# anilshanbhag/gpu-sort

Measured on AMD Instinct MI355X. Metric: Gkeys/s sorting 2^30 uint32 keys; achieved HBM GB/s vs roofline, higher is better.
Workload: dtype u32; 1 GPU; lsb_radix_sort_2^30_u32_uniform_keys_only; keys_per_gpu=1073741824, algorithm=lsb, distribution=uniform, parallelism=single

## Files before the change

### gpu-sort_amd/_lib.py

```python
import ctypes as C
import os

import torch

_HERE = os.path.dirname(os.path.abspath(__file__))
LIB_PATH = os.environ.get("GS_LIB_PATH", os.path.join(_HERE, "lib", "libgpusort.so"))
CSRC_DIR = os.path.join(_HERE, "csrc")
INCLUDE_DIR = os.path.join(os.path.dirname(_HERE), "include")

GS_KEY_U32, GS_KEY_I32, GS_KEY_F32, GS_KEY_U64, GS_KEY_I64, GS_KEY_F64 = 0, 1, 2, 3, 4, 5
GS_KEY_U8, GS_KEY_I8, GS_KEY_U16, GS_KEY_I16 = 6, 7, 8, 9
GS_KEY_F16, GS_KEY_BF16, GS_KEY_F8 = 10, 11, 12
GS_GEN_UNIFORM, GS_GEN_ZIPF, GS_GEN_ENTROPY_AND, GS_GEN_ENUMERATED = 0, 1, 2, 3

u64, i32, vp, sz = C.c_uint64, C.c_int, C.c_void_p, C.c_size_t
pp = C.POINTER(C.c_void_p)

SIGNATURES = {
    "gs_version": (i32, []),
    "gs_error_string": (C.c_char_p, [i32]),
    "gs_lsb_temp_bytes": (sz, [u64, i32]),
    "gs_lsb_sort_u32": (i32, [vp, sz, pp, pp, C.POINTER(i32), u64, i32, i32, i32, i32, vp]),
    "gs_lsb_copy_temp_bytes": (sz, [u64, i32]),
    "gs_lsb_sort_copy_u32": (i32, [vp, sz, vp, vp, vp, vp, u64, i32, i32, i32, i32, vp]),
    "gs_lsb_wide_temp_bytes": (sz, [u64, i32, i32]),
    "gs_lsb_sort_wide": (i32, [vp, sz, pp, pp, C.POINTER(i32), u64, i32, i32, i32, i32, i32, i32, vp]),
    "gs_lsb_any_temp_bytes": (sz, [u64, i32, i32]),
    "gs_lsb_sort_any": (i32, [vp, sz, vp, vp, vp, vp, u64, i32, i32, i32, i32, i32, vp]),
    "gs_lsb_narrow_temp_bytes": (sz, [u64, i32, i32]),
    "gs_lsb_sort_narrow": (i32, [vp, sz, vp, vp, vp, vp, u64, i32, i32, i32, i32, i32, vp]),
    "gs_lsb_narrow_tile": (C.c_uint32, [i32, i32]),
    "gs_lsb_geometry": (None, [u64, i32, C.POINTER(C.c_uint32), C.POINTER(C.c_uint32), C.POINTER(C.c_uint32)]),
    "gs_lsb_workspace_layout": (i32, [vp, u64, pp, pp, pp]),
    "gs_lsb_pipe_status": (i32, [vp, u64, C.POINTER(C.c_uint32), vp]),
    "gs_lsb_plan_status": (i32, [vp, u64, C.POINTER(C.c_uint32), vp]),
    "gs_lsb_plan_cursor_status": (i32, [vp, u64, C.POINTER(C.c_uint32), vp]),
    "gs_lsb_plan_peek_status": (i32, [C.POINTER(C.c_uint32)]),
    "gs_lsb_plan_look_only": (i32, [vp, vp, vp, u64, i32, i32, vp]),
    "gs_lsb_plan_layout": (i32, [u64, C.POINTER(C.c_uint64)]),
    "gs_lsb_upsweep_u32": (i32, [vp, sz, vp, u64, i32, i32, i32, i32, vp]),
    "gs_lsb_scan_spine": (i32, [vp, sz, u64, vp]),
    "gs_lsb_downsweep_u32": (i32, [vp, sz, vp, vp, vp, vp, u64, i32, i32, i32, i32, i32, vp]),
    "gs_msb_temp_bytes": (sz, [u64, i32]),
    "gs_msb_sort_u32": (i32, [vp, sz, vp, vp, u64, vp, vp, pp, pp, i32, vp, i32]),
    "gs_msb_wide_temp_bytes": (sz, [u64, i32, i32]),
    "gs_msb_sort_wide": (i32, [vp, sz, vp, vp, u64, vp, vp, i32, i32, pp, pp, i32, vp, i32]),
    "gs_msb_large_temp_bytes": (sz, [u64, i32]),
    "gs_msb_sort_large_u32": (i32, [vp, sz, vp, vp, u64, vp, vp, i32, vp, i32]),
    "gs_msb_large_wide_temp_bytes": (sz, [u64, i32, i32]),
    "gs_msb_sort_large_wide": (i32, [vp, sz, vp, vp, u64, vp, vp, i32, i32, i32, vp, i32]),
    "gs_lsb_large_temp_bytes": (sz, [u64, i32, i32]),
    "gs_lsb_sort_large": (i32, [vp, sz, pp, pp, C.POINTER(i32), u64, i32, i32, i32, i32, i32, i32, vp]),
    "gs_lsb_narrow_large_temp_bytes": (sz, [u64, i32, i32]),
    "gs_lsb_sort_narrow_large": (i32, [vp, sz, vp, vp, vp, vp, u64, i32, i32, i32, i32, i32, vp]),
    "gs_topk_temp_bytes": (sz, [u64, u64, i32]),
    "gs_topk_u32": (i32, [vp, sz, vp, vp, vp, vp, u64, u64, i32, i32, vp]),
    "gs_topk_status": (i32, [vp, u64, u64, i32, C.POINTER(C.c_uint32), vp]),
    "gs_topk_u16_temp_bytes": (sz, [u64, u64, i32]),
    "gs_topk_u16": (i32, [vp, sz, vp, vp, vp, vp, u64, u64, i32, i32, vp]),
    "gs_topk_u16_status": (i32, [vp, u64, u64, i32, C.POINTER(C.c_uint32), vp]),
    "gs_topk_u64_temp_bytes": (sz, [u64, u64, i32]),
    "gs_topk_u64": (i32, [vp, sz, vp, vp, vp, vp, u64, u64, i32, i32, vp]),
    "gs_topk_u64_status": (i32, [vp, u64, u64, i32, C.POINTER(C.c_uint32), vp]),
    "gs_topk_rows_temp_bytes": (sz, [u64, u64, u64, i32]),
    "gs_topk_rows_u32": (i32, [vp, sz, vp, vp, vp, vp, u64, u64, u64, u64, i32, i32, vp]),
    "gs_topk_rows_max_k": (C.c_uint32, []),
    "gs_topk_rows_plan": (i32, [u64, u64, u64, i32, C.POINTER(C.c_uint32)]),
    "gs_topk_rows_u16_temp_bytes": (sz, [u64, u64, u64, i32]),
    "gs_topk_rows_u16": (i32, [vp, sz, vp, vp, vp, vp, u64, u64, u64, u64, i32, i32, vp]),
    "gs_topk_rows_u64_temp_bytes": (sz, [u64, u64, u64, i32]),
    "gs_topk_rows_u64": (i32, [vp, sz, vp, vp, vp, vp, u64, u64, u64, u64, i32, i32, vp]),
    "gs_topk_segmented_temp_bytes": (sz, [u64, C.c_uint32, u64, i32]),
    "gs_topk_segmented_u32": (i32, [vp, sz, vp, vp, vp, vp, vp, u64, C.c_uint32, vp, vp, u64, i32, i32, vp]),
    "gs_topk_segmented_u16_temp_bytes": (sz, [u64, C.c_uint32, u64, i32]),
    "gs_topk_segmented_u16": (i32, [vp, sz, vp, vp, vp, vp, vp, u64, C.c_uint32, vp, vp, u64, i32, i32, vp]),
    "gs_topk_segmented_u64_temp_bytes": (sz, [u64, C.c_uint32, u64, i32]),
    "gs_topk_segmented_u64": (i32, [vp, sz, vp, vp, vp, vp, vp, u64, C.c_uint32, vp, vp, u64, i32, i32, vp]),
    "gs_topk_segmented_plan": (i32, [u64, C.c_uint32, u64, i32, C.POINTER(C.c_uint32)]),
    "gs_topk_segmented_status": (i32, [vp, u64, C.c_uint32, u64, i32, C.POINTER(C.c_uint32), vp]),
    "gs_msb_census": (i32, [vp, u64, i32, vp, vp]),
    "gs_msb_wide_census": (i32, [vp, u64, i32, i32, vp, vp]),
    "gs_msb_capacities": (None, [u64, i32, C.POINTER(C.c_uint32), C.POINTER(C.c_uint32), C.POINTER(C.c_uint32)]),
    "gs_msb_classify_upto": (i32, [vp, sz, vp, vp, u64, i32, i32, vp]),
    "gs_msb_read_lists": (i32, [vp, u64, i32, i32, vp, C.c_uint32, C.POINTER(C.c_uint32), C.POINTER(C.POINTER(C.c_uint32)), C.c_uint32,
                                C.POINTER(C.c_uint32), vp]),
    "gs_segmented_temp_bytes": (sz, [u64, i32, C.c_uint32]),
    "gs_segmented_sort_u32": (i32, [vp, sz, pp, pp, C.POINTER(i32), u64, C.c_uint32, vp, vp, i32, i32, i32, i32, vp]),
    "gs_segmented_wide_temp_bytes": (sz, [u64, i32, i32, C.c_uint32]),
    "gs_segmented_sort_wide": (i32, [vp, sz, pp, pp, C.POINTER(i32), u64, C.c_uint32, vp, vp, i32, i32, i32, i32, i32, i32, vp]),
    "gs_segmented_narrow_temp_bytes": (sz, [u64, i32, i32, C.c_uint32]),
    "gs_segmented_sort_narrow": (i32, [vp, sz, pp, pp, C.POINTER(i32), u64, C.c_uint32, vp, vp, i32, i32, i32, i32, i32, vp]),
    "gs_segmented_narrow_cap": (C.c_uint32, [i32, i32]),
    "gs_msb_first_pass_u32": (i32, [vp, sz, vp, vp, vp, vp, u64, i32, vp, vp]),
    "gs_msb_finish_temp_bytes": (sz, [u64, i32, i32]),
    "gs_msb_finish_u32": (i32, [vp, sz, vp, vp, vp, vp, u64, vp, i32, i32, vp, i32]),
    "gs_shard_histogram_u32": (i32, [vp, u64, i32, vp, i32, vp]),
    "gs_shard_partition_u32": (i32, [vp, sz, vp, vp, vp, vp, u64, i32, vp, i32, vp, vp, i32, vp]),
    "gs_generate_u32": (i32, [vp, u64, i32, u64, u64, i32, vp]),
    "gs_check_sorted_u32": (i32, [vp, u64, i32, vp, vp]),
    "gs_check_pairs_enumerated_u32": (i32, [vp, vp, vp, u64, vp, vp]),
    "gs_check_sorted_u64": (i32, [vp, u64, i32, vp, vp]),
    "gs_check_pairs_enumerated_wide": (i32, [vp, vp, vp, u64, i32, vp, vp]),
    "gs_check_sorted_stable": (i32, [vp, vp, u64, i32, i32, i32, i32, i32, vp, vp]),
    "gs_profile_create": (vp, []),
    "gs_profile_destroy": (None, [vp]),
    "gs_profile_begin": (None, [vp]),
    "gs_profile_end": (None, []),
    "gs_profile_read": (i32, [vp, C.POINTER(C.c_double), C.POINTER(u64)]),
    "gs_kernel_name": (C.c_char_p, [i32]),
}
GS_K_COUNT = 10


class GpuSortError(RuntimeError):
    def __init__(self, code, what):
        self.code = code
        super().__init__(f"{what}: hipError {code} ({error_string(code)})")


def _load():
    if not os.path.exists(LIB_PATH):
        raise ImportError(
            f"{LIB_PATH} is missing: the HIP extension is not built. "
            "Run `python -c 'import __graft_entry__ as g; g.build()'` (or make -C gpu-sort_amd/csrc). "
            "There is no CPU fallback."
        )
    lib = C.CDLL(LIB_PATH)
    for name, (res, args) in SIGNATURES.items():
        fn = getattr(lib, name)
        fn.restype = res
        fn.argtypes = args
    return lib


lib = _load()


def error_string(code):
    s = lib.gs_error_string(int(code))
    return s.decode() if s else "?"


def check(code, what):
    if code != 0:
        raise GpuSortError(code, what)


class KernelProfile:

    def __init__(self):
        self._p = lib.gs_profile_create()

    def __enter__(self):
        lib.gs_profile_begin(self._p)
        return self

    def __exit__(self, *exc):
        lib.gs_profile_end()
        return False

    def read(self):
        ms = (C.c_double * GS_K_COUNT)()
        cnt = (u64 * GS_K_COUNT)()
        check(lib.gs_profile_read(self._p, ms, cnt), "gs_profile_read")
        return {lib.gs_kernel_name(i).decode(): (ms[i], int(cnt[i])) for i in range(GS_K_COUNT) if cnt[i]}

    def close(self):
        if self._p and lib is not None:
            lib.gs_profile_destroy(self._p)
        self._p = None

    def __del__(self):
        try:
            self.close()
        except Exception:
            pass
```

### gpu-sort_amd/csrc/gs_lsb_downsweep.inc

```
#ifndef GS_EXP_SLEEP_MODE
#define GS_EXP_SLEEP_MODE 0
#endif
#ifndef GS_EXP_SLEEP_MIN_TILES
#define GS_EXP_SLEEP_MIN_TILES 49152u
#endif
#ifndef GS_EXP_SLEEP_PAIRS
#define GS_EXP_SLEEP_PAIRS 0
#endif
template <bool HAS_VALUES, bool OFF64 = false>
struct DownsweepSmem {
    uint32_t whist[LSB_WAVES][RADIX];
#ifdef GS_EXP_ALLWAVE_KEYS
    uint16_t wbase[LSB_WAVES][RADIX];
#else
    uint16_t wbase[HAS_VALUES ? LSB_WAVES : 1][RADIX];
#endif
    std::conditional_t<OFF64, uint64_t, uint32_t> gbase[RADIX];
    uint32_t stage[LSB_TILE * (HAS_VALUES ? 2 : 1)];
    uint32_t dead;
};

#ifdef GS_EXP_PHASES
__device__ uint32_t gs_phase_buf[131072 * 16];
#define GS_PHASE(k)                                                                          \
    do {                                                                                     \
        const unsigned long long now_ = __builtin_amdgcn_s_memtime();                        \
        if (tid == 0 && t < 131072u) gs_phase_buf[t * 16 + (k)] = (uint32_t)(now_ - tprev_); \
        tprev_ = now_;                                                                       \
    } while (0)
#define GS_PHASE_WAIT(what) asm volatile("s_waitcnt " what ::: "memory")
#else
#define GS_PHASE(k) do { } while (0)
#define GS_PHASE_WAIT(what) do { } while (0)
#endif

constexpr uint32_t PIPE_SPIN_LIMIT = 1u << 18;

template <bool HAS_VALUES, bool TAIL, int TW, bool BIG, bool PIPE, bool OFF64 = false, bool CURSOR = false>
__device__ __forceinline__ void downsweep_tile(DownsweepSmem<HAS_VALUES, OFF64> &sm, const uint32_t t,
    const uint32_t *__restrict__ keys_in, uint32_t *__restrict__ keys_out, const uint32_t *__restrict__ vals_in,
    uint32_t *__restrict__ vals_out, const uint32_t *__restrict__ spine, const uint16_t *__restrict__ prefix16,
    const uint32_t *__restrict__ totals, const PassParams &p, const uint64_t *__restrict__ sc, uint32_t tag,
    uint32_t *__restrict__ error_word, const uint32_t tid_ = threadIdx.x, const uint64_t *__restrict__ dbase = nullptr,
    uint32_t *__restrict__ cursor = nullptr, uint32_t *__restrict__ irr = nullptr, const uint32_t irr_cap = 0u)
{
    static_assert(!CURSOR || (!HAS_VALUES && !TAIL && !PIPE && !OFF64), "cursor mode: full tiles of keys-only three-launch passes");
#ifdef GS_EXP_ALLWAVE_KEYS
    constexpr bool ALLWAVE = true;
#else
    constexpr bool ALLWAVE = HAS_VALUES;
#endif

    [[maybe_unused]] const int tid = (int)tid_;
    const int lane = (int)(tid_ & 63u), w = (int)(tid_ >> 6);
    const uint32_t full_tiles = p.n / (uint32_t)LSB_TILE;
    auto tw_in = [&](uint32_t k) { return TW == 0 ? k : twiddle_in(k, TW == 2 ? p.f32_in : 0, p.xor_in); };
    auto tw_out = [&](uint32_t k) { return TW == 0 ? k : twiddle_out(k, TW == 2 ? p.f32_out : 0, p.xor_out); };
    uint32_t wbits = p.bits;
    asm volatile("" : "+v"(wbits));
    auto digit = [&](uint32_t k) { return __builtin_amdgcn_ubfe(k, p.shift, wbits); };

    uint32_t *my = sm.whist[w];
    const uint16_t *mybase = sm.wbase[w];
    const uint32_t wbase = (uint32_t)w * (WAVE * LSB_KPT) + lane;
    const uint32_t tail_valid = p.n - full_tiles * (uint32_t)LSB_TILE;
    (void)full_tiles;

#ifdef GS_EXP_PHASES
    unsigned long long tprev_ = __builtin_amdgcn_s_memtime();
    const unsigned long long t0_ = tprev_, r0_ = __builtin_amdgcn_s_memrealtime();
#endif
#ifdef GS_EXP_SLEEP_START
    __builtin_amdgcn_s_sleep(GS_EXP_SLEEP_START);
#endif
    if (!HAS_VALUES) __builtin_amdgcn_s_setprio(3);
    const uint64_t tile_base = (uint64_t)t * LSB_TILE;
    const uint32_t valid = TAIL ? tail_valid : (uint32_t)LSB_TILE;

    uint64_t scg[4] = {0, 0, 0, 0};
    const uint64_t *scrow = nullptr;
    if (PIPE && w == 0) {
        scrow = sc + (size_t)(t / LSB_CHUNK) * RADIX + 4 * lane;
#pragma unroll
        for (int q = 0; q < 4; ++q) scg[q] = ld_agent(scrow + q);
    }

    uint32_t key[LSB_KPT], val[HAS_VALUES ? LSB_KPT : 1], pos[LSB_KPT];
    {
        const uint32_t *kin = keys_in + tile_base;
        if (!TAIL) {
#pragma unroll
            for (int i = 0; i < LSB_KPT; ++i) key[i] = kin[wbase + i * WAVE];
        } else {
            const uint32_t pad = twiddle_out(0xffffffffu, TW == 2 ? p.f32_in : 0, TW ? p.xor_in : 0u);
#pragma unroll
            for (int i = 0; i < LSB_KPT; ++i) {
                const uint32_t idx = wbase + i * WAVE;
                key[i] = pad;
                if (idx < tail_valid) key[i] = kin[idx];
            }
        }
    }
    [[maybe_unused]] uint32_t cur_lo = 0, cur_hi = 0, claim[4] = {0, 0, 0, 0};
    if constexpr (CURSOR) {
        if (w == 0) {
            cur_lo = (tw_in(keys_in[tile_base]) >> (p.shift - (uint32_t)RADIX_BITS)) & (uint32_t)(RADIX - 1);
            cur_hi = (tw_in(keys_in[tile_base + (LSB_TILE - 1)]) >> (p.shift - (uint32_t)RADIX_BITS)) & (uint32_t)(RADIX - 1);
        }
    }
    GS_PHASE(0);
#ifndef GS_EXP_RANK_PRIO
#define GS_EXP_RANK_PRIO 0
#endif
    if (!HAS_VALUES) __builtin_amdgcn_s_setprio(GS_EXP_RANK_PRIO);
    if (HAS_VALUES) {
        const uint32_t *vin = vals_in + tile_base;
#pragma unroll
        for (int i = 0; i < LSB_KPT; ++i) {
            const uint32_t idx = wbase + i * WAVE;
            val[i] = 0;
            if (!TAIL || idx < valid) val[i] = vin[idx];
        }
    }
    uint32_t dstart[4] = {0, 0, 0, 0};
    if constexpr (OFF64) {
        if (TAIL && w == 0) {
            const uint4 tot = reinterpret_cast<const uint4 *>(totals)[lane];
            dstart[0] = tot.x; dstart[1] = tot.y; dstart[2] = tot.z; dstart[3] = tot.w;
        }
    } else if (!CURSOR && w == 0) {
        const uint4 tot = reinterpret_cast<const uint4 *>(totals)[lane];
        const uint32_t lane_sum = tot.x + tot.y + tot.z + tot.w;
        const uint32_t ex = wave_inclusive_scan(lane_sum) - lane_sum;
        dstart[0] = ex + (TAIL ? tot.x : 0u);
        dstart[1] = dstart[0] + (TAIL ? tot.y : tot.x);
        dstart[2] = dstart[1] + (TAIL ? tot.z : tot.y);
        dstart[3] = dstart[2] + (TAIL ? tot.w : tot.z);
    }

    uint32_t tbase[4] = {0, 0, 0, 0};
    if (!TAIL && !PIPE && !CURSOR && w == 0) {
        const uint32_t *sp = spine + (uint32_t)(4 * lane) * p.grid + t / LSB_CHUNK;
        const uint2 pf = reinterpret_cast<const uint2 *>(prefix16 + (size_t)t * RADIX)[lane];
        tbase[0] = sp[0] + (pf.x & 0xffffu);
        tbase[1] = sp[p.grid] + (pf.x >> 16);
        tbase[2] = sp[2 * p.grid] + (pf.y & 0xffffu);
        tbase[3] = sp[3 * p.grid] + (pf.y >> 16);
    }

    if (PIPE && !TAIL && w == 0) {
        uint32_t spins = 0;
        bool gave_up = false;
        for (;;) {
            const bool ok = (uint32_t)(scg[0] >> 32) == tag && (uint32_t)(scg[1] >> 32) == tag &&
                            (uint32_t)(scg[2] >> 32) == tag && (uint32_t)(scg[3] >> 32) == tag;
            if (__builtin_amdgcn_ballot_w64(!ok) == 0) break;
            if (++spins > PIPE_SPIN_LIMIT) {
                if (lane == 0) atomicOr(error_word, 1u);
                gave_up = true;
                break;
            }
            __builtin_amdgcn_s_sleep(8);
#pragma unroll
            for (int q = 0; q < 4; ++q) scg[q] = ld_agent(scrow + q);
        }
        if (lane == 0) sm.dead = gave_up ? 1u : 0u;
        const uint64_t pf = ld_agent(reinterpret_cast<const uint64_t *>(prefix16 + (size_t)t * RADIX) + lane);
        tbase[0] = (uint32_t)scg[0] + (uint32_t)(pf & 0xffffu);
        tbase[1] = (uint32_t)scg[1] + (uint32_t)((pf >> 16) & 0xffffu);
        tbase[2] = (uint32_t)scg[2] + (uint32_t)((pf >> 32) & 0xffffu);
        tbase[3] = (uint32_t)scg[3] + (uint32_t)(pf >> 48);
    }

    auto publish_gbase = [&](const uint32_t (&ex)[4], const uint32_t (&run)[4]) {
        uint32_t g[4];
#pragma unroll
        for (int q = 0; q < 4; ++q) g[q] = dstart[q] + tbase[q] - ex[q];
        if (TAIL) {
#pragma unroll
            for (int q = 0; q < 4; ++q) g[q] -= run[q];
            const uint32_t pads = (uint32_t)LSB_TILE - valid, dmax = p.mask;
            if (lane == (int)(dmax >> 2)) {
#pragma unroll
                for (int q = 0; q < 4; ++q)
                    if ((dmax & 3u) == (uint32_t)q) g[q] += pads;
            }
        }
        if constexpr (OFF64) {
#pragma unroll
            for (int q = 0; q < 4; ++q) sm.gbase[4 * lane + q] = dbase[4 * lane + q] + (uint64_t)(int64_t)(int32_t)g[q];
        } else {
            if (!BIG) {
#pragma unroll
                for (int q = 0; q < 4; ++q) g[q] <<= 2;
            }
            reinterpret_cast<uint4 *>(sm.gbase)[lane] = make_uint4(g[0], g[1], g[2], g[3]);
        }
    };

#pragma unroll
    for (int i = lane; i < RADIX; i += WAVE) my[i] = 0;
    GS_PHASE_WAIT("vmcnt(0)");
    GS_PHASE(1);
#pragma unroll
    for (int i = 0; i < LSB_KPT; ++i) key[i] = tw_in(key[i]);
    {
        uint32_t d_prev = 0, plo = 0, phi = 0;
#pragma unroll
        for (int i = 0; i <= LSB_KPT; ++i) {
            uint32_t d_cur = 0, clo = 0, chi = 0;
            if (i < LSB_KPT) {
                d_cur = digit(key[i]);
                match_digit(d_cur, clo, chi);
            }
            if (i > 0) {
                const uint32_t lower = count_lower(plo, phi);
                pos[i - 1] = my[d_prev] + lower;
                if (lower == 0)
                    __hip_atomic_fetch_add(&my[d_prev], (uint32_t)(__popc(plo) + __popc(phi)), __ATOMIC_RELAXED,
                                           __HIP_MEMORY_SCOPE_WAVEFRONT);
            }
            d_prev = d_cur; plo = clo; phi = chi;
        }
    }
#pragma unroll
    for (int i = 0; i < LSB_KPT; ++i) {
        asm volatile("" : "+v"(pos[i]), "+v"(key[i]));
    }
    if constexpr (CURSOR) {
        if (w == 0 && lane == 0) {
            const bool straddles = cur_lo != cur_hi;
            sm.dead = straddles ? 1u : 0u;
            if (straddles) {
                const uint32_t at = atomicAdd(&irr[0], 1u);
                if (at < irr_cap) irr[1u + at] = t;
            }
        }
    }
    GS_PHASE_WAIT("lgkmcnt(0)");
    GS_PHASE(2);
    __syncthreads();
    GS_PHASE(3);
    if (PIPE && !TAIL && sm.dead) return;
    if (CURSOR && sm.dead) return;

    if constexpr (ALLWAVE) {
        uint32_t run[4] = {0, 0, 0, 0}, below[4] = {0, 0, 0, 0};
#pragma unroll
        for (int j = 0; j < LSB_WAVES; ++j) {
            const uint4 x = reinterpret_cast<const uint4 *>(sm.whist[j])[lane];
            run[0] += x.x; run[1] += x.y; run[2] += x.z; run[3] += x.w;
            if (j < w) { below[0] += x.x; below[1] += x.y; below[2] += x.z; below[3] += x.w; }
        }
        const uint32_t lane_sum = run[0] + run[1] + run[2] + run[3];
        uint32_t ex[4];
        ex[0] = wave_inclusive_scan(lane_sum) - lane_sum;
        ex[1] = ex[0] + run[0];
        ex[2] = ex[1] + run[1];
        ex[3] = ex[2] + run[2];
        reinterpret_cast<uint2 *>(sm.wbase[w])[lane] =
            make_uint2((ex[0] + below[0]) | ((ex[1] + below[1]) << 16), (ex[2] + below[2]) | ((ex[3] + below[3]) << 16));
        if (w == 0) publish_gbase(ex, run);
    } else {
        if (w == 0) {
            uint32_t run[4] = {0, 0, 0, 0};
#pragma unroll
            for (int j = 0; j < LSB_WAVES; ++j) {
                const uint4 x = reinterpret_cast<const uint4 *>(sm.whist[j])[lane];
                run[0] += x.x; run[1] += x.y; run[2] += x.z; run[3] += x.w;
            }
            const uint32_t lane_sum = run[0] + run[1] + run[2] + run[3];
            uint32_t ex[4];
            ex[0] = wave_inclusive_scan(lane_sum) - lane_sum;
            ex[1] = ex[0] + run[0];
            ex[2] = ex[1] + run[1];
            ex[3] = ex[2] + run[2];
            if constexpr (CURSOR) {
                reinterpret_cast<uint4 *>(sm.gbase)[lane] = make_uint4(ex[0], ex[1], ex[2], ex[3]);
                uint32_t *row = cursor + (size_t)__builtin_amdgcn_readfirstlane(cur_lo) * RADIX;
#pragma unroll
                for (int q = 0; q < 4; ++q) {
                    const int d = q * WAVE + lane;
                    const uint32_t e0 = sm.gbase[d], e1 = sm.gbase[d == RADIX - 1 ? d : d + 1];
                    const uint32_t cnt = (d == RADIX - 1 ? (uint32_t)LSB_TILE : e1) - e0;
                    claim[q] = __hip_atomic_fetch_add(row + d, cnt, __ATOMIC_RELAXED, __HIP_MEMORY_SCOPE_AGENT);
                }
            } else {
                publish_gbase(ex, run);
            }
            asm volatile("" ::: "memory");
            uint4 e4 = make_uint4(ex[0] << 2, ex[1] << 2, ex[2] << 2, ex[3] << 2);
#pragma unroll
            for (int j = 0; j < LSB_WAVES; ++j) {
                const uint4 x = reinterpret_cast<const uint4 *>(sm.whist[j])[lane];
                reinterpret_cast<uint4 *>(sm.whist[j])[lane] = e4;
                e4.x += x.x << 2; e4.y += x.y << 2; e4.z += x.z << 2; e4.w += x.w << 2;
            }
        }
        __syncthreads();
    }
    GS_PHASE(4);

    {
        uint32_t wb[LSB_KPT];
#pragma unroll
        for (int i = 0; i < LSB_KPT; ++i) {
            const uint32_t d = digit(key[i]);
            wb[i] = ALLWAVE ? (uint32_t)mybase[d] : my[d];
        }
#pragma unroll
        for (int i = 0; i < LSB_KPT; ++i) {
            if (HAS_VALUES) {
                reinterpret_cast<uint2 *>(sm.stage)[pos[i] + wb[i]] = make_uint2(key[i], val[i]);
            } else if (ALLWAVE) {
                sm.stage[pos[i] + wb[i]] = key[i];
            } else {
                const uint32_t at = (pos[i] << 2) + wb[i];
                *reinterpret_cast<uint32_t *>(reinterpret_cast<char *>(sm.stage) + at) = key[i];
            }
        }
    }
    if constexpr (CURSOR) {
        if (w == 0) {
#pragma unroll
            for (int q = 0; q < 4; ++q) {
                const int d = q * WAVE + lane;
                const uint32_t g = claim[q] - sm.gbase[d];
                sm.gbase[d] = BIG ? g : g << 2;
            }
        }
    }
    GS_PHASE_WAIT("lgkmcnt(0)");
    GS_PHASE(5);
    __syncthreads();
    GS_PHASE(6);
#ifndef GS_EXP_SLEEP
#define GS_EXP_SLEEP 32
#define GS_EXP_SLEEP_MODE_DEFAULT 0
#else
#define GS_EXP_SLEEP_MODE_DEFAULT GS_EXP_SLEEP_MODE
#endif
    if ((!HAS_VALUES || GS_EXP_SLEEP_PAIRS) && full_tiles >= GS_EXP_SLEEP_MIN_TILES) {
        [[maybe_unused]] const int ws = __builtin_amdgcn_readfirstlane(w);
#if GS_EXP_SLEEP_MODE_DEFAULT == 3
        if (ws & 1) __builtin_amdgcn_s_sleep(GS_EXP_SLEEP); else __builtin_amdgcn_s_sleep(GS_EXP_SLEEP_B);
#elif GS_EXP_SLEEP_MODE_DEFAULT == 4
        if (ws >= 4) __builtin_amdgcn_s_sleep(GS_EXP_SLEEP);
#elif GS_EXP_SLEEP_MODE_DEFAULT == 1
        if (ws & 1) __builtin_amdgcn_s_sleep(GS_EXP_SLEEP);
#elif GS_EXP_SLEEP_MODE_DEFAULT == 0
        __builtin_amdgcn_s_sleep(GS_EXP_SLEEP);
#endif
    }
#ifndef GS_EXP_STORE_PRIO
#define GS_EXP_STORE_PRIO 3
#endif
    if (!HAS_VALUES) __builtin_amdgcn_s_setprio(GS_EXP_STORE_PRIO);
#pragma unroll
    for (int i = 0; i < LSB_KPT; ++i) {
        const uint32_t slot = (uint32_t)w * (WAVE * LSB_KPT) + i * WAVE + lane;
        uint32_t k, v = 0;
        if (HAS_VALUES) {
            const uint2 kv = reinterpret_cast<const uint2 *>(sm.stage)[slot];
            k = kv.x; v = kv.y;
        } else {
            k = sm.stage[slot];
        }
        const auto g = sm.gbase[digit(k)];
        if (!TAIL || slot < valid) {
            if constexpr (OFF64) {
                const uint64_t dst = g + slot;
                keys_out[dst] = tw_out(k);
                if (HAS_VALUES) vals_out[dst] = v;
            } else if (BIG) {
                const uint32_t dst = g + slot;
                keys_out[dst] = tw_out(k);
                if (HAS_VALUES) vals_out[dst] = v;
            } else {
                const uint32_t off = g + slot * 4u;
                *reinterpret_cast<uint32_t *>(reinterpret_cast<char *>(keys_out) + off) = tw_out(k);
                if (HAS_VALUES) *reinterpret_cast<uint32_t *>(reinterpret_cast<char *>(vals_out) + off) = v;
            }
        }
    }
    GS_PHASE(7);
#ifdef GS_EXP_DRAIN
    asm volatile("s_waitcnt vmcnt(0)" ::: "memory");
#endif
    GS_PHASE_WAIT("vmcnt(0)");
    GS_PHASE(8);
#ifdef GS_EXP_PHASES
    if (tid == 0 && t < 131072u) {
        gs_phase_buf[t * 16 + 9] = (uint32_t)(__builtin_amdgcn_s_memtime() - t0_);
        gs_phase_buf[t * 16 + 10] = (uint32_t)(__builtin_amdgcn_s_memrealtime() - r0_);
        gs_phase_buf[t * 16 + 11] = (uint32_t)r0_;
        gs_phase_buf[t * 16 + 12] = blockIdx.x;
        gs_phase_buf[t * 16 + 13] = __builtin_amdgcn_s_getreg((31 << 11) | 4);
        gs_phase_buf[t * 16 + 14] = __builtin_amdgcn_s_getreg((31 << 11) | 20);
    }
#endif
}
```

### gpu-sort_amd/csrc/gs_lsb_plan.hip

```cpp
#include "gs_device.hpp"
#include "gs_lsb.hpp"
#include "gs_msb_tasks.hpp"
#ifndef GS_PLAN_N_MIN
#define GS_PLAN_N_MIN (1ull << 28)
#endif
#include <cstddef>
#include <cstdlib>
#include <cstring>
#include <type_traits>

namespace gs {

#include "gs_lsb_upsweep.inc"

#include "gs_lsb_downsweep.inc"

constexpr uint32_t PLAN_GROUPS = 65536;
constexpr uint32_t PLAN_WORDS = PLAN_GROUPS / 2;
constexpr uint32_t PLAN_PLANNED = 1u, PLAN_CLASSIC = 2u;
constexpr uint32_t PLAN_SKIP = 0xffffffffu;
constexpr int PLAN_LOOK_THREADS = 1024, PLAN_LOOK_WAVES = PLAN_LOOK_THREADS / WAVE, PLAN_LOOK_BATCH = 32;
constexpr uint32_t PLAN_LOOK_HALVES = PLAN_LOOK_WAVES / LSB_CHUNK;
static_assert(PLAN_LOOK_WAVES % LSB_CHUNK == 0, "a look workgroup takes whole chunks");
constexpr uint32_t PLAN_LOOK_MAX_GRID = MI355X_CUS;
constexpr uint32_t PLAN_BLOCKS = 128, PLAN_BLOCK_WORDS = PLAN_WORDS / PLAN_BLOCKS, PLAN_BLOCK_GROUPS = PLAN_GROUPS / PLAN_BLOCKS;
constexpr int PLAN_SORT_BITS = 16;
constexpr int PLAN_SKEW_LANES = 8;
constexpr uint32_t PLAN_IRR_CAP = RADIX - 1;
constexpr size_t PLAN_CURSOR_BYTES = (size_t)PLAN_GROUPS * sizeof(uint32_t);

struct PlanBlock {
    uint32_t route, max_group, nonempty, tasks[MSB_NCLASS], total;
    uint32_t shift[4];
    uint32_t ups_skip[4];
    MsbLevel level[2];
    union {
        uint32_t wg_bad[PLAN_LOOK_MAX_GRID];
        uint32_t irr[1 + PLAN_IRR_CAP];
    };
    uint32_t blk_total[PLAN_BLOCKS], blk_max[PLAN_BLOCKS], blk_nonempty[PLAN_BLOCKS];
    uint32_t blk_class[PLAN_BLOCKS][MSB_NCLASS];
    uint32_t blk_class_base[PLAN_BLOCKS][MSB_NCLASS];
    uint32_t offsets[PLAN_GROUPS + 1];
    uint32_t cursor_mode;
};
static_assert(1 + PLAN_IRR_CAP <= PLAN_LOOK_MAX_GRID, "the list of straddling tiles fits the look's flags");
static_assert(sizeof(MsbLevel) == 64 && offsetof(PlanBlock, level) == 64, "plan block layout");

__device__ __forceinline__ int plan_class_of(uint32_t size)
{
    return size <= msb_class_cap(0) ? 0 : size <= msb_class_cap(1) ? 1 : size <= msb_class_cap(2) ? 2 : 3;
}

__device__ __forceinline__ void look_add(uint32_t *tab, uint32_t *my, uint32_t g)
{
    const unsigned long long act = __builtin_amdgcn_ballot_w64(true);
    const uint32_t g0 = __builtin_amdgcn_readfirstlane(g);
    if (__builtin_amdgcn_ballot_w64(g == g0) == act) {
        if (count_lower_mask(act) == 0) {
            atomicAdd(&tab[g0 >> 1], (uint32_t)__popcll(act) << ((g0 & 1u) * 16u));
            atomicAdd(&my[g0 & 0xffu], (uint32_t)__popcll(act));
        }
    } else {
        atomicAdd(&tab[g >> 1], 1u << ((g & 1u) * 16u));
        atomicAdd(&my[g & 0xffu], 1u);
    }
}

__device__ __forceinline__ void look_add_skew(uint32_t *tab, uint32_t *my, uint32_t g, int lane)
{
    unsigned long long rest = ~0ull;
#pragma unroll
    for (int r = 0; r < 2; ++r) {
        if (rest == 0ull) break;
        const int lead = __builtin_amdgcn_readfirstlane(__builtin_ctzll(rest));
        const uint32_t g0 = (uint32_t)__builtin_amdgcn_readlane((int)g, lead);
        const unsigned long long m = __builtin_amdgcn_ballot_w64(g == g0) & rest;
        if (lane == lead) {
            atomicAdd(&tab[g0 >> 1], (uint32_t)__popcll(m) << ((g0 & 1u) * 16u));
            atomicAdd(&my[g0 & 0xffu], (uint32_t)__popcll(m));
        }
        rest &= ~m;
    }
    if ((rest >> lane) & 1ull) {
        atomicAdd(&tab[g >> 1], 1u << ((g & 1u) * 16u));
        atomicAdd(&my[g & 0xffu], 1u);
    }
}

__device__ __forceinline__ uint32_t look_slot_of_block(uint32_t b, uint32_t grid)
{
    if (grid % MI355X_XCDS) return b;
    return (b % MI355X_XCDS) * (grid / MI355X_XCDS) + b / MI355X_XCDS;
}

struct LookSmem {
    uint32_t tab[PLAN_WORDS];
    uint32_t hist[PLAN_LOOK_WAVES][RADIX + 1];
    uint32_t red[2];
};
static_assert(sizeof(LookSmem) <= 160 * 1024, "the look's LDS");

__global__ __launch_bounds__(PLAN_LOOK_THREADS) void lsb_plan_look_kernel(const uint32_t *__restrict__ keys, uint32_t *__restrict__ partial,
                                                                          PlanBlock *__restrict__ plan, uint32_t *__restrict__ spine,
                                                                          uint16_t *__restrict__ prefix16, uint32_t n, uint32_t chunks,
                                                                          int f32_in, uint32_t xor_in)
{
    __shared__ LookSmem sm;
    uint32_t *tab = sm.tab;
    const int tid = threadIdx.x, w = wave_id(), lane = lane_id();
    for (uint32_t i = tid; i < PLAN_WORDS; i += PLAN_LOOK_THREADS) tab[i] = 0;
    for (uint32_t i = tid; i < sizeof(sm.hist) / sizeof(uint32_t); i += PLAN_LOOK_THREADS) (&sm.hist[0][0])[i] = 0;
    if (tid < 2) sm.red[tid] = 0;
    __syncthreads();
    uint32_t *my = sm.hist[w];
    const uint32_t num_tiles = n / (uint32_t)LSB_TILE + (n % (uint32_t)LSB_TILE ? 1u : 0u);
    const uint32_t units = (chunks + PLAN_LOOK_HALVES - 1u) / PLAN_LOOK_HALVES;
    auto group_of = [&](uint32_t raw) { return twiddle_in(raw, f32_in, xor_in) >> 16; };
    uint32_t counted = 0;
    constexpr int GB = PLAN_LOOK_BATCH;
#pragma unroll 1
    for (uint32_t unit = look_slot_of_block(blockIdx.x, gridDim.x); unit < units; unit += gridDim.x) {
        const uint32_t tile = unit * (uint32_t)PLAN_LOOK_WAVES + (uint32_t)w;
        if (tile < num_tiles) {
        const uint32_t lo = tile * (uint32_t)LSB_TILE;
        const uint32_t len = (n - lo < (uint32_t)LSB_TILE) ? n - lo : (uint32_t)LSB_TILE;
        const uint32_t *src = keys + lo;
        counted += len;
        if (len == (uint32_t)LSB_TILE) {
#pragma unroll 1
            for (uint32_t j = 0; j < (uint32_t)LSB_TILE; j += GB * WAVE) {
                const uint32_t *at = src + j + lane;
                uint32_t v[GB];
#pragma unroll
                for (int u = 0; u < GB; ++u) v[u] = __builtin_nontemporal_load(at + u * WAVE);
                const uint32_t ga = group_of(v[0]), gb = group_of(v[GB / 2]);
                const unsigned long long ma = __builtin_amdgcn_ballot_w64(ga == __builtin_amdgcn_readfirstlane(ga)),
                                         mb = __builtin_amdgcn_ballot_w64(gb == __builtin_amdgcn_readfirstlane(gb));
                if (ma == ~0ull || mb == ~0ull) {
#pragma unroll
                    for (int u = 0; u < GB; ++u) look_add(tab, my, group_of(v[u]));
                } else if (__popcll(ma) >= PLAN_SKEW_LANES || __popcll(mb) >= PLAN_SKEW_LANES) {
#pragma unroll
                    for (int u = 0; u < GB; ++u) look_add_skew(tab, my, group_of(v[u]), lane);
                } else {
#pragma unroll
                    for (int u = 0; u < GB; ++u) {
                        const uint32_t g = group_of(v[u]);
                        atomicAdd(&tab[g >> 1], 1u << ((g & 1u) * 16u));
                        atomicAdd(&my[g & 0xffu], 1u);
                    }
                }
            }
        } else {
            const uint32_t last = len - 1u;
#pragma unroll 1
            for (uint32_t j = 0; j < len; j += GB * WAVE) {
                uint32_t v[GB];
#pragma unroll
                for (int u = 0; u < GB; ++u) {
                    const uint32_t idx = j + u * WAVE + lane;
                    v[u] = src[idx < last ? idx : last];
                }
#pragma unroll
                for (int u = 0; u < GB; ++u)
                    if (j + u * WAVE + lane < len) look_add(tab, my, group_of(v[u]));
            }
        }
        }
        __syncthreads();
        if (tid < (int)PLAN_LOOK_HALVES * RADIX) {
            const uint32_t half = (uint32_t)tid / RADIX, d = (uint32_t)tid % RADIX, chunk = unit * PLAN_LOOK_HALVES + half;
            uint32_t run = 0;
#pragma unroll
            for (int j = 0; j < LSB_CHUNK; ++j) {
                const uint32_t t = chunk * LSB_CHUNK + (uint32_t)j;
                if (t < num_tiles) prefix16[(size_t)t * RADIX + d] = (uint16_t)run;
                uint32_t *c = &sm.hist[half * LSB_CHUNK + j][d];
                run += *c;
                *c = 0;
            }
            if (chunk < chunks) spine[d * chunks + chunk] = run;
        }
        __syncthreads();
    }
    uint32_t sum = 0;
    uint32_t *out = partial + (size_t)blockIdx.x * PLAN_WORDS;
    for (uint32_t i = tid; i < PLAN_WORDS; i += PLAN_LOOK_THREADS) {
        const uint32_t c = tab[i];
        sum += (c & 0xffffu) + (c >> 16);
        out[i] = c;
    }
    sum = wave_reduce_sum(sum);
    if (lane == 0) { atomicAdd(&sm.red[0], sum); atomicAdd(&sm.red[1], counted); }
    __syncthreads();
    if (tid == 0) plan->wg_bad[blockIdx.x] = sm.red[0] != sm.red[1] ? 1u : 0u;
}

__global__ __launch_bounds__(RADIX) void lsb_plan_reduce_kernel(const uint32_t *__restrict__ partial, PlanBlock *__restrict__ plan, uint32_t parts)
{
    __shared__ uint32_t scratch[8];
    __shared__ uint32_t red[2 + MSB_NCLASS];
    const uint32_t tid = threadIdx.x, wi = blockIdx.x * PLAN_BLOCK_WORDS + tid;
    if (tid < 2 + MSB_NCLASS) red[tid] = 0;
    uint32_t c0 = 0, c1 = 0;
#pragma unroll 8
    for (uint32_t g = 0; g < parts; ++g) {
        const uint32_t v = partial[(size_t)g * PLAN_WORDS + wi];
        c0 += v & 0xffffu;
        c1 += v >> 16;
    }
    uint32_t total = 0;
    const uint32_t ex = block_exclusive_scan_256(c0 + c1, scratch, &total);
    plan->offsets[2 * wi] = ex;
    plan->offsets[2 * wi + 1] = ex + c0;
    atomicMax(&red[0], c0 > c1 ? c0 : c1);
    if (c0) { atomicAdd(&red[1], 1u); atomicAdd(&red[2 + plan_class_of(c0)], 1u); }
    if (c1) { atomicAdd(&red[1], 1u); atomicAdd(&red[2 + plan_class_of(c1)], 1u); }
    __syncthreads();
    if (tid == 0) {
        plan->blk_total[blockIdx.x] = total;
        plan->blk_max[blockIdx.x] = red[0];
        plan->blk_nonempty[blockIdx.x] = red[1];
    }
    if (tid < MSB_NCLASS) plan->blk_class[blockIdx.x][tid] = red[2 + tid];
}

__global__ __launch_bounds__(RADIX) void lsb_plan_decide_kernel(PlanBlock *__restrict__ plan, uint32_t n, uint32_t parts, uint32_t cursor_on)
{
    __shared__ uint32_t s_base, s_total, s_max, s_nz, s_cls[MSB_NCLASS], s_clsbase[MSB_NCLASS];
    const uint32_t tid = threadIdx.x, b = blockIdx.x;
    if (tid == 0) {
        uint32_t base = 0, total = 0, mx = 0, nz = 0;
        for (uint32_t i = 0; i < PLAN_BLOCKS; ++i) {
            if (i == b) base = total;
            total += plan->blk_total[i];
            const uint32_t m = plan->blk_max[i];
            mx = m > mx ? m : mx;
            nz += plan->blk_nonempty[i];
        }
        s_base = base; s_total = total; s_max = mx; s_nz = nz;
    } else if (tid <= MSB_NCLASS) {
        const uint32_t c = tid - 1u;
        uint32_t base = 0, total = 0;
        for (uint32_t i = 0; i < PLAN_BLOCKS; ++i) {
            if (i == b) base = total;
            total += plan->blk_class[i][c];
        }
        s_cls[c] = total; s_clsbase[c] = base;
    }
    const int any_bad = __syncthreads_or(tid < parts ? (int)plan->wg_bad[tid] : 0);
    const uint32_t g = b * PLAN_BLOCK_GROUPS + 2u * tid;
    plan->offsets[g] += s_base;
    plan->offsets[g + 1] += s_base;
    if (tid < MSB_NCLASS) plan->blk_class_base[b][tid] = s_clsbase[tid];
    if (b == 0 && tid == 0) {
        const bool planned = !any_bad && s_total == n && s_max <= msb_class_cap(MSB_NCLASS - 1);
        plan->route = planned ? PLAN_PLANNED : PLAN_CLASSIC;
        plan->max_group = s_max;
        plan->nonempty = s_nz;
        plan->total = s_total;
        MsbLevel l0{}, l1{};
        for (int c = 0; c < MSB_NCLASS; ++c) {
            plan->tasks[c] = planned ? s_cls[c] : 0u;
            l0.task_count[c] = planned ? s_cls[c] : 0u;
        }
        l0.keys = n;
        l1.packed = planned ? (1ull << 32) : 0ull;
        plan->level[0] = l0;
        plan->level[1] = l1;
        for (int q = 0; q < 4; ++q) {
            plan->shift[q] = planned ? (q < 2 ? 16u + 8u * (uint32_t)q : PLAN_SKIP) : 8u * (uint32_t)q;
            plan->ups_skip[q] = planned && q != 1 ? 1u : 0u;
        }
        plan->offsets[PLAN_GROUPS] = n;
        plan->cursor_mode = planned && cursor_on ? 1u : 0u;
    }
}

constexpr int PLAN_PEEK_WORDS = 9;
static_assert(offsetof(PlanBlock, total) == (PLAN_PEEK_WORDS - 2) * sizeof(uint32_t), "the head is eight words");
__global__ void lsb_plan_peek_kernel(const PlanBlock *__restrict__ plan, uint32_t *mailbox)
{
    const uint32_t *head = &plan->route;
    for (int i = 0; i < PLAN_PEEK_WORDS - 1; ++i) mailbox[i] = head[i];
    mailbox[PLAN_PEEK_WORDS - 1] = plan->cursor_mode;
    __threadfence_system();
}

struct PlanLists { MsbTask *tasks[MSB_NCLASS]; uint32_t cap[MSB_NCLASS]; };
__global__ __launch_bounds__(PLAN_BLOCK_GROUPS) void lsb_plan_tasks_kernel(const PlanBlock *__restrict__ plan, PlanLists lists)
{
    __shared__ uint32_t wcnt[PLAN_BLOCK_GROUPS / WAVE][MSB_NCLASS];
    if (plan->route != PLAN_PLANNED) return;
    const uint32_t tid = threadIdx.x, g = blockIdx.x * PLAN_BLOCK_GROUPS + tid;
    const int w = wave_id(), lane = lane_id();
    const uint32_t off = plan->offsets[g], size = plan->offsets[g + 1] - off;
    const int cls = size ? plan_class_of(size) : -1;
    uint32_t lower = 0;
#pragma unroll
    for (int c = 0; c < MSB_NCLASS; ++c) {
        const unsigned long long m = __builtin_amdgcn_ballot_w64(cls == c);
        if (cls == c) lower = count_lower_mask(m);
        if (lane == 0) wcnt[w][c] = (uint32_t)__popcll(m);
    }
    __syncthreads();
    if (cls >= 0) {
        uint32_t idx = plan->blk_class_base[blockIdx.x][cls] + lower;
        for (int j = 0; j < w; ++j) idx += wcnt[j][cls];
        if (idx < lists.cap[cls]) lists.tasks[cls][idx] = MsbTask{off, size, (uint32_t)PLAN_SORT_BITS, 0u};
    }
}

template <bool PLAIN>
__global__ __launch_bounds__(LSB_THREADS, GS_EXP_UPS_WPE) void lsb_plan_upsweep_kernel(const uint32_t *__restrict__ keys,
                                                                       uint32_t *__restrict__ spine, uint16_t *__restrict__ prefix16,
                                                                       const uint32_t *__restrict__ slot_shift,
                                                                       const uint32_t *__restrict__ slot_ups_skip, PassParams p)
{
    __shared__ UpsweepSmem<false, false> sm;
    const uint32_t sh = *slot_shift;
    if (sh == PLAN_SKIP || *slot_ups_skip) return;
    p.shift = sh;
    upsweep_chunk<false, false, PLAIN>(sm, keys, chunk_of_block(blockIdx.x, p.grid), spine, prefix16, nullptr, nullptr, p, PipeParams{});
}

template <bool TAIL, int TW, bool BIG>
__global__ __launch_bounds__(LSB_THREADS, 6) void lsb_plan_downsweep_kernel(const uint32_t *__restrict__ keys_in, uint32_t *__restrict__ keys_out,
                                                                            const uint32_t *__restrict__ totals, const uint32_t *__restrict__ spine,
                                                                            const uint16_t *__restrict__ prefix16,
                                                                            const uint32_t *__restrict__ slot_shift, PassParams p)
{
    __shared__ __attribute__((aligned(16))) DownsweepSmem<false> sm;
    const uint32_t sh = *slot_shift;
    if (sh == PLAN_SKIP) return;
    p.shift = sh;
    const uint32_t full_tiles = p.n / (uint32_t)LSB_TILE;
    if (!TAIL && blockIdx.x >= full_tiles) return;
    const uint32_t t = TAIL ? full_tiles : tile_of_item_wide(blockIdx.x, full_tiles);
    downsweep_tile<false, TAIL, TW, BIG, false>(sm, t, keys_in, keys_out, nullptr, nullptr, spine, prefix16, totals, p, nullptr, 0u, nullptr);
}

template <bool PLAIN>
__global__ __launch_bounds__(LSB_THREADS, GS_EXP_UPS_WPE) void lsb_plan_upsweep2_kernel(const uint32_t *__restrict__ keys,
                                                                        uint32_t *__restrict__ spine, uint16_t *__restrict__ prefix16,
                                                                        PlanBlock *__restrict__ plan, uint32_t *__restrict__ cursor,
                                                                        PassParams p)
{
    __shared__ UpsweepSmem<false, false> sm;
    if (plan->cursor_mode) {
        if (blockIdx.x == 0 && threadIdx.x == 0) plan->irr[0] = 0;
        for (uint32_t i = blockIdx.x * (uint32_t)LSB_THREADS + threadIdx.x; i < PLAN_GROUPS; i += gridDim.x * (uint32_t)LSB_THREADS)
            cursor[i] = plan->offsets[((i & (uint32_t)(RADIX - 1)) << RADIX_BITS) | (i >> RADIX_BITS)];
        return;
    }
    const uint32_t sh = plan->shift[1];
    if (sh == PLAN_SKIP || plan->ups_skip[1]) return;
    p.shift = sh;
    upsweep_chunk<false, false, PLAIN>(sm, keys, chunk_of_block(blockIdx.x, p.grid), spine, prefix16, nullptr, nullptr, p, PipeParams{});
}

template <bool TAIL, bool BIG>
__global__ __launch_bounds__(LSB_THREADS, 6) void lsb_plan_scatter2_kernel(const uint32_t *__restrict__ keys_in, uint32_t *__restrict__ keys_out,
                                                                           const uint32_t *__restrict__ totals, const uint32_t *__restrict__ spine,
                                                                           const uint16_t *__restrict__ prefix16, PlanBlock *__restrict__ plan,
                                                                           uint32_t *__restrict__ cursor, PassParams p)
{
    __shared__ __attribute__((aligned(16))) DownsweepSmem<false> sm;
    const uint32_t sh = plan->shift[1];
    if (sh == PLAN_SKIP) return;
    p.shift = sh;
    const uint32_t full_tiles = p.n / (uint32_t)LSB_TILE;
    const uint32_t mode = plan->cursor_mode;
    if constexpr (TAIL) {
        if (mode) return;
        downsweep_tile<false, true, 2, true, false>(sm, full_tiles, keys_in, keys_out, nullptr, nullptr, spine, prefix16, totals, p, nullptr, 0u,
                                                    nullptr);
    } else {
        if (blockIdx.x >= full_tiles) return;
        const uint32_t t = tile_of_item_wide(blockIdx.x, full_tiles);
        if (mode)
            downsweep_tile<false, false, 0, BIG, false, false, true>(sm, t, keys_in, keys_out, nullptr, nullptr, spine, prefix16, totals, p,
                                                                     nullptr, 0u, nullptr, threadIdx.x, nullptr, cursor, plan->irr, PLAN_IRR_CAP);
        else
            downsweep_tile<false, false, 0, BIG, false>(sm, t, keys_in, keys_out, nullptr, nullptr, spine, prefix16, totals, p, nullptr, 0u,
                                                        nullptr);
    }
}

__global__ __launch_bounds__(LSB_THREADS) void lsb_plan_irregular_kernel(const uint32_t *__restrict__ keys_in, uint32_t *__restrict__ keys_out,
                                                                         const PlanBlock *__restrict__ plan, uint32_t *__restrict__ cursor,
                                                                         uint32_t n)
{
    if (!plan->cursor_mode) return;
    const uint32_t full_tiles = n / (uint32_t)LSB_TILE;
    uint32_t lo, len;
    if (blockIdx.x == PLAN_IRR_CAP) {
        lo = full_tiles * (uint32_t)LSB_TILE;
        len = n - lo;
    } else {
        const uint32_t listed = plan->irr[0] < PLAN_IRR_CAP ? plan->irr[0] : PLAN_IRR_CAP;
        if (blockIdx.x >= listed) return;
        const uint32_t t = plan->irr[1u + blockIdx.x];
        if (t >= full_tiles) return;
        lo = t * (uint32_t)LSB_TILE;
        len = (uint32_t)LSB_TILE;
    }
    const int lane = lane_id();
    for (uint32_t i = threadIdx.x; i - (uint32_t)lane < len; i += (uint32_t)LSB_THREADS) {
        const bool have = i < len;
        const uint32_t k = have ? keys_in[lo + i] : 0u;
        const uint32_t g = k >> 16, c = ((g & (uint32_t)(RADIX - 1)) << RADIX_BITS) | (g >> RADIX_BITS);
        unsigned long long rest = __builtin_amdgcn_ballot_w64(have);
        uint32_t at = 0;
#pragma unroll
        for (int r = 0; r < 2; ++r) {
            if (rest == 0ull) break;
            const int lead = __builtin_amdgcn_readfirstlane(__builtin_ctzll(rest));
            const uint32_t c0 = (uint32_t)__builtin_amdgcn_readlane((int)c, lead);
            const unsigned long long m = __builtin_amdgcn_ballot_w64(have && c == c0) & rest;
            uint32_t first = 0;
            if (lane == lead) first = __hip_atomic_fetch_add(cursor + c0, (uint32_t)__popcll(m), __ATOMIC_RELAXED, __HIP_MEMORY_SCOPE_AGENT);
            first = (uint32_t)__builtin_amdgcn_readlane((int)first, lead);
            if ((m >> lane) & 1ull) at = first + (uint32_t)__popcll(m & ((1ull << lane) - 1ull));
            rest &= ~m;
        }
        if ((rest >> lane) & 1ull) at = __hip_atomic_fetch_add(cursor + c, 1u, __ATOMIC_RELAXED, __HIP_MEMORY_SCOPE_AGENT);
        if (have && at < n) keys_out[at] = k;
    }
}

static inline size_t align256(size_t x) { return (x + 255) & ~(size_t)255; }

static inline bool plan_enabled()
{
    static const bool v = [] { const char *e = getenv("GS_LSB_KEYS_PLAN"); return !(e && strcmp(e, "classic") == 0); }();
    return v;
}
static inline bool plan_cursor_enabled()
{
    static const bool v = [] { const char *e = getenv("GS_LSB_PLAN_SCATTER2"); return !(e && strcmp(e, "stable") == 0); }();
    return v;
}
constexpr uint64_t PLAN_N_MAX = (uint64_t)PLAN_GROUPS * 16620u;
constexpr uint64_t PLAN_N_FLOOR = 65536;
constexpr uint64_t PLAN_N_MIN = GS_PLAN_N_MIN;
static inline uint64_t plan_min_items()
{
    static const uint64_t v = [] {
        const char *e = getenv("GS_LSB_PLAN_MIN_ITEMS");
        if (!e) return PLAN_N_MIN;
        const uint64_t x = strtoull(e, nullptr, 10);
        return x < PLAN_N_FLOOR ? PLAN_N_FLOOR : x;
    }();
    return v;
}
static inline bool plan_has_block(uint64_t n) { return !lsb_pipe_enabled() && n >= plan_min_items(); }
static inline bool plan_size_ok(uint64_t n) { return plan_has_block(n) && n <= PLAN_N_MAX; }
static inline uint32_t plan_list_cap(uint64_t n, int c)
{
    const uint64_t m = c == 0 ? n : n / ((uint64_t)msb_class_cap(c - 1) + 1u) + 1u;
    return (uint32_t)(m < PLAN_GROUPS ? m : PLAN_GROUPS);
}
static inline size_t plan_lists_bytes(uint64_t n)
{
    size_t b = 0;
    for (int c = 0; c < MSB_NCLASS; ++c) b += (size_t)plan_list_cap(n, c) * sizeof(MsbTask);
    return b;
}
static inline size_t plan_block_offset(uint64_t n)
{
    const size_t a = lsb_temp_bytes(n), b = plan_lists_bytes(n);
    return align256(a > b ? a : b);
}
static inline size_t plan_temp_bytes(uint64_t n) { return plan_block_offset(n) + align256(sizeof(PlanBlock)); }
static inline uint32_t *plan_cursors(char *base, uint64_t n) { return (uint32_t *)(base + plan_block_offset(n) - PLAN_CURSOR_BYTES); }

template <int TW, bool BIG>
static void launch_plan_downsweep(const uint32_t *kin, uint32_t *kout, const LsbWorkspace &ws, const uint32_t *slot_shift,
                                  const PassParams &p, hipStream_t s)
{
    hipLaunchKernelGGL((lsb_plan_downsweep_kernel<false, TW, BIG>), dim3(p.ds_grid), dim3(LSB_THREADS), 0, s, kin, kout, ws.totals,
                       ws.spine, ws.prefix16, slot_shift, p);
}

static int lsb_plan_slot2(const uint32_t *kin, uint32_t *kout, const LsbWorkspace &ws, PlanBlock *plan, uint32_t *cursor,
                          const PassParams &p, hipStream_t s);
static int lsb_plan_slot(const uint32_t *kin, uint32_t *kout, const LsbWorkspace &ws, const uint32_t *slot_shift,
                         const uint32_t *slot_ups_skip, const PassParams &p, bool real, bool ups_real, hipStream_t s)
{
    {
        KernelTimer kt(ups_real ? GS_K_LSB_UPSWEEP : GS_K_OTHER, s);
        if (!p.f32_in && !p.xor_in)
            hipLaunchKernelGGL(lsb_plan_upsweep_kernel<true>, dim3(p.grid), dim3(LSB_THREADS), 0, s, kin, ws.spine, ws.prefix16, slot_shift,
                               slot_ups_skip, p);
        else
            hipLaunchKernelGGL(lsb_plan_upsweep_kernel<false>, dim3(p.grid), dim3(LSB_THREADS), 0, s, kin, ws.spine, ws.prefix16, slot_shift,
                               slot_ups_skip, p);
    }
    {
        if (const int e = lsb_scan_as(ws.spine, ws.totals, p.grid, s, real ? GS_K_LSB_SCAN : GS_K_OTHER)) return e;
    }
    {
        KernelTimer kt(real ? GS_K_LSB_DOWNSWEEP : GS_K_OTHER, s);
        if (p.n >= (uint32_t)LSB_TILE) {
            const int tw = (p.f32_in || p.f32_out) ? 2 : ((p.xor_in | p.xor_out) ? 1 : 0);
            const bool big = p.n > (1u << 30);
#define GS_PDS(TW_, BIG_) launch_plan_downsweep<TW_, BIG_>(kin, kout, ws, slot_shift, p, s)
            if (big) { if (tw == 2) GS_PDS(2, true); else if (tw == 1) GS_PDS(1, true); else GS_PDS(0, true); }
            else { if (tw == 2) GS_PDS(2, false); else if (tw == 1) GS_PDS(1, false); else GS_PDS(0, false); }
#undef GS_PDS
        }
        if (p.n % (uint32_t)LSB_TILE)
            hipLaunchKernelGGL((lsb_plan_downsweep_kernel<true, 2, true>), dim3(1), dim3(LSB_THREADS), 0, s, kin, kout, ws.totals,
                               (const uint32_t *)nullptr, (const uint16_t *)nullptr, slot_shift, p);
    }
    return (int)hipGetLastError();
}

static int lsb_plan_slot2(const uint32_t *kin, uint32_t *kout, const LsbWorkspace &ws, PlanBlock *plan, uint32_t *cursor,
                          const PassParams &p, hipStream_t s)
{
    if (p.f32_in || p.f32_out || p.xor_in || p.xor_out) return hipErrorInvalidValue;
    if ((char *)cursor < (char *)ws.prefix16) return hipErrorInvalidValue;
    {
        KernelTimer kt(GS_K_OTHER, s);
        hipLaunchKernelGGL(lsb_plan_upsweep2_kernel<true>, dim3(p.grid), dim3(LSB_THREADS), 0, s, kin, ws.spine, ws.prefix16, plan, cursor, p);
    }
    if (const int e = lsb_scan_as(ws.spine, ws.totals, p.grid, s, GS_K_LSB_SCAN)) return e;
    {
        KernelTimer kt(GS_K_LSB_DOWNSWEEP, s);
        if (p.n >= (uint32_t)LSB_TILE) {
            if (p.n > (1u << 30))
                hipLaunchKernelGGL((lsb_plan_scatter2_kernel<false, true>), dim3(p.ds_grid), dim3(LSB_THREADS), 0, s, kin, kout, ws.totals,
                                   ws.spine, ws.prefix16, plan, cursor, p);
            else
                hipLaunchKernelGGL((lsb_plan_scatter2_kernel<false, false>), dim3(p.ds_grid), dim3(LSB_THREADS), 0, s, kin, kout, ws.totals,
                                   ws.spine, ws.prefix16, plan, cursor, p);
        }
        if (p.n % (uint32_t)LSB_TILE)
            hipLaunchKernelGGL((lsb_plan_scatter2_kernel<true, true>), dim3(1), dim3(LSB_THREADS), 0, s, kin, kout, ws.totals,
                               (const uint32_t *)nullptr, (const uint16_t *)nullptr, plan, cursor, p);
    }
    {
        KernelTimer kt(GS_K_OTHER, s);
        hipLaunchKernelGGL(lsb_plan_irregular_kernel, dim3(PLAN_IRR_CAP + (p.n % (uint32_t)LSB_TILE ? 1u : 0u)), dim3(LSB_THREADS), 0, s, kin,
                           kout, plan, cursor, p.n);
    }
    return (int)hipGetLastError();
}

static int lsb_plan_look(const uint32_t *keys, uint32_t *alt, const LsbWorkspace &ws, PlanBlock *plan, uint64_t n, const PassParams &tw,
                         hipStream_t s)
{
    const uint32_t parts = (uint32_t)(n / PLAN_WORDS < PLAN_LOOK_MAX_GRID ? n / PLAN_WORDS : PLAN_LOOK_MAX_GRID);
    const uint32_t chunks = lsb_make_params(n, 16, RADIX_BITS).grid;
    KernelTimer kt(GS_K_OTHER, s);
    hipLaunchKernelGGL(lsb_plan_look_kernel, dim3(parts), dim3(PLAN_LOOK_THREADS), 0, s, keys, alt, plan, ws.spine, ws.prefix16, (uint32_t)n,
                       chunks, tw.f32_in, tw.xor_in);
    hipLaunchKernelGGL(lsb_plan_reduce_kernel, dim3(PLAN_BLOCKS), dim3(RADIX), 0, s, alt, plan, parts);
    hipLaunchKernelGGL(lsb_plan_decide_kernel, dim3(PLAN_BLOCKS), dim3(RADIX), 0, s, plan, (uint32_t)n, parts, plan_cursor_enabled() ? 1u : 0u);
    return (int)hipGetLastError();
}

static int lsb_plan_slot2_cursor(const uint32_t *kin, uint32_t *kout, const LsbWorkspace &ws, PlanBlock *plan, uint32_t *cursor,
                                 const PassParams &p, hipStream_t s)
{
    if (p.f32_in || p.f32_out || p.xor_in || p.xor_out) return hipErrorInvalidValue;
    if ((char *)cursor < (char *)ws.prefix16) return hipErrorInvalidValue;
    {
        KernelTimer kt(GS_K_OTHER, s);
        hipLaunchKernelGGL(lsb_plan_upsweep2_kernel<true>, dim3(p.grid), dim3(LSB_THREADS), 0, s, kin, ws.spine, ws.prefix16, plan, cursor, p);
    }
    if (p.n >= (uint32_t)LSB_TILE) {
        KernelTimer kt(GS_K_LSB_DOWNSWEEP, s);
        if (p.n > (1u << 30))
            hipLaunchKernelGGL((lsb_plan_scatter2_kernel<false, true>), dim3(p.ds_grid), dim3(LSB_THREADS), 0, s, kin, kout, ws.totals,
                               ws.spine, ws.prefix16, plan, cursor, p);
        else
            hipLaunchKernelGGL((lsb_plan_scatter2_kernel<false, false>), dim3(p.ds_grid), dim3(LSB_THREADS), 0, s, kin, kout, ws.totals,
                               ws.spine, ws.prefix16, plan, cursor, p);
    }
    {
        KernelTimer kt(GS_K_OTHER, s);
        hipLaunchKernelGGL(lsb_plan_irregular_kernel, dim3(PLAN_IRR_CAP + (p.n % (uint32_t)LSB_TILE ? 1u : 0u)), dim3(LSB_THREADS), 0, s, kin,
                           kout, plan, cursor, p.n);
    }
    return (int)hipGetLastError();
}

struct PlanPeek {
    uint32_t *host = nullptr, *dev = nullptr;
    hipEvent_t ev = nullptr;
    int device = -1;
    bool armed = false;
};
static bool plan_peek_enabled()
{
    static const bool on = [] { const char *e = getenv("GS_LSB_PLAN_PEEK"); return !(e && e[0] == '0'); }();
    return on;
}
constexpr int PLAN_PEEK_DEVICES = 16;
struct PlanPeekTable {
    PlanPeek slot[PLAN_PEEK_DEVICES];
    ~PlanPeekTable()
    {
        for (PlanPeek &pk : slot) {
            if (pk.ev) (void)hipEventDestroy(pk.ev);
            if (pk.host) (void)hipHostFree(pk.host);
        }
    }
};
static PlanPeek *plan_peek_get(hipStream_t s)
{
    if (!plan_peek_enabled()) return nullptr;
    hipStreamCaptureStatus cs = hipStreamCaptureStatusNone;
    if (hipStreamIsCapturing(s, &cs) != hipSuccess || cs != hipStreamCaptureStatusNone) { (void)hipGetLastError(); return nullptr; }
    thread_local PlanPeekTable table;
    int dev = -1;
    if (hipGetDevice(&dev) != hipSuccess || dev < 0 || dev >= PLAN_PEEK_DEVICES) { (void)hipGetLastError(); return nullptr; }
    PlanPeek &pk = table.slot[dev];
    if (pk.device != dev) {
        void *h = nullptr, *d = nullptr;
        if (hipHostMalloc(&h, 64, hipHostMallocMapped | hipHostMallocPortable) != hipSuccess ||
            hipHostGetDevicePointer(&d, h, 0) != hipSuccess ||
            hipEventCreateWithFlags(&pk.ev, hipEventDisableTiming) != hipSuccess) {
            (void)hipGetLastError();
            if (h) (void)hipHostFree(h);
            pk.ev = nullptr;
            return nullptr;
        }
        pk.host = (uint32_t *)h; pk.dev = (uint32_t *)d; pk.device = dev;
    }
    if (pk.armed) { (void)hipEventSynchronize(pk.ev); (void)hipGetLastError(); }
    pk.armed = false;
    return &pk;
}
static void plan_peek_arm(PlanPeek *pk, const PlanBlock *plan, hipStream_t s)
{
    if (!pk) return;
    for (int i = 0; i < PLAN_PEEK_WORDS; ++i) ((volatile uint32_t *)pk->host)[i] = 0;
    KernelTimer kt(GS_K_OTHER, s);
    hipLaunchKernelGGL(lsb_plan_peek_kernel, dim3(1), dim3(1), 0, s, plan, pk->dev);
    pk->armed = hipGetLastError() == hipSuccess && hipEventRecord(pk->ev, s) == hipSuccess;
    if (!pk->armed) (void)hipGetLastError();
}
struct PlanSeen { bool ok = false; uint32_t route = 0, tasks[MSB_NCLASS] = {0, 0, 0, 0}, cursor_mode = 0; };
static PlanSeen plan_peek_wait(PlanPeek *pk, uint64_t n)
{
    PlanSeen seen;
    if (!pk || !pk->armed) return seen;
    pk->armed = false;
    if (hipEventSynchronize(pk->ev) != hipSuccess) { (void)hipGetLastError(); return seen; }
    uint32_t w[PLAN_PEEK_WORDS];
    for (int i = 0; i < PLAN_PEEK_WORDS; ++i) w[i] = ((const volatile uint32_t *)pk->host)[i];
    const uint32_t route = w[0], nonempty = w[2], total = w[7], mode = w[8];
    if (route != PLAN_PLANNED && route != PLAN_CLASSIC) return seen;
    if (route == PLAN_PLANNED ? (uint64_t)total != n : (uint64_t)total > n) return seen;
    if (mode > 1u || (mode && route != PLAN_PLANNED)) return seen;
    uint64_t sum = 0;
    for (int c = 0; c < MSB_NCLASS; ++c) {
        if (w[3 + c] > plan_list_cap(n, c)) return seen;
        sum += w[3 + c];
    }
    if (route == PLAN_PLANNED ? sum != nonempty : sum != 0) return seen;
    seen.ok = true;
    seen.route = route;
    seen.cursor_mode = mode;
    for (int c = 0; c < MSB_NCLASS; ++c) seen.tasks[c] = w[3 + c];
    return seen;
}
static thread_local uint32_t plan_peek_last[4] = {0, 0, 0, 0};

int lsb_plan_sort(char *base, uint32_t *d_keys[2], int *selector, uint64_t n, int descending, int key_type, hipStream_t s)
{
    const LsbWorkspace ws = lsb_carve(base, n);
    char *lists_end = base + plan_block_offset(n);
    PlanBlock *plan = (PlanBlock *)lists_end;
    PlanLists lists;
    for (int c = MSB_NCLASS - 1; c >= 0; --c) {
        lists.cap[c] = plan_list_cap(n, c);
        lists_end -= (size_t)lists.cap[c] * sizeof(MsbTask);
        lists.tasks[c] = (MsbTask *)lists_end;
    }
    int sel = *selector, e;
    PassParams tw{};
    lsb_twiddle_masks(key_type, descending, true, true, tw);
    if ((e = lsb_plan_look(d_keys[sel], d_keys[sel ^ 1], ws, plan, n, tw, s))) return e;
    PlanPeek *peek = plan_peek_get(s);
    plan_peek_arm(peek, plan, s);
    PlanSeen seen;
    plan_peek_last[0] = plan_peek_last[1] = 0; plan_peek_last[2] = 4; plan_peek_last[3] = (1u << MSB_NCLASS) - 1u;
    for (int slot = 0; slot < 4; ++slot) {
        PassParams p = lsb_make_params(n, 0, RADIX_BITS);
        lsb_twiddle_masks(key_type, descending, slot == 0, slot == 3, p);
        const uint32_t *kin = d_keys[sel];
        uint32_t *kout = d_keys[sel ^ 1];
        e = hipSuccess;
        if (seen.ok && seen.route == PLAN_CLASSIC)
            e = lsb_plan_slot(kin, kout, ws, &plan->shift[slot], &plan->ups_skip[slot], p, true, true, s);
        else if (seen.ok && slot >= 2)
            ;
        else if (seen.ok && slot == 1 && seen.cursor_mode)
            e = lsb_plan_slot2_cursor(kin, kout, ws, plan, plan_cursors(base, n), p, s);
        else if (slot == 1 && plan_cursor_enabled())
            e = lsb_plan_slot2(kin, kout, ws, plan, plan_cursors(base, n), p, s);
        else
            e = lsb_plan_slot(kin, kout, ws, &plan->shift[slot], &plan->ups_skip[slot], p, slot < 2, slot == 1, s);
        if (e) return e;
        sel ^= 1;
        if (slot == 0) {
            seen = plan_peek_wait(peek, n);
            if (seen.ok) {
                plan_peek_last[0] = 1; plan_peek_last[1] = seen.route; plan_peek_last[2] = seen.route == PLAN_PLANNED ? 2 : 4;
                plan_peek_last[3] = 0;
                for (int c = 0; c < MSB_NCLASS; ++c) plan_peek_last[3] |= seen.tasks[c] ? 1u << c : 0u;
            }
        }
    }
    if (seen.ok && seen.route == PLAN_CLASSIC) {
        *selector = sel;
        return hipSuccess;
    }
    {
        KernelTimer kt(GS_K_OTHER, s);
        hipLaunchKernelGGL(lsb_plan_tasks_kernel, dim3(PLAN_BLOCKS), dim3(PLAN_BLOCK_GROUPS), 0, s, plan, lists);
    }
    if ((e = (int)hipGetLastError())) return e;
    if ((e = msb_local_sorts_in_place(plan->level, lists.tasks, PLAN_GROUPS, PLAN_GROUPS, d_keys[sel], PLAN_SORT_BITS, n, tw.f32_out,
                                      tw.xor_out, s, seen.ok ? seen.tasks : nullptr)))
        return e;
    *selector = sel;
    return hipSuccess;
}


bool lsb_plan_has_block(uint64_t n) { return plan_has_block(n); }
size_t lsb_plan_temp_bytes(uint64_t n) { return plan_temp_bytes(n); }
bool lsb_plan_applies(uint64_t n) { return plan_enabled() && plan_size_ok(n); }

}

using namespace gs;

extern "C" {

int gs_lsb_plan_status(void *d_temp, uint64_t num_items, uint32_t out[8], void *stream)
{
    GS_CLEAR_STALE_ERROR();
    if (!d_temp || !out || num_items >= (1ull << 32)) return hipErrorInvalidValue;
    memset(out, 0, 8 * sizeof(uint32_t));
    if (!plan_enabled() || !plan_size_ok(num_items)) return hipSuccess;
    const PlanBlock *plan = (const PlanBlock *)(gs_ws_base(d_temp) + plan_block_offset(num_items));
    hipError_t e = hipMemcpyAsync(out, plan, 8 * sizeof(uint32_t), hipMemcpyDeviceToHost, (hipStream_t)stream);
    if (e == hipSuccess) e = hipStreamSynchronize((hipStream_t)stream);
    return (int)e;
}

int gs_lsb_plan_cursor_status(void *d_temp, uint64_t num_items, uint32_t out[4], void *stream)
{
    GS_CLEAR_STALE_ERROR();
    if (!d_temp || !out || num_items >= (1ull << 32)) return hipErrorInvalidValue;
    memset(out, 0, 4 * sizeof(uint32_t));
    if (!plan_enabled() || !plan_size_ok(num_items)) return hipSuccess;
    const PlanBlock *plan = (const PlanBlock *)(gs_ws_base(d_temp) + plan_block_offset(num_items));
    uint32_t w[2] = {0, 0};
    hipError_t e = hipMemcpyAsync(&w[0], &plan->cursor_mode, sizeof(uint32_t), hipMemcpyDeviceToHost, (hipStream_t)stream);
    if (e == hipSuccess) e = hipMemcpyAsync(&w[1], &plan->irr[0], sizeof(uint32_t), hipMemcpyDeviceToHost, (hipStream_t)stream);
    if (e == hipSuccess) e = hipStreamSynchronize((hipStream_t)stream);
    if (e != hipSuccess) return (int)e;
    if (w[0] == 1u) {
        out[0] = 1;
        out[2] = w[1];
        out[1] = w[1] + (num_items % (uint64_t)LSB_TILE ? 1u : 0u);
    }
    return hipSuccess;
}

int gs_lsb_plan_peek_status(uint32_t out[4])
{
    if (!out) return hipErrorInvalidValue;
    memcpy(out, plan_peek_last, sizeof(plan_peek_last));
    return hipSuccess;
}

int gs_lsb_plan_look_only(void *d_temp, const void *d_keys, void *d_alt, uint64_t num_items, int key_type, int descending, void *stream)
{
    GS_CLEAR_STALE_ERROR();
    if (!d_temp || !d_keys || !d_alt || num_items >= (1ull << 32)) return hipErrorInvalidValue;
    if (!plan_enabled() || !plan_size_ok(num_items)) return hipErrorInvalidValue;
    char *base = gs_ws_base(d_temp);
    PassParams tw{};
    lsb_twiddle_masks(key_type, descending, true, true, tw);
    return lsb_plan_look((const uint32_t *)d_keys, (uint32_t *)d_alt, lsb_carve(base, num_items), (PlanBlock *)(base + plan_block_offset(num_items)),
                         num_items, tw, (hipStream_t)stream);
}

int gs_lsb_plan_layout(uint64_t num_items, uint64_t out[4])
{
    if (!out || num_items >= (1ull << 32) || !plan_enabled() || !plan_size_ok(num_items)) return hipErrorInvalidValue;
    char *base = (char *)(uintptr_t)GS_WS_ALIGN;
    const LsbWorkspace ws = lsb_carve(base, num_items);
    out[0] = (uint64_t)((char *)ws.spine - base);
    out[1] = (uint64_t)((char *)ws.prefix16 - base);
    out[2] = plan_block_offset(num_items);
    out[3] = lsb_make_params(num_items, 16, RADIX_BITS).grid;
    return hipSuccess;
}

}
```

### gpu-sort_amd/csrc/gs_msb.hip

```cpp
#include "gs_device.hpp"
#include <new>
#include "gs_lsb.hpp"
#include "gs_msb_tasks.hpp"
#include <type_traits>
#include <vector>
#include <cstdlib>

namespace gs {

constexpr int MSB_THREADS = 512;
constexpr int MSB_WAVES = MSB_THREADS / WAVE;
constexpr int MSB_KPT = 16;
constexpr int MSB_TILE = MSB_THREADS * MSB_KPT;
constexpr uint32_t MSB_MERGE = 3000;
constexpr uint32_t MSB_MAX_GRID = 16384;
__host__ __device__ constexpr uint32_t msb_tiles_of(uint32_t x) { return x / (uint32_t)MSB_TILE + (x % (uint32_t)MSB_TILE ? 1u : 0u); }
#ifndef GS_PAIR_CLASSES
#define GS_PAIR_CLASSES 4
#endif
__host__ __device__ constexpr int msb_num_classes(bool has_values) { return has_values ? GS_PAIR_CLASSES : 4; }

struct MsbBucket { uint32_t offset, size, tile_start, tiles; };
struct MsbPiece { uint32_t lo, size, tile_start, bucket; };
struct MsbTile { uint32_t lo, valid, bucket, pad; };
// ... 685 lines not shown
    const uint32_t cand = P->cand, mid_lo = B.offset + P->less, mid_hi = mid_lo + P->eq;
    const uint32_t cand_out = twiddle_out(cand, f32_out, xor_out);
    uint32_t wl = 0, wg = 0;
#pragma unroll
    for (int i = 0; i < MSB_KPT; ++i) {
        const bool in = FULL || wbase + i * WAVE < valid;
        wl += (uint32_t)__popcll(__builtin_amdgcn_ballot_w64(in && key[i] < cand));
        wg += (uint32_t)__popcll(__builtin_amdgcn_ballot_w64(in && key[i] > cand));
    }
    if (lane == 0) { scratch[w] = wl; scratch[MSB_WAVES + w] = wg; }
    __syncthreads();
    if (threadIdx.x == 0) {
        uint32_t tl = 0, tg = 0;
#pragma unroll
        for (int j = 0; j < MSB_WAVES; ++j) { const uint32_t a = scratch[j], b2 = scratch[MSB_WAVES + j]; scratch[j] = tl; scratch[MSB_WAVES + j] = tg; tl += a; tg += b2; }
        scratch[2 * MSB_WAVES] = tl ? atomicAdd(&P->cur_less, tl) : 0u;
        scratch[2 * MSB_WAVES + 1] = tg ? atomicAdd(&P->cur_greater, tg) : 0u;
    }
    __syncthreads();
    uint32_t nl = B.offset + scratch[2 * MSB_WAVES] + scratch[w];
    uint32_t ng = B.offset + B.size - 1u - scratch[2 * MSB_WAVES + 1] - scratch[MSB_WAVES + w];
#pragma unroll
    for (int i = 0; i < MSB_KPT; ++i) {
        const uint32_t idx = wbase + i * WAVE;
        const bool in = FULL || idx < valid;
        const uint32_t k = key[i], at = lo + idx;
        const unsigned long long ml = __builtin_amdgcn_ballot_w64(in && k < cand), mg = __builtin_amdgcn_ballot_w64(in && k > cand);
        if (in) {
            if (k < cand) other[nl + count_lower_mask(ml)] = k;
            else if (k > cand) other[ng - count_lower_mask(mg)] = k;
            if (at >= mid_lo && at < mid_hi && (write_all || k != cand)) result[at] = cand_out;
        }
        nl += (uint32_t)__popcll(ml);
        ng -= (uint32_t)__popcll(mg);
    }
}

template <bool FULL>
__device__ __forceinline__ void msb_pivot_tile_pairs(uint32_t *__restrict__ scratch ,
                                                     MsbPivot *__restrict__ P, const MsbBucket &B, const uint32_t *__restrict__ src_k,
                                                     const uint32_t *__restrict__ src_v, uint32_t *__restrict__ other_k,
                                                     uint32_t *__restrict__ other_v, uint32_t *__restrict__ mid_k,
                                                     uint32_t *__restrict__ mid_v, uint32_t lo, uint32_t valid, int f32_out, uint32_t xor_out)
{
    const int lane = lane_id(), w = wave_id();
    const uint32_t wbase = (uint32_t)w * (WAVE * MSB_KPT) + lane;
    uint32_t key[MSB_KPT], val[MSB_KPT];
    const uint32_t *pk = src_k + lo, *pv = src_v + lo;
#pragma unroll
    for (int i = 0; i < MSB_KPT; ++i) {
        const uint32_t idx = wbase + i * WAVE, at = FULL ? idx : (idx < valid ? idx : valid - 1u);
        key[i] = pk[at]; val[i] = pv[at];
    }
    const uint32_t cand = P->cand, mid_lo = B.offset + P->less;
    const uint32_t cand_out = twiddle_out(cand, f32_out, xor_out);
    uint32_t wl = 0, wg = 0, we = 0;
#pragma unroll
    for (int i = 0; i < MSB_KPT; ++i) {
        const bool in = FULL || wbase + i * WAVE < valid;
        wl += (uint32_t)__popcll(__builtin_amdgcn_ballot_w64(in && key[i] < cand));
        wg += (uint32_t)__popcll(__builtin_amdgcn_ballot_w64(in && key[i] > cand));
        we += (uint32_t)__popcll(__builtin_amdgcn_ballot_w64(in && key[i] == cand));
    }
    if (lane == 0) { scratch[w] = wl; scratch[MSB_WAVES + w] = wg; scratch[2 * MSB_WAVES + w] = we; }
    __syncthreads();
    if (threadIdx.x == 0) {
        uint32_t tl = 0, tg = 0, te = 0;
#pragma unroll
        for (int j = 0; j < MSB_WAVES; ++j) {
            const uint32_t a = scratch[j], b2 = scratch[MSB_WAVES + j], c = scratch[2 * MSB_WAVES + j];
            scratch[j] = tl; scratch[MSB_WAVES + j] = tg; scratch[2 * MSB_WAVES + j] = te;
            tl += a; tg += b2; te += c;
        }
        scratch[3 * MSB_WAVES] = tl ? atomicAdd(&P->cur_less, tl) : 0u;
        scratch[3 * MSB_WAVES + 1] = tg ? atomicAdd(&P->cur_greater, tg) : 0u;
        scratch[3 * MSB_WAVES + 2] = te ? atomicAdd(&P->pad1, te) : 0u;
    }
    __syncthreads();
    uint32_t nl = B.offset + scratch[3 * MSB_WAVES] + scratch[w];
    uint32_t ng = B.offset + B.size - 1u - scratch[3 * MSB_WAVES + 1] - scratch[MSB_WAVES + w];
    uint32_t ne = mid_lo + scratch[3 * MSB_WAVES + 2] + scratch[2 * MSB_WAVES + w];
#pragma unroll
    for (int i = 0; i < MSB_KPT; ++i) {
        const bool in = FULL || wbase + i * WAVE < valid;
        const uint32_t k = key[i];
        const unsigned long long ml = __builtin_amdgcn_ballot_w64(in && k < cand), mg = __builtin_amdgcn_ballot_w64(in && k > cand),
                                 me = __builtin_amdgcn_ballot_w64(in && k == cand);
        if (in) {
            if (k < cand) { const uint32_t at = nl + count_lower_mask(ml); other_k[at] = k; other_v[at] = val[i]; }
            else if (k > cand) { const uint32_t at = ng - count_lower_mask(mg); other_k[at] = k; other_v[at] = val[i]; }
            else { const uint32_t at = ne + count_lower_mask(me); if (mid_k) mid_k[at] = cand_out; mid_v[at] = val[i]; }
        }
        nl += (uint32_t)__popcll(ml);
        ng -= (uint32_t)__popcll(mg);
        ne += (uint32_t)__popcll(me);
    }
}

__global__ __launch_bounds__(MSB_THREADS) void msb_pivot_copyback_kernel(MsbWs ws, int L, const uint32_t *__restrict__ from_v,
                                                                         uint32_t *__restrict__ result_k, uint32_t *__restrict__ result_v,
                                                                         int f32_out, uint32_t xor_out)
{
    const unsigned long long packed = ws.level[L].packed;
    if (blockIdx.x >= (uint32_t)packed) return;
    const MsbTile T = ws.tiles[blockIdx.x];
    const MsbPivot P = ws.pivots[T.bucket];
    if (!P.flag) return;
    const MsbBucket B = ws.buckets[L & 1][T.bucket];
    const uint32_t mid_lo = B.offset + P.less, mid_hi = mid_lo + P.eq, cand_out = twiddle_out(P.cand, f32_out, xor_out);
    for (uint32_t i = threadIdx.x; i < T.valid; i += MSB_THREADS) {
        const uint32_t at = T.lo + i;
        if (at >= mid_lo && at < mid_hi) { result_k[at] = cand_out; result_v[at] = from_v[at]; }
    }
}

template <bool HAS_VALUES, bool REMAP, bool TWOUT, bool FULL, bool BIG, bool PIVOT = false>
__global__ __launch_bounds__(MSB_THREADS, HAS_VALUES ? 4 : 6) void msb_scatter_kernel(
    MsbWs ws, int L, const uint32_t *__restrict__ src_k, uint32_t *__restrict__ dst_k, const uint32_t *__restrict__ src_v,
    uint32_t *__restrict__ dst_v, DigitSel ds, int f32_out, uint32_t xor_out, int ragged_anywhere,
    uint32_t *__restrict__ result_k = nullptr, int pivot_f32_out = 0, uint32_t pivot_xor_out = 0u, uint32_t *__restrict__ result_v = nullptr)
{
    __shared__ __attribute__((aligned(16))) ScatterSmem<HAS_VALUES, REMAP> sm;
    const unsigned long long packed = ws.level[L].packed;
    auto one_tile = [&](uint32_t g) {
        const MsbTile T = ws.tiles[g];
        if (FULL ? T.valid != (uint32_t)MSB_TILE : T.valid == (uint32_t)MSB_TILE) return;
        if (PIVOT && ws.pivots[T.bucket].flag) {
            const MsbBucket B = ws.buckets[L & 1][T.bucket];
            const bool in_place = result_k == src_k;
            if constexpr (HAS_VALUES) {
                msb_pivot_tile_pairs<FULL>(sm.gbase, ws.pivots + T.bucket, B, src_k, src_v, dst_k, dst_v, in_place ? (uint32_t *)nullptr : result_k,
                                           in_place ? dst_v : result_v, T.lo, T.valid, pivot_f32_out, pivot_xor_out);
            } else {
                msb_pivot_tile<FULL>(sm.gbase, ws.pivots + T.bucket, B, src_k, dst_k, result_k, T.lo, T.valid, pivot_f32_out, pivot_xor_out,
                                     !in_place || pivot_f32_out != 0 || pivot_xor_out != 0u);
            }
            return;
        }
        if (REMAP) load_remap(ds, sm.tab);
        msb_scatter_tile<HAS_VALUES, REMAP, TWOUT, FULL, BIG>(sm, ds, ws.cursors + (size_t)T.bucket * RADIX, ws.spine + g / MSB_WAVES,
                                                              ws.stride, ws.prefix16 + (size_t)g * RADIX, src_k, dst_k, src_v, dst_v,
                                                              T.lo, T.valid, f32_out, xor_out);
    };
    if (FULL) {
        if (blockIdx.x >= (uint32_t)packed) return;
#ifdef GS_MSB_WIDE_GROUP
        one_tile(tile_of_item_wide(blockIdx.x, (uint32_t)packed));
#else
        one_tile(tile_of_item(blockIdx.x, (uint32_t)packed));
#endif
    } else if (ragged_anywhere == 1) {
        if (blockIdx.x >= (uint32_t)packed) return;
        one_tile(blockIdx.x);
    } else {
        const bool two = ragged_anywhere == 2;
        const uint32_t b = two ? blockIdx.x >> 1 : blockIdx.x;
        if (b >= (uint32_t)(packed >> 32)) return;
        const MsbBucket B = ws.buckets[L & 1][b];
        const bool short_first = B.tiles >= 2u && ws_first_tile(ws, B.offset, B.size) != (1u << ws.tile_shift);
        if (two) {
            if (blockIdx.x & 1u) { if (short_first) one_tile(B.tile_start); }
            else one_tile(B.tile_start + B.tiles - 1u);
        } else {
            one_tile(B.tile_start + B.tiles - 1u);
            if (short_first) {
                __syncthreads();
                one_tile(B.tile_start);
            }
        }
    }
}

template <bool HAS_VALUES, bool REMAP, bool TWOUT>
static void launch_scatter(const MsbWs &ws, int L, uint32_t tiles_ub, uint32_t buckets_ub, bool big, const uint32_t *sk, uint32_t *dk,
                           const uint32_t *sv, uint32_t *dv, const DigitSel &ds, int f32_out, uint32_t xor_out, hipStream_t s,
                           bool ragged_anywhere = false, uint32_t *pivot_result = nullptr, int pivot_f32_out = 0,
                           uint32_t pivot_xor_out = 0u, uint32_t *pivot_result_v = nullptr)
{
    const dim3 blk(MSB_THREADS);
    const bool two_per_bucket = !ragged_anywhere && buckets_ub <= 1024u;
    const dim3 rg(ragged_anywhere ? tiles_ub : two_per_bucket ? 2u * buckets_ub : buckets_ub);
    const int ra = ragged_anywhere ? 1 : two_per_bucket ? 2 : 0;
    if constexpr (!REMAP) {
        if (pivot_result) {
            if (big) {
                hipLaunchKernelGGL((msb_scatter_kernel<HAS_VALUES, false, TWOUT, true, true, true>), dim3(tiles_ub), blk, 0, s, ws, L, sk, dk, sv,
                                   dv, ds, f32_out, xor_out, 0, pivot_result, pivot_f32_out, pivot_xor_out, pivot_result_v);
                hipLaunchKernelGGL((msb_scatter_kernel<HAS_VALUES, false, TWOUT, false, true, true>), rg, blk, 0, s, ws, L, sk, dk, sv, dv, ds,
                                   f32_out, xor_out, ra, pivot_result, pivot_f32_out, pivot_xor_out, pivot_result_v);
            } else {
                hipLaunchKernelGGL((msb_scatter_kernel<HAS_VALUES, false, TWOUT, true, false, true>), dim3(tiles_ub), blk, 0, s, ws, L, sk, dk, sv,
                                   dv, ds, f32_out, xor_out, 0, pivot_result, pivot_f32_out, pivot_xor_out, pivot_result_v);
                hipLaunchKernelGGL((msb_scatter_kernel<HAS_VALUES, false, TWOUT, false, false, true>), rg, blk, 0, s, ws, L, sk, dk, sv, dv, ds,
                                   f32_out, xor_out, ra, pivot_result, pivot_f32_out, pivot_xor_out, pivot_result_v);
            }
            if constexpr (HAS_VALUES) {
                if (pivot_result == sk)
                    hipLaunchKernelGGL(msb_pivot_copyback_kernel, dim3(tiles_ub), blk, 0, s, ws, L, (const uint32_t *)dv, pivot_result,
                                       pivot_result_v, pivot_f32_out, pivot_xor_out);
            }
            return;
        }
    }
    if (big) {
        hipLaunchKernelGGL((msb_scatter_kernel<HAS_VALUES, REMAP, TWOUT, true, true>), dim3(tiles_ub), blk, 0, s, ws, L, sk, dk, sv, dv,
                           ds, f32_out, xor_out, 0);
        hipLaunchKernelGGL((msb_scatter_kernel<HAS_VALUES, REMAP, TWOUT, false, true>), rg, blk, 0, s, ws, L, sk, dk, sv, dv, ds,
                           f32_out, xor_out, ra);
    } else {
        hipLaunchKernelGGL((msb_scatter_kernel<HAS_VALUES, REMAP, TWOUT, true, false>), dim3(tiles_ub), blk, 0, s, ws, L, sk, dk, sv, dv,
                           ds, f32_out, xor_out, 0);
        hipLaunchKernelGGL((msb_scatter_kernel<HAS_VALUES, REMAP, TWOUT, false, false>), rg, blk, 0, s, ws, L, sk, dk, sv, dv, ds,
                           f32_out, xor_out, ra);
    }
}

__host__ __device__ constexpr int local_b1(int cap) { return cap >= 16384 ? 14 : cap >= 8192 ? 13 : cap >= 4096 ? 12 : 11; }
template <int THREADS, int KPT, bool HAS_VALUES>
struct LocalSmem {
    static constexpr int WAVES = THREADS / WAVE;
    union {
        uint32_t stage[KPT * THREADS * (HAS_VALUES ? 2 : 1)];
        uint32_t hist[1 << (local_b1(KPT * THREADS * (HAS_VALUES ? 2 : 1)) > local_b1(KPT * THREADS) ? local_b1(KPT * THREADS * (HAS_VALUES ? 2 : 1)) : local_b1(KPT * THREADS))];
        uint32_t whist[WAVES][RADIX];
    };
    uint32_t wtot[16];
};

enum { LS_ALL = 0, LS_ONEPASS = 1, LS_FLAGGED = 2, LS_DEDUPE = 3, LS_DEDUPE_ALL = 4 };
constexpr uint32_t LS_FLAG = 0x80000000u;
constexpr uint32_t LS_DONE = 0x40000000u;
constexpr uint32_t DD_BITW = 4096;
constexpr uint32_t DD_MAX = 2048;
constexpr uint32_t DD_CNT = 4096;
__host__ __device__ constexpr bool ls_is_dedupe(int mode) { return mode == LS_DEDUPE || mode == LS_DEDUPE_ALL; }
constexpr uint32_t LS_DD = 0x20000000u;

__global__ __launch_bounds__(256) void msb_task_sample_kernel(MsbWs ws, int L, const uint32_t *__restrict__ src_k, int has_values)
{
    if (!(L < 3 && (ws.level[L + 1].packed >> 32) != 0ull)) return;
    const uint32_t lane = lane_id(), wv = (blockIdx.x * blockDim.x + threadIdx.x) >> 6, nwv = (gridDim.x * blockDim.x) >> 6;
    bool flagged = false;
    for (int cls = 0; cls < MSB_NCLASS; ++cls) {
        uint32_t ntasks = ws.level[L].task_count[cls];
        if (ntasks > ws.max_tasks) ntasks = ws.max_tasks;
        const int b1 = local_b1((int)ws.caps[cls]), onepass_bits = local_b1((int)ws.caps[cls] * (has_values ? 2 : 1)) + 2;
        for (uint32_t t = wv; t < ntasks; t += nwv) {
            const MsbTask c = ws.tasks[cls][t];
            if (c.sort_bits <= (uint32_t)b1 || c.sort_bits > 16u || c.size < 64u) continue;
            const uint32_t smp = src_k[c.offset + (uint32_t)(((unsigned long long)(c.size - 8u) * (2u * (lane >> 3) + 1u)) >> 4) + (lane & 7u)];
            unsigned long long same = ~0ull;
            for (uint32_t b = 0; b < c.sort_bits; ++b) {
                const bool bit = (smp >> b) & 1u;
                const unsigned long long m = __builtin_amdgcn_ballot_w64(bit);
                same &= bit ? m : ~m;
            }
            const int mult = __popcll(same);
            uint32_t add = 0;
            if (c.sort_bits <= (uint32_t)onepass_bits && __builtin_amdgcn_ballot_w64(mult >= 3) != 0ull) { add |= LS_FLAG; flagged = true; }
            if (__popcll(__builtin_amdgcn_ballot_w64(mult >= 2)) >= 4) add |= LS_DD;
            if (add && lane == 0) ws.tasks[cls][t].pad = c.pad | add;
        }
    }
    if (flagged && lane == 0) ws.level[L].flagged = 1u;
}
#ifdef GS_EXP_LS_PHASES
constexpr uint32_t LSP_TASKS = 65536;
__device__ uint32_t gs_ls_phase_buf[3 * MSB_NCLASS * LSP_TASKS * 16];
#define LSP_PLAN (MODE == LS_ONEPASS ? 0 : ls_is_dedupe(MODE) ? 2 : 1)
#define LSP(k)                                                                                                         \
    do {                                                                                                               \
        const unsigned long long now_ = __builtin_amdgcn_s_memtime();                                                  \
        if (tid == 0 && ti < LSP_TASKS) gs_ls_phase_buf[((LSP_PLAN * MSB_NCLASS + cls) * LSP_TASKS + ti) * 16 + (k)] += (uint32_t)(now_ - tprev_); \
        tprev_ = now_;                                                                                                 \
    } while (0)
#define LSP_WAIT(what) asm volatile("s_waitcnt " what ::: "memory")
#else
#define LSP(k) do { } while (0)
#define LSP_WAIT(what) do { } while (0)
#endif
template <int THREADS, int KPT, bool HAS_VALUES, bool STABLE = false, int MODE = LS_ALL, bool PLAIN = false>
#ifndef GS_LS_WPE_512x18
#define GS_LS_WPE_512x18 4
#endif
__global__ __launch_bounds__(THREADS, (THREADS == 1024 && !(HAS_VALUES && KPT > 9)) ? 8 : (THREADS == 512 && KPT == 18 && !HAS_VALUES) ? GS_LS_WPE_512x18 : 4) void msb_local_sort_kernel(
    MsbWs ws, int L, int cls, const uint32_t *__restrict__ src_k, uint32_t *__restrict__ dst_k, const uint32_t *__restrict__ src_v,
    uint32_t *__restrict__ dst_v, int f32_in, uint32_t xor_in, int f32_out, uint32_t xor_out)
{
    constexpr int WAVES = THREADS / WAVE;
    constexpr int LOCAL_B1 = local_b1(KPT * THREADS);
    constexpr int ONEPASS_BITS = local_b1(KPT * THREADS * (HAS_VALUES ? 2 : 1)) + 2;
    static_assert(KPT * THREADS >= (1 << LOCAL_B1) && KPT * THREADS >= WAVES * RADIX, "counters must fit the staging buffer");
    __shared__ __attribute__((aligned(16))) LocalSmem<THREADS, KPT, HAS_VALUES> sm;
    uint32_t ntasks = ws.level[L].task_count[cls];
    if (ntasks > ws.max_tasks) ntasks = ws.max_tasks;
    if ((MODE == LS_FLAGGED || MODE == LS_DEDUPE) && ws.level[L].flagged == 0u) return;
    const int tid = threadIdx.x, lane = lane_id(), w = wave_id();
    uint32_t *my = sm.whist[w];
    const uint32_t wbase0 = (uint32_t)w * (WAVE * KPT) + lane;
    auto fresh = [](uint32_t x) { asm volatile("" : "+v"(x)); return x; };
    static_assert(!(STABLE && MODE != LS_ALL), "the stable sort has one plan");
    auto advance = [&](uint32_t from, MsbTask &out) {
        uint32_t t = from;
        for (; t < ntasks; t += gridDim.x) {
            const MsbTask c = ws.tasks[cls][t];
            const bool mine = MODE == LS_ALL ? (STABLE || (c.pad & LS_DONE) == 0u)
                        : MODE == LS_ONEPASS ? (c.sort_bits > (uint32_t)LOCAL_B1 && c.sort_bits <= (uint32_t)ONEPASS_BITS && (c.pad & LS_FLAG) == 0u)
                        : MODE == LS_FLAGGED ? (c.pad & (LS_FLAG | LS_DONE)) == LS_FLAG
                        : ((c.pad & LS_DD) != 0u && (MODE == LS_DEDUPE_ALL || (c.pad & LS_FLAG) != 0u) && c.sort_bits > (uint32_t)LOCAL_B1 && c.sort_bits <= 16u);
            if (mine) {
                out.offset = __builtin_amdgcn_readfirstlane(c.offset);
                out.size = __builtin_amdgcn_readfirstlane(c.size);
                out.sort_bits = __builtin_amdgcn_readfirstlane(c.sort_bits);
                out.pad = __builtin_amdgcn_readfirstlane(c.pad);
                break;
            }
            if (MODE == LS_ONEPASS && tid == 0 && (c.pad & LS_FLAG) == 0u) { ws.tasks[cls][t].pad = c.pad | LS_FLAG; ws.level[L].flagged = 1u; }
        }
        return t;
    };
    MsbTask T{};
    uint32_t ti = advance(blockIdx.x, T);
    if (ti >= ntasks) return;
    uint32_t key[KPT], val[HAS_VALUES ? KPT : 1], pos[KPT];
    auto request = [&](const MsbTask &t) {
        const uint32_t *pk = src_k + t.offset, *pv = HAS_VALUES ? src_v + t.offset : nullptr;
        const uint32_t last = t.size - 1u;
        const uint32_t wbase = fresh(wbase0);
#pragma unroll
        for (int i = 0; i < KPT; ++i) {
            const uint32_t idx = wbase + i * WAVE;
            const uint32_t off = (idx < last ? idx : last) * 4u;
            key[i] = *reinterpret_cast<const uint32_t *>(reinterpret_cast<const char *>(pk) + off);
            if (HAS_VALUES) val[i] = *reinterpret_cast<const uint32_t *>(reinterpret_cast<const char *>(pv) + off);
        }
    };
    request(T);
    [[maybe_unused]] bool zeroed = false;
    for (;;) {
#ifdef GS_EXP_LS_PHASES
        unsigned long long tprev_ = __builtin_amdgcn_s_memtime();
        const unsigned long long t0_ = tprev_, r0_ = __builtin_amdgcn_s_memrealtime();
#endif
        MsbTask Tn = T;
        const uint32_t tn = advance(ti + gridDim.x, Tn);
        const bool has_next = tn < ntasks;
        LSP(0);
        LSP_WAIT("vmcnt(0)");
        LSP(1);
        {
            const uint32_t wbase = fresh(wbase0);
#pragma unroll
            for (int i = 0; i < KPT; ++i) {
                const uint32_t idx = wbase + i * WAVE;
                const uint32_t k = PLAIN ? key[i] : twiddle_in(key[i], f32_in, xor_in);
                key[i] = (idx < T.size) ? k : 0xffffffffu;
            }
        }
        const uint32_t B = T.sort_bits;
        bool done = false;
        if constexpr (MODE == LS_ONEPASS) {
            const uint32_t nwords = (1u << B) >> 2, maskB = (1u << B) - 1u, wmask = maskB & ~3u;
            if (!zeroed) {
                for (uint32_t j = tid; j < nwords; j += THREADS) sm.hist[j] = 0;
                __syncthreads();
            }
            zeroed = false;
            LSP(2);
            uint32_t overflow = 0;
            {
                const uint32_t wbase = fresh(wbase0);
                const uint32_t ba = key[0] & maskB, bb = key[KPT / 2] & maskB;
                const bool hot = __builtin_amdgcn_ballot_w64(ba == __builtin_amdgcn_readfirstlane(ba)) == __builtin_amdgcn_ballot_w64(true) ||
                                 __builtin_amdgcn_ballot_w64(bb == __builtin_amdgcn_readfirstlane(bb)) == __builtin_amdgcn_ballot_w64(true);
                if (hot) {
#pragma unroll
                for (int i = 0; i < KPT; ++i) {
                    pos[i] = 0;
                    if (wbase + i * WAVE < T.size) {
                        const uint32_t bin = key[i] & maskB, sh = (bin & 3u) * 8u;
                        const unsigned long long act = __builtin_amdgcn_ballot_w64(true);
                        const uint32_t b0 = __builtin_amdgcn_readfirstlane(bin);
                        uint32_t r;
                        if (__builtin_amdgcn_ballot_w64(bin == b0) == act) {
                            const uint32_t lower = count_lower_mask(act), cnt = (uint32_t)__popcll(act);
                            uint32_t old = 0;
                            if (lower == 0) old = atomicAdd(&sm.hist[b0 >> 2], cnt << sh);
                            old = (__builtin_amdgcn_readfirstlane(old) >> sh) & 255u;
                            r = old + lower;
                            overflow |= (old + cnt > 255u) ? 1u : 0u;
                        } else {
                            r = (atomicAdd(&sm.hist[bin >> 2], 1u << sh) >> sh) & 255u;
                            overflow |= (r >= 255u) ? 1u : 0u;
                        }
                        pos[i] = r;
                    }
                }
                } else {
                    uint32_t rmax = 0;
#pragma unroll
                    for (int i = 0; i < KPT; ++i) {
                        const uint32_t sh = (key[i] & 3u) << 3;
                        const uint32_t inc = (wbase + i * WAVE < T.size) ? (1u << sh) : 0u;
                        const uint32_t old = atomicAdd(reinterpret_cast<uint32_t *>(reinterpret_cast<char *>(sm.hist) + (key[i] & wmask)), inc);
                        pos[i] = __builtin_amdgcn_ubfe(old, sh, 8u);
                        rmax = pos[i] > rmax ? pos[i] : rmax;
                    }
                    overflow = (rmax >= 255u) ? 1u : 0u;
                }
            }
            LSP_WAIT("lgkmcnt(0)");
            LSP(3);
            const int ovf_ = __syncthreads_or((int)overflow);
            LSP(4);
            if (!ovf_) {
                constexpr uint32_t WPT = ((1u << ONEPASS_BITS) >> 2) / THREADS;
                static_assert(WPT >= 4 && WPT % 4 == 0, "words per thread");
                static_assert(KPT * THREADS <= 65536, "a word's base must fit 16 bits");
                uint32_t rk[(KPT + 3) / 4];
#pragma unroll
                for (int j = 0; j < (KPT + 3) / 4; ++j) {
                    rk[j] = pos[4 * j];
                    if (4 * j + 1 < KPT) rk[j] |= pos[4 * j + 1] << 8;
                    if (4 * j + 2 < KPT) rk[j] |= pos[4 * j + 2] << 16;
                    if (4 * j + 3 < KPT) rk[j] |= pos[4 * j + 3] << 24;
                }
#pragma unroll
                for (int j = 0; j < (KPT + 3) / 4; ++j) asm volatile("" : "+v"(rk[j]));
#pragma unroll
                for (int i = 0; i < KPT; ++i) asm volatile("" : "+v"(key[i]));
                const bool act = (uint32_t)tid * WPT < nwords;
                uint32_t ssum = 0;
                if (act) {
#pragma unroll
                    for (uint32_t q = 0; q < WPT; q += 4) {
                        const uint4 c4 = reinterpret_cast<const uint4 *>(sm.hist)[((uint32_t)tid * WPT + q) >> 2];
                        ssum = __builtin_amdgcn_sad_u8(c4.x, 0u, ssum); ssum = __builtin_amdgcn_sad_u8(c4.y, 0u, ssum);
                        ssum = __builtin_amdgcn_sad_u8(c4.z, 0u, ssum); ssum = __builtin_amdgcn_sad_u8(c4.w, 0u, ssum);
                    }
                }
                const uint32_t inc = wave_inclusive_scan(ssum);
                if (lane == 63) sm.wtot[w] = inc;
                LSP(5);
                __syncthreads();
                LSP(6);
                const uint32_t wsv = (lane < WAVES) ? sm.wtot[lane] : 0u;
                const uint32_t wincl = wave_inclusive_scan(wsv);
                uint32_t run = (uint32_t)__shfl((int)(wincl - wsv), w, WAVE) + inc - ssum;
                uint32_t wide = 0;
                auto pack = [&](uint32_t c) {
                    wide |= c & 0xf0f0f0f0u;
                    const uint32_t nib = (c & 0xfu) | ((c >> 4) & 0xf0u) | ((c >> 8) & 0xf00u) | ((c >> 12) & 0xf000u);
                    const uint32_t e = run | (nib << 16);
                    run = __builtin_amdgcn_sad_u8(c, 0u, run);
                    return e;
                };
                if (act) {
#pragma unroll
                    for (uint32_t q = 0; q < WPT; q += 4) {
                        uint4 *p4 = reinterpret_cast<uint4 *>(sm.hist) + (((uint32_t)tid * WPT + q) >> 2);
                        const uint4 c4 = *p4;
                        uint4 e4;
                        e4.x = pack(c4.x); e4.y = pack(c4.y); e4.z = pack(c4.z); e4.w = pack(c4.w);
                        *p4 = e4;
                    }
                }
                LSP_WAIT("lgkmcnt(0)");
                LSP(7);
                const int wide_ = __syncthreads_or((int)(wide != 0u));
                LSP(8);
                if (!wide_) {
#pragma unroll
                for (int i = 0; i < KPT; ++i) {
                    const uint32_t wd = *reinterpret_cast<const uint32_t *>(reinterpret_cast<const char *>(sm.hist) + (key[i] & wmask));
                    const uint32_t low = __builtin_amdgcn_ubfe(wd >> 16, 0u, (key[i] & 3u) << 2);
                    pos[i] = ((rk[i >> 2] >> (8 * (i & 3))) & 255u) + (wd & 0xffffu) + (low & 0xfu) + ((low >> 4) & 0xfu) + (low >> 8);
                }
#pragma unroll
                for (int i = 0; i < KPT; ++i) asm volatile("" : "+v"(pos[i]));
                LSP(9);
                __syncthreads();
                LSP(10);
                {
                    const uint32_t wbase = fresh(wbase0);
#pragma unroll
                    for (int i = 0; i < KPT; ++i) {
                        const uint32_t idx = wbase + i * WAVE;
                        const uint32_t at = idx < T.size ? pos[i] : idx;
                        if (HAS_VALUES) reinterpret_cast<uint2 *>(sm.stage)[at] = make_uint2(key[i], val[i]);
                        else sm.stage[at] = key[i];
                    }
                }
                LSP_WAIT("lgkmcnt(0)");
                LSP(11);
                __syncthreads();
                LSP(12);
                done = true;
                }
            }
        }
        if constexpr (ls_is_dedupe(MODE)) {
            static_assert((uint32_t)(KPT * THREADS * (HAS_VALUES ? 2 : 1)) >= DD_BITW + DD_CNT, "the map and the counters are overlaid on the staging buffer");
            static_assert(DD_BITW % THREADS == 0 && DD_CNT % (4 * THREADS) == 0 && KPT * THREADS <= 65536 && DD_MAX * 2 <= DD_CNT, "dedupe geometry");
            const uint32_t maskB = (1u << B) - 1u;
            uint32_t *const bitw = sm.stage, *const cnt = sm.stage + DD_BITW;
            if (!zeroed) {
                for (uint32_t j = tid; j < DD_BITW + DD_CNT; j += THREADS) sm.stage[j] = 0;
                __syncthreads();
            }
            zeroed = false;
            LSP(2);
            {
                const uint32_t wbase = fresh(wbase0);
#pragma unroll
                for (int i = 0; i < KPT; ++i) {
                    if (wbase + i * WAVE < T.size) {
                        const uint32_t v = key[i] & maskB, bit = 1u << (v & 15u);
                        if (!(bitw[v >> 4] & bit)) atomicOr(&bitw[v >> 4], bit);
                    }
                }
            }
            LSP_WAIT("lgkmcnt(0)");
            LSP(3);
            __syncthreads();
            LSP(4);
            constexpr uint32_t WPT = DD_BITW / THREADS;
            static_assert(WPT % 4 == 0, "map words per thread");
            uint32_t ssum = 0;
#pragma unroll
            for (uint32_t q = 0; q < WPT; q += 4) {
                const uint4 c4 = reinterpret_cast<const uint4 *>(bitw)[((uint32_t)tid * WPT + q) >> 2];
                ssum += (uint32_t)(__popc(c4.x) + __popc(c4.y) + __popc(c4.z) + __popc(c4.w));
            }
            uint32_t inc = wave_inclusive_scan(ssum);
            if (lane == 63) sm.wtot[w] = inc;
            __syncthreads();
            uint32_t wsv = (lane < WAVES) ? sm.wtot[lane] : 0u;
            uint32_t wincl = wave_inclusive_scan(wsv);
            uint32_t run = (uint32_t)__shfl((int)(wincl - wsv), w, WAVE) + inc - ssum;
            const uint32_t distinct = (uint32_t)__shfl((int)wincl, WAVES - 1, WAVE);
            LSP(5);
            if (distinct <= DD_MAX) {
#pragma unroll
                for (uint32_t q = 0; q < WPT; q += 4) {
                    uint4 *p4 = reinterpret_cast<uint4 *>(bitw) + (((uint32_t)tid * WPT + q) >> 2);
                    uint4 c4 = *p4;
                    const uint32_t px = run, py = px + (uint32_t)__popc(c4.x), pz = py + (uint32_t)__popc(c4.y), pw = pz + (uint32_t)__popc(c4.z);
                    run = pw + (uint32_t)__popc(c4.w);
                    c4.x |= px << 16; c4.y |= py << 16; c4.z |= pz << 16; c4.w |= pw << 16;
                    *p4 = c4;
                }
                __syncthreads();
                LSP(6);
                const uint32_t rs = distinct <= 256u ? 4u : distinct <= 512u ? 3u : distinct <= 1024u ? 2u : 1u;
                const uint32_t rep = (uint32_t)lane & ((1u << rs) - 1u);
                {
                    const uint32_t wbase = fresh(wbase0);
#pragma unroll
                    for (int i = 0; i < KPT; ++i) {
                        pos[i] = 0;
                        if (wbase + i * WAVE < T.size) {
                            const uint32_t v = key[i] & maskB, wd = bitw[v >> 4];
                            const uint32_t id = (((wd >> 16) + (uint32_t)__popc(wd & ((1u << (v & 15u)) - 1u))) << rs) | rep;
#ifdef GS_EXP_DD_NOCONTEND
                            pos[i] = atomicAdd(&cnt[(id + (uint32_t)lane * 31u) & (DD_CNT - 1u)], 1u) | (id << 16);
#else
                            pos[i] = atomicAdd(&cnt[id], 1u) | (id << 16);
#endif
                        }
                    }
                }
#pragma unroll
                for (int i = 0; i < KPT; ++i) asm volatile("" : "+v"(pos[i]), "+v"(key[i]));
                LSP_WAIT("lgkmcnt(0)");
                LSP(7);
                __syncthreads();
                LSP(8);
                constexpr uint32_t CPT = DD_CNT / THREADS;
                uint32_t csum = 0;
#pragma unroll
                for (uint32_t q = 0; q < CPT; q += 4) {
                    const uint4 c4 = reinterpret_cast<const uint4 *>(cnt)[((uint32_t)tid * CPT + q) >> 2];
                    csum += c4.x + c4.y + c4.z + c4.w;
                }
                inc = wave_inclusive_scan(csum);
                if (lane == 63) sm.wtot[w] = inc;
                __syncthreads();
                wsv = (lane < WAVES) ? sm.wtot[lane] : 0u;
                wincl = wave_inclusive_scan(wsv);
                run = (uint32_t)__shfl((int)(wincl - wsv), w, WAVE) + inc - csum;
#pragma unroll
                for (uint32_t q = 0; q < CPT; q += 4) {
                    uint4 *p4 = reinterpret_cast<uint4 *>(cnt) + (((uint32_t)tid * CPT + q) >> 2);
                    const uint4 c4 = *p4;
                    uint4 e4;
                    e4.x = run; e4.y = e4.x + c4.x; e4.z = e4.y + c4.y; e4.w = e4.z + c4.z;
                    run = e4.w + c4.w;
                    *p4 = e4;
                }
                __syncthreads();
                LSP(9);
#pragma unroll
                for (int i = 0; i < KPT; ++i) pos[i] = cnt[pos[i] >> 16] + (pos[i] & 0xffffu);
#pragma unroll
                for (int i = 0; i < KPT; ++i) asm volatile("" : "+v"(pos[i]));
                LSP(10);
                __syncthreads();
                {
                    const uint32_t wbase = fresh(wbase0);
#pragma unroll
                    for (int i = 0; i < KPT; ++i) {
                        const uint32_t idx = wbase + i * WAVE;
                        const uint32_t at = idx < T.size ? pos[i] : idx;
                        if (HAS_VALUES) reinterpret_cast<uint2 *>(sm.stage)[at] = make_uint2(key[i], val[i]);
                        else sm.stage[at] = key[i];
                    }
                }
                LSP_WAIT("lgkmcnt(0)");
                LSP(11);
                __syncthreads();
                LSP(12);
                done = true;
            } else {
                __syncthreads();
            }
        }
        if constexpr (MODE == LS_ONEPASS) {
            if (!done && tid == 0) { ws.tasks[cls][ti].pad = T.pad | LS_FLAG; ws.level[L].flagged = 1u; }
        } else if constexpr (ls_is_dedupe(MODE)) {
            if (done && tid == 0) ws.tasks[cls][ti].pad = T.pad | LS_DONE;
        } else {
        done = true;
        const uint32_t b1 = STABLE ? 0u : (B < (uint32_t)LOCAL_B1 ? B : (uint32_t)LOCAL_B1);
        bool in_regs = STABLE;
        if (!STABLE) {
            const uint32_t nbins = 1u << b1, mask1 = nbins - 1u;
            for (uint32_t j = tid; j < nbins; j += THREADS) sm.hist[j] = 0;
            __syncthreads();
            LSP(2);
            {
                const uint32_t wbase = fresh(wbase0);
#pragma unroll
                for (int i = 0; i < KPT; ++i) {
                    pos[i] = 0;
                    if (wbase + i * WAVE < T.size) {
                        const uint32_t d = key[i] & mask1;
                        const unsigned long long act = __builtin_amdgcn_ballot_w64(true);
                        const uint32_t d0 = __builtin_amdgcn_readfirstlane(d);
                        if (__builtin_amdgcn_ballot_w64(d == d0) == act) {
                            const uint32_t lower = count_lower_mask(act);
                            uint32_t base = 0;
                            if (lower == 0) base = atomicAdd(&sm.hist[d0], (uint32_t)__popcll(act));
                            pos[i] = __builtin_amdgcn_readfirstlane(base) + lower;
                        } else {
                            pos[i] = atomicAdd(&sm.hist[d], 1u);
                        }
                    }
                }
            }
#pragma unroll
            for (int i = 0; i < KPT; ++i) asm volatile("" : "+v"(pos[i]), "+v"(key[i]));
            LSP_WAIT("lgkmcnt(0)");
            LSP(3);
            __syncthreads();
            LSP(4);
            constexpr uint32_t IPT = (1u << LOCAL_B1) / THREADS;
            const bool act = (uint32_t)tid * IPT < nbins;
            uint32_t ssum = 0;
            if (act) {
#pragma unroll
                for (uint32_t q = 0; q < IPT; q += 4) {
                    const uint4 c4 = reinterpret_cast<const uint4 *>(sm.hist)[((uint32_t)tid * IPT + q) >> 2];
                    ssum += c4.x + c4.y + c4.z + c4.w;
                }
            }
            const uint32_t inc = wave_inclusive_scan(ssum);
            if (lane == 63) sm.wtot[w] = inc;
            __syncthreads();
            const uint32_t wsv = (lane < WAVES) ? sm.wtot[lane] : 0u;
            const uint32_t wincl = wave_inclusive_scan(wsv);
            uint32_t run = (uint32_t)__shfl((int)(wincl - wsv), w, WAVE) + inc - ssum;
            if (act) {
#pragma unroll
                for (uint32_t q = 0; q < IPT; q += 4) {
                    uint4 *p4 = reinterpret_cast<uint4 *>(sm.hist) + (((uint32_t)tid * IPT + q) >> 2);
                    const uint4 c4 = *p4;
                    uint4 e4;
                    e4.x = run; e4.y = e4.x + c4.x; e4.z = e4.y + c4.y; e4.w = e4.z + c4.z;
                    run = e4.w + c4.w;
                    *p4 = e4;
                }
            }
            LSP_WAIT("lgkmcnt(0)");
            LSP(5);
            __syncthreads();
            LSP(6);
#pragma unroll
            for (int i = 0; i < KPT; ++i) pos[i] += sm.hist[key[i] & mask1];
#pragma unroll
            for (int i = 0; i < KPT; ++i) asm volatile("" : "+v"(pos[i]));
            LSP(7);
            __syncthreads();
            LSP(8);
            {
                const uint32_t wbase = fresh(wbase0);
#pragma unroll
                for (int i = 0; i < KPT; ++i) {
                    if (wbase + i * WAVE < T.size) {
                        if (HAS_VALUES) reinterpret_cast<uint2 *>(sm.stage)[pos[i]] = make_uint2(key[i], val[i]);
                        else sm.stage[pos[i]] = key[i];
                    }
                }
            }
            LSP_WAIT("lgkmcnt(0)");
            LSP(9);
            __syncthreads();
            LSP(10);
        }
        uint32_t rem = B - b1, np = (rem + 7u) / 8u, shift = b1 + (STABLE ? T.pad : 0u);
        while (rem) {
            const uint32_t b = (rem + np - 1u) / np, nd = 1u << b;
            const uint32_t wbase = fresh(wbase0);
            if (!in_regs) {
#pragma unroll
            for (int i = 0; i < KPT; ++i) {
                const uint32_t idx = wbase + i * WAVE;
                if (HAS_VALUES) {
                    const uint2 kv = reinterpret_cast<const uint2 *>(sm.stage)[idx];
                    key[i] = kv.x; val[i] = kv.y;
                } else {
                    key[i] = sm.stage[idx];
                }
                if (idx >= T.size) key[i] = 0xffffffffu;
            }
            __syncthreads();
            }
            in_regs = false;
#pragma unroll
            for (int i = lane; i < RADIX; i += WAVE) my[i] = 0;
            auto rank_pass = [&](auto width) {
                uint32_t d_prev = 0, plo = 0, phi = 0;
#pragma unroll
                for (int i = 0; i <= KPT; ++i) {
                    uint32_t d_cur = 0, clo = 0, chi = 0;
                    if (i < KPT) {
                        d_cur = __builtin_amdgcn_ubfe(key[i], shift, b);
                        constexpr int MB = decltype(width)::value;
                        if (MB == 2) match_digit2(d_cur, clo, chi);
                        else if (MB == 4) match_digit4(d_cur, clo, chi);
                        else if (MB == 5) match_digit5(d_cur, clo, chi);
                        else match_digit(d_cur, clo, chi);
                    }
                    if (i > 0) {
                        const uint32_t lower = count_lower(plo, phi);
                        pos[i - 1] = my[d_prev] + lower;
                        if (lower == 0)
                            __hip_atomic_fetch_add(&my[d_prev], (uint32_t)(__popc(plo) + __popc(phi)), __ATOMIC_RELAXED,
                                                   __HIP_MEMORY_SCOPE_WAVEFRONT);
                    }
                    d_prev = d_cur; plo = clo; phi = chi;
                }
            };
            if (b <= 2u) rank_pass(std::integral_constant<int, 2>{});
            else if (b <= 4u) rank_pass(std::integral_constant<int, 4>{});
            else if (b <= 5u) rank_pass(std::integral_constant<int, 5>{});
            else rank_pass(std::integral_constant<int, 8>{});
#pragma unroll
            for (int i = 0; i < KPT; ++i) asm volatile("" : "+v"(pos[i]), "+v"(key[i]));
            __syncthreads();
            uint32_t tot = 0, inc = 0;
            if ((uint32_t)tid < nd) {
#pragma unroll
                for (int j = 0; j < WAVES; ++j) {
                    const uint32_t c = sm.whist[j][tid];
                    sm.whist[j][tid] = tot;
                    tot += c;
                }
            }
            if (tid < RADIX) {
                inc = wave_inclusive_scan(tot);
                if (lane == 63) sm.wtot[w] = inc;
            }
            __syncthreads();
            if ((uint32_t)tid < nd) {
                uint32_t ex = inc - tot;
                if (w > 0) ex += sm.wtot[0];
                if (w > 1) ex += sm.wtot[1];
                if (w > 2) ex += sm.wtot[2];
#pragma unroll
                for (int j = 0; j < WAVES; ++j) sm.whist[j][tid] += ex;
            }
            __syncthreads();
#pragma unroll
            for (int i = 0; i < KPT; ++i) pos[i] += my[__builtin_amdgcn_ubfe(key[i], shift, b)];
#pragma unroll
            for (int i = 0; i < KPT; ++i) asm volatile("" : "+v"(pos[i]));
            __syncthreads();
#pragma unroll
            for (int i = 0; i < KPT; ++i) {
                if (HAS_VALUES) reinterpret_cast<uint2 *>(sm.stage)[pos[i]] = make_uint2(key[i], val[i]);
                else sm.stage[pos[i]] = key[i];
            }
            __syncthreads();
            shift += b; rem -= b; --np;
        }
        LSP(11);
        }
        if (has_next) request(Tn);
        LSP(13);
        constexpr uint32_t CAP = (uint32_t)(KPT * THREADS);
        const uint32_t ssh = (T.size + (T.offset & 63u) <= CAP) ? (T.offset & 63u) : 0u;
        if (done) {
        uint32_t *qk = dst_k + T.offset, *qv = HAS_VALUES ? dst_v + T.offset : nullptr;
        if (HAS_VALUES) {
            for (uint32_t jj = tid; jj < T.size + ssh; jj += THREADS) {
                const uint32_t j = jj - ssh;
                if (j >= T.size) continue;
                const uint2 kv = reinterpret_cast<const uint2 *>(sm.stage)[j];
                __builtin_nontemporal_store(PLAIN ? kv.x : twiddle_out(kv.x, f32_out, xor_out), &qk[j]);
                __builtin_nontemporal_store(kv.y, &qv[j]);
            }
        } else {
            const uint32_t t0 = fresh((uint32_t)tid);
            const uint32_t jb = t0 - ssh, s0 = jb < CAP ? jb : jb + CAP;
            pos[0] = sm.stage[s0];
#pragma unroll
            for (int i = 1; i < KPT; ++i) pos[i] = sm.stage[jb + i * THREADS];
            if constexpr ((MODE == LS_ONEPASS || ls_is_dedupe(MODE)) && !HAS_VALUES) {
#pragma unroll
                for (int i = 1; i < KPT; ++i) sm.stage[jb + i * THREADS] = 0;
                sm.stage[s0] = 0;
                zeroed = true;
            }
#pragma unroll
            for (int i = 0; i < KPT; ++i) {
                const uint32_t j = jb + i * THREADS;
                if (j < T.size) __builtin_nontemporal_store(PLAIN ? pos[i] : twiddle_out(pos[i], f32_out, xor_out), reinterpret_cast<uint32_t *>(reinterpret_cast<char *>(qk) + j * 4u));
            }
        }
        }
        LSP(14);
        __syncthreads();
#ifdef GS_EXP_LS_PHASES
        if (tid == 0 && ti < LSP_TASKS) {
            gs_ls_phase_buf[((LSP_PLAN * MSB_NCLASS + cls) * LSP_TASKS + ti) * 16 + 15] += (uint32_t)(__builtin_amdgcn_s_memtime() - t0_);
            (void)r0_;
        }
#endif
        if (!has_next) break;
        T = Tn; ti = tn;
    }
}


template <bool VEC>
__global__ __launch_bounds__(MSB_THREADS) void shard_hist_kernel(const uint32_t *__restrict__ keys, uint64_t n, int bits,
                                                                 unsigned long long *__restrict__ hist, int f32_in,
                                                                 uint32_t xor_in)
{
    __shared__ uint32_t lh[1 << SHARD_MAX_BITS];
    const uint32_t nb = 1u << bits;
    for (uint32_t i = threadIdx.x; i < nb; i += MSB_THREADS) lh[i] = 0;
    __syncthreads();
    const int rshift = 32 - bits;
    auto count = [&](uint32_t k) { atomicAdd(&lh[twiddle_in(k, f32_in, xor_in) >> rshift], 1u); };
    const uint64_t stride = (uint64_t)gridDim.x * MSB_THREADS;
    uint64_t done = 0;
    if (VEC) {
        const uint4 *k4 = reinterpret_cast<const uint4 *>(keys);
        const uint64_t nvec = n >> 2;
        uint64_t v = (uint64_t)blockIdx.x * MSB_THREADS + threadIdx.x;
        for (; v + 3 * stride < nvec; v += 4 * stride) {
            const uint4 a = k4[v], b = k4[v + stride], c = k4[v + 2 * stride], d = k4[v + 3 * stride];
            count(a.x); count(a.y); count(a.z); count(a.w);
            count(b.x); count(b.y); count(b.z); count(b.w);
            count(c.x); count(c.y); count(c.z); count(c.w);
            count(d.x); count(d.y); count(d.z); count(d.w);
        }
        for (; v < nvec; v += stride) { const uint4 a = k4[v]; count(a.x); count(a.y); count(a.z); count(a.w); }
        done = nvec << 2;
    }
    for (uint64_t i = done + (uint64_t)blockIdx.x * MSB_THREADS + threadIdx.x; i < n; i += stride) count(keys[i]);
    __syncthreads();
    for (uint32_t i = threadIdx.x; i < nb; i += MSB_THREADS)
        if (lh[i]) atomicAdd(&hist[i], (unsigned long long)lh[i]);
}

__global__ void shard_counts_kernel(const uint32_t *__restrict__ row, uint32_t n, int num_ranks, unsigned long long *__restrict__ counts)
{
    const int r = threadIdx.x;
    if (r < num_ranks) counts[r] = (unsigned long long)((r + 1 < RADIX ? row[r + 1] : n) - row[r]);
}


static inline bool onepass_possible(int min_bits, int b1, int onepass_bits)
{
    return (min_bits > b1 && min_bits <= onepass_bits) || (min_bits + 8 > b1 && min_bits + 8 <= onepass_bits);
}
template <bool HAS_VALUES, bool STABLE = false>
static void launch_local_sorts(const MsbWs &ws, int L, uint32_t bound, const uint32_t *sk, uint32_t *dk, const uint32_t *sv,
                               uint32_t *dv, int f32_in, uint32_t xor_in, int f32_out, uint32_t xor_out, hipStream_t s,
                               int min_bits = 0, uint64_t num_items = 0, const uint32_t *known_tasks = nullptr, bool maybe_skew = true)
{
    KernelTimer kt(GS_K_MSB_LOCAL_SORT, s);
    auto grid_of = [&](int c) {
        uint64_t b = bound;
        if (known_tasks && known_tasks[c] < b) b = known_tasks[c];
        if (num_items && c > 0) {
            const uint64_t lim = num_items / msb_class_cap(c - 1) + RADIX;
            if (lim < b) b = lim;
        }
#ifndef MSB_LS_MAX_GRID
#define MSB_LS_MAX_GRID MSB_MAX_GRID
#endif
        return (uint32_t)(b < MSB_LS_MAX_GRID ? (b ? b : 1) : MSB_LS_MAX_GRID);
    };
#define GS_LS1P(C, HV, M, P) hipLaunchKernelGGL((msb_local_sort_kernel<msb_class_threads(C), msb_class_kpt(C), HV, STABLE, M, P>), dim3(grid_of(C)), \
                                               dim3(msb_class_threads(C)), 0, s, ws, L, C, sk, dk, sv, dv, f32_in, xor_in, f32_out, xor_out)
#define GS_LS1(C, HV, M) GS_LS1P(C, HV, M, false)
#define GS_LSDD(C, HV, M) hipLaunchKernelGGL((msb_local_sort_kernel<msb_class_threads(C), msb_class_kpt(C), HV, STABLE, M, false>),                \
                                             dim3(grid_of(C)), dim3(msb_class_threads(C)), 0, s, ws, L, C, sk, dk, sv, dv,                             \
                                             f32_in, xor_in, f32_out, xor_out)
    const bool plain = !f32_in && !xor_in && !f32_out && !xor_out;
    static const bool dedupe_on = [] { const char *e = getenv("GS_MSB_DEDUPE"); return !(e && e[0] == '0'); }();
#define GS_LS(C, HV)                                                                                                  \
    do {                                                                                                              \
        constexpr bool DD = !STABLE && msb_class_cap(C) * (HV ? 2u : 1u) >= DD_BITW + DD_CNT;                           \
        const bool dd = DD && dedupe_on && maybe_skew && L < 3 && onepass_possible(min_bits, local_b1((int)msb_class_cap(C)), 16);          \
        if constexpr (STABLE) { GS_LS1(C, HV, LS_ALL); }                                                              \
        else if (!onepass_possible(min_bits, local_b1((int)msb_class_cap(C)), local_b1((int)msb_class_cap(C) * (HV ? 2 : 1)) + 2)) \
            { if constexpr (DD) { if (dd) GS_LSDD(C, HV, LS_DEDUPE_ALL); } GS_LS1(C, HV, LS_ALL); }                    \
        else { if (plain) GS_LS1P(C, HV, LS_ONEPASS, true); else GS_LS1(C, HV, LS_ONEPASS);                           \
               if constexpr (DD) { if (dd) GS_LSDD(C, HV, LS_DEDUPE); } GS_LS1(C, HV, LS_FLAGGED); }                   \
    } while (0)
    auto wanted = [&](int c) { return !known_tasks || known_tasks[c] != 0u; };
    if constexpr (!STABLE) {
        uint64_t waves = bound;
        if (known_tasks) waves = (uint64_t)known_tasks[0] + known_tasks[1] + known_tasks[2] + known_tasks[3];
        if (L < 3 && waves && maybe_skew) {
            const uint32_t blocks = (uint32_t)(waves / 4 + 1 < 2048 ? waves / 4 + 1 : 2048);
            hipLaunchKernelGGL(msb_task_sample_kernel, dim3(blocks), dim3(256), 0, s, ws, L, sk, HAS_VALUES ? 1 : 0);
        }
    }
    if (wanted(0)) GS_LS(0, HAS_VALUES);
    if (wanted(1)) GS_LS(1, HAS_VALUES);
    if (wanted(2)) GS_LS(2, HAS_VALUES);
    if ((!HAS_VALUES || GS_PAIR_CLASSES > 3) && wanted(3)) GS_LS(3, HAS_VALUES);
#undef GS_LS
#undef GS_LS1
#undef GS_LS1P
#undef GS_LSDD
}

int msb_local_sorts_in_place(MsbLevel *level, MsbTask *const tasks[MSB_NCLASS], uint32_t max_tasks, uint32_t bound, uint32_t *keys,
                             int sort_bits, uint64_t num_items, int f32_out, uint32_t xor_out, hipStream_t s, const uint32_t *known_tasks)
{
    MsbWs ws{};
    ws.level = level;
    for (int c = 0; c < MSB_NCLASS; ++c) { ws.tasks[c] = tasks[c]; ws.caps[c] = msb_class_cap(c); }
    ws.max_tasks = max_tasks;
    ws.tile_shift = 13u;
    ws.key_bits = 32u;
    launch_local_sorts<false>(ws, 0, bound, keys, keys, nullptr, nullptr, 0, 0u, f32_out, xor_out, s, sort_bits, num_items, known_tasks);
    return (int)hipGetLastError();
}

static inline bool msb_pivot_enabled()
{
    static const bool on = [] { const char *e = getenv("GS_MSB_PIVOT"); return !(e && e[0] == '0'); }();
    return on;
}

__global__ void msb_peek_kernel(MsbWs ws, int L, unsigned long long *mailbox)
{
    mailbox[0] = ws.level[L].packed;
    mailbox[1] = ((unsigned long long)ws.level[L - 1].task_count[1] << 32) | ws.level[L - 1].task_count[0];
    mailbox[2] = ((unsigned long long)ws.level[L - 1].task_count[3] << 32) | ws.level[L - 1].task_count[2];
    __threadfence_system();
}
struct MsbPeek {
    unsigned long long *host = nullptr, *dev = nullptr;
    hipEvent_t ev = nullptr;
    int device = -1;
    bool armed = false;
};
static bool msb_peek_enabled()
{
    static const bool on = [] { const char *e = getenv("GS_MSB_PEEK"); return !(e && e[0] == '0'); }();
    return on;
}
constexpr int MSB_PEEK_DEVICES = 16;
struct MsbPeekTable {
    MsbPeek slot[MSB_PEEK_DEVICES];
    ~MsbPeekTable()
    {
        for (MsbPeek &pk : slot) {
            if (pk.ev) (void)hipEventDestroy(pk.ev);
            if (pk.host) (void)hipHostFree(pk.host);
        }
    }
};
static MsbPeek *msb_peek_get(hipStream_t s)
{
    if (!msb_peek_enabled()) return nullptr;
    hipStreamCaptureStatus cs = hipStreamCaptureStatusNone;
    if (hipStreamIsCapturing(s, &cs) != hipSuccess || cs != hipStreamCaptureStatusNone) { (void)hipGetLastError(); return nullptr; }
    thread_local MsbPeekTable table;
    int dev = -1;
    if (hipGetDevice(&dev) != hipSuccess || dev < 0 || dev >= MSB_PEEK_DEVICES) { (void)hipGetLastError(); return nullptr; }
    MsbPeek &pk = table.slot[dev];
    if (pk.device != dev) {
        void *h = nullptr, *d = nullptr;
        if (hipHostMalloc(&h, 64, hipHostMallocMapped | hipHostMallocPortable) != hipSuccess ||
            hipHostGetDevicePointer(&d, h, 0) != hipSuccess ||
            hipEventCreateWithFlags(&pk.ev, hipEventDisableTiming) != hipSuccess) {
            (void)hipGetLastError();
            if (h) (void)hipHostFree(h);
            pk.ev = nullptr;
            return nullptr;
        }
        pk.host = (unsigned long long *)h; pk.dev = (unsigned long long *)d; pk.device = dev;
    }
    if (pk.armed) { (void)hipEventSynchronize(pk.ev); (void)hipGetLastError(); }
    pk.armed = false;
    return &pk;
}

static void msb_peek_arm(MsbPeek *pk, const MsbWs &ws, int L, hipStream_t s)
{
    if (!pk) return;
    hipLaunchKernelGGL(msb_peek_kernel, dim3(1), dim3(1), 0, s, ws, L, pk->dev);
    pk->armed = hipEventRecord(pk->ev, s) == hipSuccess;
    if (!pk->armed) (void)hipGetLastError();
}
struct MsbLook { bool ok = false; uint32_t buckets = 0, tiles = 0, tasks[MSB_NCLASS] = {0, 0, 0, 0}; };
static MsbLook msb_peek_wait(MsbPeek *pk)
{
    MsbLook lk;
    if (!pk || !pk->armed) return lk;
    pk->armed = false;
    if (hipEventSynchronize(pk->ev) != hipSuccess) { (void)hipGetLastError(); return lk; }
    const volatile unsigned long long *m = pk->host;
    const unsigned long long a = m[0], b = m[1], c = m[2];
    lk.ok = true;
    lk.buckets = (uint32_t)(a >> 32); lk.tiles = (uint32_t)a;
    lk.tasks[0] = (uint32_t)b; lk.tasks[1] = (uint32_t)(b >> 32); lk.tasks[2] = (uint32_t)c; lk.tasks[3] = (uint32_t)(c >> 32);
    return lk;
}

static void msb_run_levels(const MsbWs &ws, uint64_t num_items, bool pairs, uint32_t npieces, uint32_t *const buf_k[2],
                           uint32_t *const buf_v[2], const PassParams &tw, hipStream_t s, int stop_level = 99,
                           bool allow_pivot = true)
{
    const int nclass = msb_num_classes(pairs);
    const uint32_t tiles_all = (uint32_t)((num_items + MSB_TILE - 1) / MSB_TILE);
    const uint32_t max_tasks_lvl = ws.max_tasks;
    uint32_t *d_keys = buf_k[0], *d_vals = buf_v[0];
    MsbPeek *peek = (stop_level == 99 && (npieces == 0 || getenv("GS_MSB_PEEK_FINISH"))) ? msb_peek_get(s) : nullptr;
    uint32_t known_b = 0, known_tiles = 0;
    bool known = false;
    for (int L = 1; L <= 3; ++L) {
        const int shift = 24 - 8 * L;
        const DigitSel dsel{shift, nullptr, 0, 0, 0u, 8, 0};
        uint32_t *sk = buf_k[L & 1], *dk = buf_k[(L + 1) & 1];
        uint32_t *sv = buf_v[L & 1], *dv = buf_v[(L + 1) & 1];
        const bool in_pieces = npieces != 0 && L == 1;
        const bool pivot = allow_pivot && msb_pivot_enabled() && !in_pieces && L <= 2;
        uint32_t max_b = (L == 1) ? (uint32_t)RADIX : ws.max_buckets;
        uint32_t max_tiles = tiles_all + (in_pieces ? 2u * npieces : max_b + tiles_all / MSB_ALIGN_MIN_TILES + 1u);
        if (known && L >= 2) {
            if (known_b < max_b) max_b = known_b;
            if (known_tiles < max_tiles) max_tiles = known_tiles;
            known = false;
        }
        const bool last = (L == 3);
        { KernelTimer kt(GS_K_MSB_HISTOGRAM, s);
          if (in_pieces) {
              hipLaunchKernelGGL(msb_expand_pieces_kernel, dim3(npieces < 4096u ? npieces : 4096u), dim3(256), 0, s, ws, npieces);
          } else {
              const uint32_t eg = max_b < 4096u ? max_b : 4096u;
              hipLaunchKernelGGL(msb_expand_kernel, dim3(eg), dim3(256), 0, s, ws, L, pivot ? (const uint32_t *)sk : (const uint32_t *)nullptr);
          }
          const uint32_t hg_ub = max_tiles / MSB_WAVES + 1;
          const uint32_t hg = hg_ub < MSB_MAX_GRID ? hg_ub : MSB_MAX_GRID;
          if (pivot) hipLaunchKernelGGL((msb_upsweep_kernel<false, true>), dim3(hg), dim3(MSB_THREADS), 0, s, ws, L, (const uint32_t *)sk, dsel);
          else hipLaunchKernelGGL((msb_upsweep_kernel<false, false>), dim3(hg), dim3(MSB_THREADS), 0, s, ws, L, (const uint32_t *)sk, dsel);
          hipLaunchKernelGGL(msb_scan_kernel, dim3(RADIX), dim3(1024), 0, s, ws, L); }
        { KernelTimer kt(GS_K_MSB_CLASSIFY, s);
          const uint32_t cg = max_b < 4096u ? max_b : 4096u;
          if (last) hipLaunchKernelGGL((msb_classify_kernel<true, false>), dim3(cg), dim3(256), 0, s, ws, L, (const uint32_t *)nullptr, nclass);
          else if (pivot) hipLaunchKernelGGL((msb_classify_kernel<false, true>), dim3(cg), dim3(256), 0, s, ws, L, (const uint32_t *)nullptr, nclass);
          else hipLaunchKernelGGL((msb_classify_kernel<false, false>), dim3(cg), dim3(256), 0, s, ws, L, (const uint32_t *)nullptr, nclass); }
        if (L == stop_level) return;
        if (!last) msb_peek_arm(peek, ws, L + 1, s);
        { KernelTimer kt(GS_K_MSB_PARTITION, s);
          const bool big = num_items > (1ull << 30);
          const uint32_t *svc = pairs ? (const uint32_t *)sv : (const uint32_t *)nullptr;
          uint32_t *dvc = pairs ? dv : (uint32_t *)nullptr;
#define GS_SC(HV, TW) launch_scatter<HV, false, TW>(ws, L, max_tiles, max_b, big, (const uint32_t *)sk, dk, svc, dvc, dsel, tw.f32_out, tw.xor_out, s, in_pieces, \
                                                  pivot ? d_keys : (uint32_t *)nullptr, tw.f32_out, tw.xor_out, pivot && pairs ? d_vals : (uint32_t *)nullptr)
          if (pairs) { if (last) GS_SC(true, true); else GS_SC(true, false); }
          else { if (last) GS_SC(false, true); else GS_SC(false, false); }
#undef GS_SC
        }
        if (!last) {
            const MsbLook lk = msb_peek_wait(peek);
            const uint32_t tb = (uint64_t)max_b * RADIX < (uint64_t)max_tasks_lvl ? max_b * (uint32_t)RADIX : max_tasks_lvl;
            const uint32_t *kt_ = lk.ok ? lk.tasks : nullptr;
            const bool skew = !(lk.ok && lk.buckets == 0);
            if (pairs) launch_local_sorts<true>(ws, L, tb, dk, d_keys, dv, d_vals, 0, 0u, tw.f32_out, tw.xor_out, s, 24 - 8 * L, num_items, kt_, skew);
            else launch_local_sorts<false>(ws, L, tb, dk, d_keys, nullptr, nullptr, 0, 0u, tw.f32_out, tw.xor_out, s, 24 - 8 * L, num_items, kt_, skew);
            if (lk.ok) {
                if (lk.buckets == 0) return;
                known = true; known_b = lk.buckets; known_tiles = lk.tiles;
            }
        }
    }
}

__global__ void msb_small_task_kernel(MsbLevel *level, MsbTask *task, uint32_t n, int cls, uint32_t bits, uint32_t shift0)
{
    if (threadIdx.x == 0) {
        MsbLevel z{};
        z.task_count[cls] = 1;
        level[0] = z;
        task[0] = MsbTask{0u, n, bits, shift0};
    }
}

uint32_t small_sort_capacity(bool pairs) { return msb_class_cap(msb_num_classes(pairs) - 1); }

int small_stable_sort(void *scratch, size_t scratch_bytes, const uint32_t *kin, uint32_t *kout, const uint32_t *vin, uint32_t *vout,
                      uint32_t n, int begin_bit, int end_bit, int f32_in, uint32_t xor_in, int f32_out, uint32_t xor_out,
                      hipStream_t s)
{
    const bool pairs = vin != nullptr;
    if (n == 0 || n > small_sort_capacity(pairs) || scratch_bytes < 256 + sizeof(MsbTask)) return hipErrorInvalidValue;
    int cls = 0;
    while (msb_class_cap(cls) < n) ++cls;
    MsbWs ws{};
    ws.level = (MsbLevel *)scratch;
    for (int c = 0; c < MSB_NCLASS; ++c) ws.tasks[c] = (MsbTask *)((char *)scratch + 256);
    ws.max_tasks = 1;
    KernelTimer kt(GS_K_MSB_LOCAL_SORT, s);
    hipLaunchKernelGGL(msb_small_task_kernel, dim3(1), dim3(64), 0, s, ws.level, ws.tasks[cls], n, cls,
                       (uint32_t)(end_bit - begin_bit), (uint32_t)begin_bit);
#define GS_SM(C, HV) hipLaunchKernelGGL((msb_local_sort_kernel<msb_class_threads(C), msb_class_kpt(C), HV, true, LS_ALL>), dim3(1), \
                                        dim3(msb_class_threads(C)), 0, s, ws, 0, C, kin, kout, vin, vout, f32_in, xor_in, f32_out, xor_out)
    if (pairs) { if (cls == 0) GS_SM(0, true); else if (cls == 1) GS_SM(1, true); else if (cls == 2 || GS_PAIR_CLASSES < 4) GS_SM(2, true); else GS_SM(3, true); }
    else { if (cls == 0) GS_SM(0, false); else if (cls == 1) GS_SM(1, false); else if (cls == 2) GS_SM(2, false); else GS_SM(3, false); }
#undef GS_SM
    return (int)hipGetLastError();
}


constexpr uint32_t SEG_TINY = 256;
__global__ __launch_bounds__(256) void seg_classify_kernel(MsbWs ws, const int *__restrict__ seg_begin,
                                                           const int *__restrict__ seg_end, uint32_t nseg, int nclass,
                                                           uint32_t sort_bits, uint32_t shift0, uint32_t num_items,
                                                           uint32_t tiny_cap = 0)
{
    constexpr int NW = 4, SPT = 4, NLIST = NW + MSB_NCLASS;
    __shared__ uint32_t s_cnt[NLIST], s_base[NLIST];
    const uint32_t cap_max = ws.caps[nclass - 1];
    const int tid = threadIdx.x;
    for (uint32_t base = blockIdx.x * (256u * SPT); base < nseg; base += gridDim.x * (256u * SPT)) {
        if (tid < NLIST) s_cnt[tid] = 0;
        __syncthreads();
        uint32_t b[SPT], size[SPT], off[NLIST], cnt[NLIST];
        int list[SPT];
#pragma unroll
        for (int q = 0; q < NLIST; ++q) cnt[q] = 0;
#pragma unroll
        for (int j = 0; j < SPT; ++j) {
            const uint32_t sg = base + (uint32_t)tid * SPT + j;
            b[j] = 0; size[j] = 0; list[j] = -1;
            if (sg < nseg) {
                int lo = seg_begin[sg], hi = seg_end[sg];
                if (lo < 0) lo = 0;
                if (hi > (int)num_items) hi = (int)num_items;
                if (hi > lo) { b[j] = (uint32_t)lo; size[j] = (uint32_t)(hi - lo); }
            }
            const uint32_t sz = size[j];
            if (sz != 0 && tiny_cap != 0 && sz <= 4u * tiny_cap) list[j] = sz <= (uint32_t)WAVE ? 3 : sz <= tiny_cap ? 0 : sz <= 2u * tiny_cap ? 1 : 2;
            else if (sz != 0 && sz <= cap_max) { int c = 0; while (ws.caps[c] < sz) ++c; list[j] = NW + c; }
            else if (sz > cap_max) {
                const uint32_t tiles = ws_tiles_of_at(ws, b[j], sz);
                const unsigned long long old = atomicAdd(&ws.level[1].packed, (1ull << 32) | tiles);
                if ((uint32_t)(old >> 32) < ws.max_buckets) ws.buckets[1][(uint32_t)(old >> 32)] = MsbBucket{b[j], sz, (uint32_t)old, tiles};
                else MSB_OVERFLOW(ws);
            }
#pragma unroll
            for (int q = 0; q < NLIST; ++q) cnt[q] += list[j] == q ? 1u : 0u;
        }
#pragma unroll
        for (int q = 0; q < NLIST; ++q) off[q] = cnt[q] ? atomicAdd(&s_cnt[q], cnt[q]) : 0u;
        __syncthreads();
        if (tid < NLIST && s_cnt[tid] != 0u)
            s_base[tid] = atomicAdd(tid < NW ? &ws.level[2].task_count[tid] : &ws.level[1].task_count[tid - NW], s_cnt[tid]);
        __syncthreads();
#pragma unroll
        for (int j = 0; j < SPT; ++j) {
#pragma unroll
            for (int q = 0; q < NLIST; ++q) {
                if (list[j] != q) continue;
                const uint32_t at = s_base[q] + off[q]++;
                if (at < ws.max_tasks) {
                    if (q < NW) ws.tasks[q][ws.max_tasks - 1u - at] = MsbTask{b[j], size[j], sort_bits, shift0};
                    else ws.tasks[q - NW][at] = MsbTask{b[j], size[j], sort_bits, shift0};
                } else {
                    MSB_OVERFLOW(ws);
                }
            }
        }
        __syncthreads();
    }
}


template <bool HAS_VALUES, int WKPT >
__global__ __launch_bounds__(256) void seg_wave_sort_kernel(MsbWs ws, const uint32_t *__restrict__ src_k, uint32_t *__restrict__ dst_k,
                                                            const uint32_t *__restrict__ src_v, uint32_t *__restrict__ dst_v, int f32_in,
                                                            uint32_t xor_in, int f32_out, uint32_t xor_out)
{
    typedef uint32_t K;
    constexpr int FW = 0;
#include "gs_seg_wave_body.inc"
}

template <bool HAS_VALUES>
__global__ __launch_bounds__(256) void seg_wave4_sort_kernel(MsbWs ws, const uint32_t *__restrict__ src_k, uint32_t *__restrict__ dst_k,
                                                             const uint32_t *__restrict__ src_v, uint32_t *__restrict__ dst_v, int f32_in,
                                                             uint32_t xor_in, int f32_out, uint32_t xor_out)
{
    typedef uint32_t K;
    constexpr int FW = 0;
#include "gs_seg_wave4_body.inc"
}

template <bool HAS_VALUES, int WKPT, typename K, int FW>
__global__ __launch_bounds__(256) void seg_wave_sort_narrow_kernel(MsbWs ws, const K *__restrict__ src_k, K *__restrict__ dst_k,
                                                                   const uint32_t *__restrict__ src_v, uint32_t *__restrict__ dst_v, int f32_in,
                                                                   uint32_t xor_in, int f32_out, uint32_t xor_out)
{
#include "gs_seg_wave_body.inc"
}
template <bool HAS_VALUES, typename K, int FW>
__global__ __launch_bounds__(256) void seg_wave4_sort_narrow_kernel(MsbWs ws, const K *__restrict__ src_k, K *__restrict__ dst_k,
                                                                    const uint32_t *__restrict__ src_v, uint32_t *__restrict__ dst_v, int f32_in,
                                                                    uint32_t xor_in, int f32_out, uint32_t xor_out)
{
#include "gs_seg_wave4_body.inc"
}

constexpr int MW_THREADS = 512, MW_WAVES = MW_THREADS / WAVE, MW_KPT = 8, MW_TILE = MW_THREADS * MW_KPT;
constexpr uint32_t MW_CAP = 8192;
struct MwNoVal {};

template <typename K> __device__ __forceinline__ K mw_tw_in(K k, int f, uint64_t x)
{
    if constexpr (sizeof(K) == 8) { if (f) k ^= (uint64_t)((int64_t)k >> 63) | 0x8000000000000000ull; return k ^ x; }
    else return twiddle_in((uint32_t)k, f, (uint32_t)x);
}
template <typename K> __device__ __forceinline__ K mw_tw_out(K k, int f, uint64_t x)
{
    if constexpr (sizeof(K) == 8) { k ^= x; if (f) k ^= ~(uint64_t)((int64_t)k >> 63) | 0x8000000000000000ull; return k; }
// ... 1205 lines not shown
```

### gpu-sort_amd/csrc/gs_msb_tasks.hpp

```cpp
#pragma once

#include "gs_host.hpp"

namespace gs {

constexpr int MSB_NCLASS = 4;
#ifndef GS_LS3_THREADS
#define GS_LS3_THREADS 1024
#define GS_LS3_KPT 17
#endif
#ifndef GS_LS2_THREADS
#define GS_LS2_THREADS 512
#define GS_LS2_KPT 18
#endif
#ifndef GS_LS1_THREADS
#define GS_LS1_THREADS 512
#define GS_LS1_KPT 9
#endif
#ifndef GS_LS0_THREADS
#define GS_LS0_THREADS 512
#define GS_LS0_KPT 4
#endif
__host__ __device__ constexpr int msb_class_threads(int c) { return c == 0 ? GS_LS0_THREADS : c == 1 ? GS_LS1_THREADS : c == 2 ? GS_LS2_THREADS : GS_LS3_THREADS; }
__host__ __device__ constexpr int msb_class_kpt(int c) { return c == 0 ? GS_LS0_KPT : c == 1 ? GS_LS1_KPT : c == 2 ? GS_LS2_KPT : GS_LS3_KPT; }
__host__ __device__ constexpr uint32_t msb_class_cap(int c) { return (uint32_t)(msb_class_kpt(c) * msb_class_threads(c)); }
struct MsbTask { uint32_t offset, size, sort_bits, pad; };
struct MsbLevel {
    unsigned long long packed;
    uint32_t task_count[MSB_NCLASS];
    uint32_t flagged;
    uint32_t overflow;
    unsigned long long unused1;
    unsigned long long keys;
    unsigned long long unused2;
    uint32_t census_blocks, pad;
};

int msb_local_sorts_in_place(MsbLevel *level, MsbTask *const tasks[MSB_NCLASS], uint32_t max_tasks, uint32_t bound, uint32_t *keys,
                             int sort_bits, uint64_t num_items, int f32_out, uint32_t xor_out, hipStream_t s,
                             const uint32_t *known_tasks = nullptr);

}
```

### include/gpusort.h

```cpp
#ifndef GPUSORT_H_
#define GPUSORT_H_

#include <stddef.h>
#include <stdint.h>

#ifdef __cplusplus
extern "C" {
#endif

#define GS_VERSION 100

enum gs_key_type {
    GS_KEY_U32 = 0,
    GS_KEY_I32 = 1,
    GS_KEY_F32 = 2,
    GS_KEY_U64 = 3,
    GS_KEY_I64 = 4,
    GS_KEY_F64 = 5,
    GS_KEY_U8 = 6,
    GS_KEY_I8 = 7,
    GS_KEY_U16 = 8,
    GS_KEY_I16 = 9,
    GS_KEY_F16 = 10,
    GS_KEY_BF16 = 11,
    GS_KEY_F8 = 12
};

int         gs_version(void);
const char *gs_error_string(int err);


size_t gs_lsb_temp_bytes(uint64_t num_items, int has_values);

int gs_lsb_sort_u32(void *d_temp, size_t temp_bytes,
                    uint32_t *d_keys[2], uint32_t *d_vals[2], int *selector,
                    uint64_t num_items, int begin_bit, int end_bit,
                    int descending, int key_type, void *stream);

size_t gs_lsb_copy_temp_bytes(uint64_t num_items, int has_values);
int gs_lsb_sort_copy_u32(void *d_temp, size_t temp_bytes,
                         const uint32_t *d_keys_in, uint32_t *d_keys_out,
                         const uint32_t *d_vals_in, uint32_t *d_vals_out,
                         uint64_t num_items, int begin_bit, int end_bit,
                         int descending, int key_type, void *stream);

size_t gs_lsb_wide_temp_bytes(uint64_t num_items, int key_bytes, int val_bytes);
int gs_lsb_sort_wide(void *d_temp, size_t temp_bytes, void *d_keys[2], void *d_vals[2],
                     int *selector, uint64_t num_items, int key_bytes, int val_bytes,
                     int begin_bit, int end_bit, int descending, int key_type, void *stream);

void gs_lsb_geometry(uint64_t num_items, int has_values, uint32_t *grid, uint32_t *tile,
                     uint32_t *tiles_per_chunk);
int  gs_lsb_workspace_layout(void *d_temp, uint64_t num_items, uint32_t **d_spine,
                             uint32_t **d_totals, uint16_t **d_prefix16);
int  gs_lsb_pipe_status(void *d_temp, uint64_t num_items, uint32_t *h_status, void *stream);
int  gs_lsb_plan_status(void *d_temp, uint64_t num_items, uint32_t out[8], void *stream);
int  gs_lsb_plan_cursor_status(void *d_temp, uint64_t num_items, uint32_t out[4], void *stream);
int  gs_lsb_plan_peek_status(uint32_t out[4]);
int  gs_lsb_plan_look_only(void *d_temp, const void *d_keys, void *d_alt, uint64_t num_items,
                           int key_type, int descending, void *stream);
int  gs_lsb_plan_layout(uint64_t num_items, uint64_t out[4]);
int  gs_lsb_upsweep_u32(void *d_temp, size_t temp_bytes, const uint32_t *d_keys_in,
                        uint64_t num_items, int shift, int bits, int descending,
                        int key_type_in, void *stream);
int  gs_lsb_scan_spine(void *d_temp, size_t temp_bytes, uint64_t num_items, void *stream);
int  gs_lsb_downsweep_u32(void *d_temp, size_t temp_bytes,
                          const uint32_t *d_keys_in, uint32_t *d_keys_out,
                          const uint32_t *d_vals_in, uint32_t *d_vals_out,
                          uint64_t num_items, int shift, int bits, int descending,
                          int key_type_in, int key_type_out, void *stream);

size_t gs_lsb_any_temp_bytes(uint64_t num_items, int key_type, int val_bytes);
int gs_lsb_sort_any(void *d_temp, size_t temp_bytes, const void *d_keys_in, void *d_keys_out,
                    const void *d_vals_in, void *d_vals_out, uint64_t num_items, int key_type, int val_bytes,
                    int begin_bit, int end_bit, int descending, void *stream);

size_t gs_lsb_narrow_temp_bytes(uint64_t num_items, int key_type, int val_bytes);
int gs_lsb_sort_narrow(void *d_temp, size_t temp_bytes, const void *d_keys_in, void *d_keys_out,
                       const void *d_vals_in, void *d_vals_out, uint64_t num_items, int key_type, int val_bytes,
                       int begin_bit, int end_bit, int descending, void *stream);
uint32_t gs_lsb_narrow_tile(int key_type, int val_bytes);


size_t gs_msb_temp_bytes(uint64_t num_items, int has_values);

int gs_msb_sort_u32(void *d_temp, size_t temp_bytes,
                    uint32_t *d_keys, uint32_t *d_vals, uint64_t num_items,
                    uint32_t *d_keys_alt, uint32_t *d_vals_alt,
                    uint32_t **d_sorted_keys, uint32_t **d_sorted_vals,
                    int key_type, void *stream, int synchronize);

size_t gs_msb_wide_temp_bytes(uint64_t num_items, int key_bytes, int val_bytes);
int gs_msb_sort_wide(void *d_temp, size_t temp_bytes, void *d_keys, void *d_vals, uint64_t num_items,
                     void *d_keys_alt, void *d_vals_alt, int key_bytes, int val_bytes,
                     void **d_sorted_keys, void **d_sorted_vals, int key_type, void *stream, int synchronize);

size_t gs_msb_large_temp_bytes(uint64_t num_items, int has_values);
int    gs_msb_sort_large_u32(void *d_temp, size_t temp_bytes,
                             uint32_t *d_keys, uint32_t *d_vals, uint64_t num_items,
                             uint32_t *d_keys_alt, uint32_t *d_vals_alt,
                             int key_type, void *stream, int synchronize);

size_t gs_msb_large_wide_temp_bytes(uint64_t num_items, int key_bytes, int val_bytes);
int    gs_msb_sort_large_wide(void *d_temp, size_t temp_bytes, void *d_keys, void *d_vals, uint64_t num_items,
                              void *d_keys_alt, void *d_vals_alt, int key_bytes, int val_bytes, int key_type,
                              void *stream, int synchronize);

size_t gs_lsb_large_temp_bytes(uint64_t num_items, int key_bytes, int val_bytes);
int    gs_lsb_sort_large(void *d_temp, size_t temp_bytes, void *d_keys[2], void *d_vals[2], int *selector,
                         uint64_t num_items, int key_bytes, int val_bytes, int begin_bit, int end_bit,
                         int descending, int key_type, void *stream);

size_t gs_lsb_narrow_large_temp_bytes(uint64_t num_items, int key_type, int val_bytes);
int    gs_lsb_sort_narrow_large(void *d_temp, size_t temp_bytes, const void *d_keys_in, void *d_keys_out,
                                const void *d_vals_in, void *d_vals_out, uint64_t num_items, int key_type,
                                int val_bytes, int begin_bit, int end_bit, int descending, void *stream);

size_t gs_topk_temp_bytes(uint64_t num_items, uint64_t k, int has_values);
int    gs_topk_u32(void *d_temp, size_t temp_bytes,
                   const uint32_t *d_keys_in, const uint32_t *d_vals_in,
                   uint32_t *d_keys_out, uint32_t *d_vals_out,
                   uint64_t num_items, uint64_t k, int descending, int key_type, void *stream);
int    gs_topk_status(void *d_temp, uint64_t num_items, uint64_t k, int has_values, uint32_t out[8], void *stream);

size_t gs_topk_u16_temp_bytes(uint64_t num_items, uint64_t k, int has_values);
int    gs_topk_u16(void *d_temp, size_t temp_bytes,
                   const uint16_t *d_keys_in, const uint32_t *d_vals_in,
                   uint16_t *d_keys_out, uint32_t *d_vals_out,
                   uint64_t num_items, uint64_t k, int descending, int key_type, void *stream);
int    gs_topk_u16_status(void *d_temp, uint64_t num_items, uint64_t k, int has_values, uint32_t out[8], void *stream);

size_t gs_topk_u64_temp_bytes(uint64_t num_items, uint64_t k, int has_values);
int    gs_topk_u64(void *d_temp, size_t temp_bytes,
                   const uint64_t *d_keys_in, const uint32_t *d_vals_in,
                   uint64_t *d_keys_out, uint32_t *d_vals_out,
                   uint64_t num_items, uint64_t k, int descending, int key_type, void *stream);
int    gs_topk_u64_status(void *d_temp, uint64_t num_items, uint64_t k, int has_values, uint32_t out[8], void *stream);

size_t   gs_topk_rows_temp_bytes(uint64_t num_rows, uint64_t num_cols, uint64_t k, int has_values);
int      gs_topk_rows_u32(void *d_temp, size_t temp_bytes,
                          const uint32_t *d_keys_in, const uint32_t *d_vals_in,
                          uint32_t *d_keys_out, uint32_t *d_vals_out,
                          uint64_t num_rows, uint64_t num_cols, uint64_t row_stride, uint64_t k,
                          int descending, int key_type, void *stream);
uint32_t gs_topk_rows_max_k(void);
int      gs_topk_rows_plan(uint64_t num_rows, uint64_t num_cols, uint64_t k, int has_values, uint32_t out[8]);

size_t   gs_topk_rows_u16_temp_bytes(uint64_t num_rows, uint64_t num_cols, uint64_t k, int has_values);
int      gs_topk_rows_u16(void *d_temp, size_t temp_bytes,
                          const uint16_t *d_keys_in, const uint32_t *d_vals_in,
                          uint16_t *d_keys_out, uint32_t *d_vals_out,
                          uint64_t num_rows, uint64_t num_cols, uint64_t row_stride, uint64_t k,
                          int descending, int key_type, void *stream);

size_t   gs_topk_rows_u64_temp_bytes(uint64_t num_rows, uint64_t num_cols, uint64_t k, int has_values);
int      gs_topk_rows_u64(void *d_temp, size_t temp_bytes,
                          const uint64_t *d_keys_in, const uint32_t *d_vals_in,
                          uint64_t *d_keys_out, uint32_t *d_vals_out,
                          uint64_t num_rows, uint64_t num_cols, uint64_t row_stride, uint64_t k,
                          int descending, int key_type, void *stream);

size_t gs_topk_segmented_temp_bytes(uint64_t num_items, uint32_t num_segments, uint64_t k, int has_values);
int    gs_topk_segmented_u32(void *d_temp, size_t temp_bytes,
                             const uint32_t *d_keys_in, const uint32_t *d_vals_in,
                             uint32_t *d_keys_out, uint32_t *d_vals_out, uint32_t *d_counts_out,
                             uint64_t num_items, uint32_t num_segments,
                             const int32_t *d_begin_offsets, const int32_t *d_end_offsets,
                             uint64_t k, int descending, int key_type, void *stream);
int    gs_topk_segmented_plan(uint64_t num_items, uint32_t num_segments, uint64_t k, int has_values, uint32_t out[8]);
int    gs_topk_segmented_status(void *d_temp, uint64_t num_items, uint32_t num_segments, uint64_t k, int has_values,
                                uint32_t out[8], void *stream);

size_t gs_topk_segmented_u16_temp_bytes(uint64_t num_items, uint32_t num_segments, uint64_t k, int has_values);
int    gs_topk_segmented_u16(void *d_temp, size_t temp_bytes,
                             const uint16_t *d_keys_in, const uint32_t *d_vals_in,
                             uint16_t *d_keys_out, uint32_t *d_vals_out, uint32_t *d_counts_out,
                             uint64_t num_items, uint32_t num_segments,
                             const int32_t *d_begin_offsets, const int32_t *d_end_offsets,
                             uint64_t k, int descending, int key_type, void *stream);

size_t gs_topk_segmented_u64_temp_bytes(uint64_t num_items, uint32_t num_segments, uint64_t k, int has_values);
int    gs_topk_segmented_u64(void *d_temp, size_t temp_bytes,
                             const uint64_t *d_keys_in, const uint32_t *d_vals_in,
                             uint64_t *d_keys_out, uint32_t *d_vals_out, uint32_t *d_counts_out,
                             uint64_t num_items, uint32_t num_segments,
                             const int32_t *d_begin_offsets, const int32_t *d_end_offsets,
                             uint64_t k, int descending, int key_type, void *stream);

typedef struct gs_msb_level_census {
    uint64_t buckets;
    uint64_t tiles;
    uint64_t keys;
    uint64_t pivot_buckets;
    uint64_t pivot_keys;
    uint64_t task_keys;
    uint32_t tasks[4];
    uint32_t flagged;
    uint32_t overflow;
} gs_msb_level_census;
int gs_msb_census(void *d_temp, uint64_t num_items, int has_values, gs_msb_level_census out[4], void *stream);
int gs_msb_wide_census(void *d_temp, uint64_t num_items, int key_bytes, int val_bytes, gs_msb_level_census out[8], void *stream);
void gs_msb_capacities(uint64_t num_items, int has_values, uint32_t *max_buckets, uint32_t *max_tasks, uint32_t *max_tiles);

int gs_msb_classify_upto(void *d_temp, size_t temp_bytes, uint32_t *d_keys, uint32_t *d_keys_alt, uint64_t num_items,
                         int stop_level, int flags, void *stream);
int gs_msb_read_lists(void *d_temp, uint64_t num_items, int has_values, int level,
                      uint32_t *h_buckets, uint32_t max_buckets, uint32_t *n_buckets,
                      uint32_t *h_tasks[4], uint32_t max_tasks, uint32_t n_tasks[4], void *stream);


size_t gs_segmented_temp_bytes(uint64_t num_items, int has_values, uint32_t num_segments);
int gs_segmented_sort_u32(void *d_temp, size_t temp_bytes, uint32_t *d_keys[2], uint32_t *d_vals[2],
                          int *selector, uint64_t num_items, uint32_t num_segments,
                          const int32_t *d_begin_offsets, const int32_t *d_end_offsets, int begin_bit,
                          int end_bit, int descending, int key_type, void *stream);

size_t gs_segmented_wide_temp_bytes(uint64_t num_items, int key_bytes, int val_bytes, uint32_t num_segments);
int gs_segmented_sort_wide(void *d_temp, size_t temp_bytes, void *d_keys[2], void *d_vals[2], int *selector,
                           uint64_t num_items, uint32_t num_segments, const int32_t *d_begin_offsets,
                           const int32_t *d_end_offsets, int key_bytes, int val_bytes, int begin_bit, int end_bit,
                           int descending, int key_type, void *stream);

size_t gs_segmented_narrow_temp_bytes(uint64_t num_items, int key_type, int val_bytes, uint32_t num_segments);
int gs_segmented_sort_narrow(void *d_temp, size_t temp_bytes, void *d_keys[2], void *d_vals[2], int *selector,
                             uint64_t num_items, uint32_t num_segments, const int32_t *d_begin_offsets,
                             const int32_t *d_end_offsets, int key_type, int val_bytes, int begin_bit, int end_bit,
                             int descending, void *stream);
uint32_t gs_segmented_narrow_cap(int key_type, int val_bytes);

int gs_msb_first_pass_u32(void *d_temp, size_t temp_bytes, const uint32_t *d_keys_in,
                          uint32_t *d_keys_out, const uint32_t *d_vals_in, uint32_t *d_vals_out,
                          uint64_t num_items, int key_type, uint64_t *d_bucket_counts, void *stream);
size_t gs_msb_finish_temp_bytes(uint64_t num_items, int has_values, int num_src);
int gs_msb_finish_u32(void *d_temp, size_t temp_bytes, uint32_t *d_keys, uint32_t *d_vals,
                      uint32_t *d_keys_out, uint32_t *d_vals_out, uint64_t num_items,
                      const uint64_t *h_piece_counts, int num_src, int key_type, void *stream,
                      int synchronize);

int gs_shard_histogram_u32(const uint32_t *d_keys, uint64_t num_items, int bits,
                           uint64_t *d_hist, int key_type, void *stream);
int gs_shard_partition_u32(void *d_temp, size_t temp_bytes,
                           const uint32_t *d_keys_in, uint32_t *d_keys_out,
                           const uint32_t *d_vals_in, uint32_t *d_vals_out,
                           uint64_t num_items, int bits, const uint8_t *d_dest_of_bin,
                           int num_ranks, const uint64_t *d_bin_hist, uint64_t *d_counts,
                           int key_type, void *stream);

enum gs_gen_kind { GS_GEN_UNIFORM = 0, GS_GEN_ZIPF = 1, GS_GEN_ENTROPY_AND = 2, GS_GEN_ENUMERATED = 3 };
int gs_generate_u32(uint32_t *d_out, uint64_t num_items, int kind, uint64_t seed,
                    uint64_t start_index, int level, void *stream);

int gs_check_sorted_u32(const uint32_t *d_keys, uint64_t num_items, int descending,
                        uint64_t *d_result, void *stream);
int gs_check_pairs_enumerated_u32(const uint32_t *d_keys_in, const uint32_t *d_keys_sorted,
                                  const uint32_t *d_vals, uint64_t num_items,
                                  uint64_t *d_result, void *stream);
int gs_check_sorted_u64(const uint64_t *d_keys, uint64_t num_items, int key_type, uint64_t *d_result, void *stream);
int gs_check_pairs_enumerated_wide(const void *d_keys_in, const void *d_keys_sorted, const uint64_t *d_vals,
                                   uint64_t num_items, int key_bytes, uint64_t *d_result, void *stream);
int gs_check_sorted_stable(const void *d_keys_sorted, const uint64_t *d_rowids, uint64_t num_items, int key_bytes,
                           int key_type, int begin_bit, int end_bit, int descending, uint64_t *d_result, void *stream);

enum gs_kernel_id {
    GS_K_LSB_UPSWEEP = 0, GS_K_LSB_SCAN = 1, GS_K_LSB_DOWNSWEEP = 2,
    GS_K_MSB_HISTOGRAM = 3, GS_K_MSB_CLASSIFY = 4, GS_K_MSB_PARTITION = 5, GS_K_MSB_LOCAL_SORT = 6,
    GS_K_SHARD = 7, GS_K_OTHER = 8,
    GS_K_LSB_PASS = 9,
    GS_K_COUNT = 10
};
typedef struct gs_profile gs_profile;
gs_profile *gs_profile_create(void);
void        gs_profile_destroy(gs_profile *p);
void        gs_profile_begin(gs_profile *p);
void        gs_profile_end(void);
int         gs_profile_read(gs_profile *p, double total_ms[GS_K_COUNT], uint64_t launches[GS_K_COUNT]);
const char *gs_kernel_name(int kernel_id);

#ifdef __cplusplus
}
#endif
#endif
```

Before: 161.6 Gkeys/s.

## Rework planned LSB sort: rank-free cursor scatter, fused peek, capped leftover sorts

Several changes to the planned LSB path. The separate upsweep is replaced with a small cursor-init kernel, and the scatter now uses a cursor kernel that can rank keys with wave-scope LDS atomics in any order. The irregular-tile fix-up kernel is rewritten to aggregate atomics through shared-memory edge counters. The plan peek mailbox is written directly by the decide kernel, which removes one launch. The flagged and dedupe local-sort passes scan tasks a wave at a time and launch with a capped grid. Together these aim to cut kernel launches, global atomic traffic and idle workgroups, at the cost of nondeterministic ordering within digits and more complex code.

```diff
diff --git a/gpu-sort_amd/_lib.py b/gpu-sort_amd/_lib.py
--- a/gpu-sort_amd/_lib.py
+++ b/gpu-sort_amd/_lib.py
@@ -36,6 +36,7 @@
     "gs_lsb_plan_status": (i32, [vp, u64, C.POINTER(C.c_uint32), vp]),
     "gs_lsb_plan_cursor_status": (i32, [vp, u64, C.POINTER(C.c_uint32), vp]),
     "gs_lsb_plan_peek_status": (i32, [C.POINTER(C.c_uint32)]),
+    "gs_lsb_plan_finish_cap": (C.c_uint32, []),
     "gs_lsb_plan_look_only": (i32, [vp, vp, vp, u64, i32, i32, vp]),
     "gs_lsb_plan_layout": (i32, [u64, C.POINTER(C.c_uint64)]),
     "gs_lsb_upsweep_u32": (i32, [vp, sz, vp, u64, i32, i32, i32, i32, vp]),
diff --git a/gpu-sort_amd/csrc/gs_lsb_downsweep.inc b/gpu-sort_amd/csrc/gs_lsb_downsweep.inc
--- a/gpu-sort_amd/csrc/gs_lsb_downsweep.inc
+++ b/gpu-sort_amd/csrc/gs_lsb_downsweep.inc
@@ -36,7 +36,7 @@
 
 constexpr uint32_t PIPE_SPIN_LIMIT = 1u << 18;
 
-template <bool HAS_VALUES, bool TAIL, int TW, bool BIG, bool PIPE, bool OFF64 = false, bool CURSOR = false>
+template <bool HAS_VALUES, bool TAIL, int TW, bool BIG, bool PIPE, bool OFF64 = false, bool CURSOR = false, bool RANK_FREE = false>
 __device__ __forceinline__ void downsweep_tile(DownsweepSmem<HAS_VALUES, OFF64> &sm, const uint32_t t,
     const uint32_t *__restrict__ keys_in, uint32_t *__restrict__ keys_out, const uint32_t *__restrict__ vals_in,
     uint32_t *__restrict__ vals_out, const uint32_t *__restrict__ spine, const uint16_t *__restrict__ prefix16,
@@ -204,7 +204,11 @@
     GS_PHASE(1);
 #pragma unroll
     for (int i = 0; i < LSB_KPT; ++i) key[i] = tw_in(key[i]);
-    {
+    if constexpr (RANK_FREE) {
+        static_assert(!RANK_FREE || CURSOR, "only the cursor scatter is free to rank in any order");
+#pragma unroll
+        for (int i = 0; i < LSB_KPT; ++i) pos[i] = __hip_atomic_fetch_add(&my[digit(key[i])], 1u, __ATOMIC_RELAXED, __HIP_MEMORY_SCOPE_WAVEFRONT);
+    } else {
         uint32_t d_prev = 0, plo = 0, phi = 0;
 #pragma unroll
         for (int i = 0; i <= LSB_KPT; ++i) {
diff --git a/gpu-sort_amd/csrc/gs_lsb_plan.hip b/gpu-sort_amd/csrc/gs_lsb_plan.hip
--- a/gpu-sort_amd/csrc/gs_lsb_plan.hip
+++ b/gpu-sort_amd/csrc/gs_lsb_plan.hip
@@ -226,7 +226,9 @@
     if (tid < MSB_NCLASS) plan->blk_class[blockIdx.x][tid] = red[2 + tid];
 }
 
-__global__ __launch_bounds__(RADIX) void lsb_plan_decide_kernel(PlanBlock *__restrict__ plan, uint32_t n, uint32_t parts, uint32_t cursor_on)
+constexpr int PLAN_PEEK_WORDS = 9;
+__global__ __launch_bounds__(RADIX) void lsb_plan_decide_kernel(PlanBlock *__restrict__ plan, uint32_t n, uint32_t parts, uint32_t cursor_on,
+                                                                uint32_t *mailbox)
 {
     __shared__ uint32_t s_base, s_total, s_max, s_nz, s_cls[MSB_NCLASS], s_clsbase[MSB_NCLASS];
     const uint32_t tid = threadIdx.x, b = blockIdx.x;
@@ -274,19 +276,20 @@
             plan->ups_skip[q] = planned && q != 1 ? 1u : 0u;
         }
         plan->offsets[PLAN_GROUPS] = n;
-        plan->cursor_mode = planned && cursor_on ? 1u : 0u;
-    }
-}
-
-constexpr int PLAN_PEEK_WORDS = 9;
-static_assert(offsetof(PlanBlock, total) == (PLAN_PEEK_WORDS - 2) * sizeof(uint32_t), "the head is eight words");
-__global__ void lsb_plan_peek_kernel(const PlanBlock *__restrict__ plan, uint32_t *mailbox)
-{
-    const uint32_t *head = &plan->route;
-    for (int i = 0; i < PLAN_PEEK_WORDS - 1; ++i) mailbox[i] = head[i];
-    mailbox[PLAN_PEEK_WORDS - 1] = plan->cursor_mode;
-    __threadfence_system();
-}
+        const uint32_t mode = planned && cursor_on ? 1u : 0u;
+        plan->cursor_mode = mode;
+        if (mailbox) {
+            mailbox[0] = planned ? PLAN_PLANNED : PLAN_CLASSIC;
+            mailbox[1] = s_max;
+            mailbox[2] = s_nz;
+            for (int c = 0; c < MSB_NCLASS; ++c) mailbox[3 + c] = planned ? s_cls[c] : 0u;
+            mailbox[3 + MSB_NCLASS] = s_total;
+            mailbox[PLAN_PEEK_WORDS - 1] = mode;
+            __threadfence_system();
+        }
+    }
+}
+static_assert(offsetof(PlanBlock, total) == (PLAN_PEEK_WORDS - 2) * sizeof(uint32_t) && PLAN_PEEK_WORDS == 5 + MSB_NCLASS, "the head is eight words");
 
 struct PlanLists { MsbTask *tasks[MSB_NCLASS]; uint32_t cap[MSB_NCLASS]; };
 __global__ __launch_bounds__(PLAN_BLOCK_GROUPS) void lsb_plan_tasks_kernel(const PlanBlock *__restrict__ plan, PlanLists lists)
@@ -388,45 +391,116 @@
     }
 }
 
-__global__ __launch_bounds__(LSB_THREADS) void lsb_plan_irregular_kernel(const uint32_t *__restrict__ keys_in, uint32_t *__restrict__ keys_out,
-                                                                         const PlanBlock *__restrict__ plan, uint32_t *__restrict__ cursor,
-                                                                         uint32_t n)
-{
-    if (!plan->cursor_mode) return;
+__global__ __launch_bounds__(LSB_THREADS) void lsb_plan_cursor_init_kernel(PlanBlock *__restrict__ plan, uint32_t *__restrict__ cursor)
+{
+    const uint32_t i = blockIdx.x * (uint32_t)LSB_THREADS + threadIdx.x;
+    if (i == 0) plan->irr[0] = 0;
+    cursor[i] = plan->offsets[((i & (uint32_t)(RADIX - 1)) << RADIX_BITS) | (i >> RADIX_BITS)];
+}
+static_assert(PLAN_GROUPS % LSB_THREADS == 0, "whole workgroups set the cursors");
+
+#ifndef GS_PLAN_RANK_FREE
+#define GS_PLAN_RANK_FREE 1
+#endif
+template <bool BIG>
+__global__ __launch_bounds__(LSB_THREADS, 6) void lsb_plan_scatter2_cursor_kernel(const uint32_t *__restrict__ keys_in, uint32_t *__restrict__ keys_out,
+                                                                                  uint32_t *__restrict__ irr, uint32_t *__restrict__ cursor,
+                                                                                  PassParams p)
+{
+    __shared__ __attribute__((aligned(16))) DownsweepSmem<false> sm;
+    const uint32_t full_tiles = p.n / (uint32_t)LSB_TILE;
+    if (blockIdx.x >= full_tiles) return;
+    const uint32_t t = tile_of_item_wide(blockIdx.x, full_tiles);
+    constexpr bool RANK_FREE = GS_PLAN_RANK_FREE != 0;
+    downsweep_tile<false, false, 0, BIG, false, false, true, RANK_FREE>(sm, t, keys_in, keys_out, nullptr, nullptr, nullptr, nullptr, nullptr, p, nullptr,
+                                                                        0u, nullptr, threadIdx.x, nullptr, cursor, irr, PLAN_IRR_CAP);
+}
+
+constexpr int PLAN_IRR_ROUNDS = LSB_TILE / LSB_THREADS;
+static_assert(LSB_THREADS == 2 * RADIX, "the follow-up kernel: one thread per group of the tile's first and last d1");
+__global__ __launch_bounds__(LSB_THREADS, 4) void lsb_plan_irregular_kernel(const uint32_t *__restrict__ keys_in, uint32_t *__restrict__ keys_out,
+                                                                            const PlanBlock *__restrict__ plan, uint32_t *__restrict__ cursor,
+                                                                            uint32_t n)
+{
+    __shared__ uint32_t edge[2 * RADIX];
+    const uint32_t mode = plan->cursor_mode, count = plan->irr[0], t = plan->irr[blockIdx.x < PLAN_IRR_CAP ? 1u + blockIdx.x : 1u];
+    asm volatile("" ::"s"(mode), "s"(count), "s"(t));
+    if (!mode) return;
     const uint32_t full_tiles = n / (uint32_t)LSB_TILE;
     uint32_t lo, len;
     if (blockIdx.x == PLAN_IRR_CAP) {
         lo = full_tiles * (uint32_t)LSB_TILE;
         len = n - lo;
+        if (len == 0u) return;
     } else {
-        const uint32_t listed = plan->irr[0] < PLAN_IRR_CAP ? plan->irr[0] : PLAN_IRR_CAP;
+        const uint32_t listed = count < PLAN_IRR_CAP ? count : PLAN_IRR_CAP;
         if (blockIdx.x >= listed) return;
-        const uint32_t t = plan->irr[1u + blockIdx.x];
         if (t >= full_tiles) return;
         lo = t * (uint32_t)LSB_TILE;
         len = (uint32_t)LSB_TILE;
     }
     const int lane = lane_id();
-    for (uint32_t i = threadIdx.x; i - (uint32_t)lane < len; i += (uint32_t)LSB_THREADS) {
-        const bool have = i < len;
-        const uint32_t k = have ? keys_in[lo + i] : 0u;
-        const uint32_t g = k >> 16, c = ((g & (uint32_t)(RADIX - 1)) << RADIX_BITS) | (g >> RADIX_BITS);
-        unsigned long long rest = __builtin_amdgcn_ballot_w64(have);
-        uint32_t at = 0;
-#pragma unroll
-        for (int r = 0; r < 2; ++r) {
-            if (rest == 0ull) break;
-            const int lead = __builtin_amdgcn_readfirstlane(__builtin_ctzll(rest));
-            const uint32_t c0 = (uint32_t)__builtin_amdgcn_readlane((int)c, lead);
-            const unsigned long long m = __builtin_amdgcn_ballot_w64(have && c == c0) & rest;
-            uint32_t first = 0;
-            if (lane == lead) first = __hip_atomic_fetch_add(cursor + c0, (uint32_t)__popcll(m), __ATOMIC_RELAXED, __HIP_MEMORY_SCOPE_AGENT);
-            first = (uint32_t)__builtin_amdgcn_readlane((int)first, lead);
-            if ((m >> lane) & 1ull) at = first + (uint32_t)__popcll(m & ((1ull << lane) - 1ull));
-            rest &= ~m;
-        }
-        if ((rest >> lane) & 1ull) at = __hip_atomic_fetch_add(cursor + c, 1u, __ATOMIC_RELAXED, __HIP_MEMORY_SCOPE_AGENT);
-        if (have && at < n) keys_out[at] = k;
+    const uint32_t tid = threadIdx.x, last = len - 1u;
+    const uint32_t *src = keys_in + lo;
+    uint32_t k[PLAN_IRR_ROUNDS];
+#pragma unroll
+    for (int r = 0; r < PLAN_IRR_ROUNDS; ++r) {
+        const uint32_t i = tid + (uint32_t)r * (uint32_t)LSB_THREADS;
+        k[r] = src[i < last ? i : last];
+    }
+    const uint32_t k_first = src[0], k_last = src[last];
+    asm volatile("" ::"s"(k_first), "s"(k_last));
+    const uint32_t d1_first = (k_first >> 16) & (uint32_t)(RADIX - 1), d1_last = (k_last >> 16) & (uint32_t)(RADIX - 1);
+    edge[tid] = 0;
+    __syncthreads();
+    uint32_t claim[PLAN_IRR_ROUNDS], got[PLAN_IRR_ROUNDS];
+    auto cursor_of = [](uint32_t key) {
+        const uint32_t g = key >> 16;
+        return ((g & (uint32_t)(RADIX - 1)) << RADIX_BITS) | (g >> RADIX_BITS);
+    };
+    auto edge_of = [&](uint32_t key) {
+        const uint32_t d1 = (key >> 16) & (uint32_t)(RADIX - 1);
+        return d1 == d1_first ? key >> 24 : d1 == d1_last ? (uint32_t)RADIX + (key >> 24) : 2u * (uint32_t)RADIX;
+    };
+    const unsigned long long below = (1ull << lane) - 1ull;
+#pragma unroll
+    for (int r = 0; r < PLAN_IRR_ROUNDS; ++r) {
+        const bool have = tid + (uint32_t)r * (uint32_t)LSB_THREADS < len;
+        const uint32_t e = edge_of(k[r]), c = cursor_of(k[r]);
+        const bool mid = have && e == 2u * (uint32_t)RADIX;
+        got[r] = 0;
+        if (have && !mid) got[r] = atomicAdd(&edge[e], 1u);
+        unsigned long long rest = __builtin_amdgcn_ballot_w64(mid);
+        uint32_t cl = (uint32_t)lane;
+        if (rest != 0ull) {
+#pragma unroll
+            for (int q = 0; q < 2; ++q) {
+                const int lead = __builtin_amdgcn_readfirstlane(rest ? __builtin_ctzll(rest) : 0);
+                const uint32_t c0 = (uint32_t)__builtin_amdgcn_readlane((int)c, lead);
+                const unsigned long long m = __builtin_amdgcn_ballot_w64(mid && c == c0) & rest;
+                if ((m >> lane) & 1ull) cl = (uint32_t)lead | ((uint32_t)__popcll(m & below) << 8) | (lane == lead ? (uint32_t)__popcll(m) << 16 : 0u);
+                rest &= ~m;
+            }
+            if ((rest >> lane) & 1ull) cl |= 1u << 16;
+        }
+        claim[r] = cl;
+    }
+#pragma unroll
+    for (int r = 0; r < PLAN_IRR_ROUNDS; ++r)
+        if (claim[r] >> 16) got[r] = __hip_atomic_fetch_add(cursor + cursor_of(k[r]), claim[r] >> 16, __ATOMIC_RELAXED, __HIP_MEMORY_SCOPE_AGENT);
+    __syncthreads();
+    {
+        const uint32_t mine = edge[tid], d1 = tid < (uint32_t)RADIX ? d1_first : d1_last;
+        if (mine) edge[tid] = __hip_atomic_fetch_add(cursor + ((d1 << RADIX_BITS) | (tid & (uint32_t)(RADIX - 1))), mine, __ATOMIC_RELAXED, __HIP_MEMORY_SCOPE_AGENT);
+    }
+    __syncthreads();
+#pragma unroll
+    for (int r = 0; r < PLAN_IRR_ROUNDS; ++r) {
+        const bool have = tid + (uint32_t)r * (uint32_t)LSB_THREADS < len;
+        const uint32_t e = edge_of(k[r]);
+        uint32_t at = (uint32_t)__shfl((int)got[r], (int)(claim[r] & 0xffu)) + ((claim[r] >> 8) & 0xffu);
+        if (e < 2u * (uint32_t)RADIX) at += edge[e];
+        if (have && at < n) keys_out[at] = k[r];
     }
 }
 
@@ -551,7 +625,7 @@
 }
 
 static int lsb_plan_look(const uint32_t *keys, uint32_t *alt, const LsbWorkspace &ws, PlanBlock *plan, uint64_t n, const PassParams &tw,
-                         hipStream_t s)
+                         hipStream_t s, uint32_t *mailbox = nullptr)
 {
     const uint32_t parts = (uint32_t)(n / PLAN_WORDS < PLAN_LOOK_MAX_GRID ? n / PLAN_WORDS : PLAN_LOOK_MAX_GRID);
     const uint32_t chunks = lsb_make_params(n, 16, RADIX_BITS).grid;
@@ -559,7 +633,8 @@
     hipLaunchKernelGGL(lsb_plan_look_kernel, dim3(parts), dim3(PLAN_LOOK_THREADS), 0, s, keys, alt, plan, ws.spine, ws.prefix16, (uint32_t)n,
                        chunks, tw.f32_in, tw.xor_in);
     hipLaunchKernelGGL(lsb_plan_reduce_kernel, dim3(PLAN_BLOCKS), dim3(RADIX), 0, s, alt, plan, parts);
-    hipLaunchKernelGGL(lsb_plan_decide_kernel, dim3(PLAN_BLOCKS), dim3(RADIX), 0, s, plan, (uint32_t)n, parts, plan_cursor_enabled() ? 1u : 0u);
+    hipLaunchKernelGGL(lsb_plan_decide_kernel, dim3(PLAN_BLOCKS), dim3(RADIX), 0, s, plan, (uint32_t)n, parts, plan_cursor_enabled() ? 1u : 0u,
+                       mailbox);
     return (int)hipGetLastError();
 }
 
@@ -570,16 +645,16 @@
     if ((char *)cursor < (char *)ws.prefix16) return hipErrorInvalidValue;
     {
         KernelTimer kt(GS_K_OTHER, s);
-        hipLaunchKernelGGL(lsb_plan_upsweep2_kernel<true>, dim3(p.grid), dim3(LSB_THREADS), 0, s, kin, ws.spine, ws.prefix16, plan, cursor, p);
+        hipLaunchKernelGGL(lsb_plan_cursor_init_kernel, dim3(PLAN_GROUPS / LSB_THREADS), dim3(LSB_THREADS), 0, s, plan, cursor);
     }
     if (p.n >= (uint32_t)LSB_TILE) {
         KernelTimer kt(GS_K_LSB_DOWNSWEEP, s);
+        PassParams q = p;
+        q.shift = 24;
         if (p.n > (1u << 30))
-            hipLaunchKernelGGL((lsb_plan_scatter2_kernel<false, true>), dim3(p.ds_grid), dim3(LSB_THREADS), 0, s, kin, kout, ws.totals,
-                               ws.spine, ws.prefix16, plan, cursor, p);
+            hipLaunchKernelGGL((lsb_plan_scatter2_cursor_kernel<true>), dim3(p.ds_grid), dim3(LSB_THREADS), 0, s, kin, kout, plan->irr, cursor, q);
         else
-            hipLaunchKernelGGL((lsb_plan_scatter2_kernel<false, false>), dim3(p.ds_grid), dim3(LSB_THREADS), 0, s, kin, kout, ws.totals,
-                               ws.spine, ws.prefix16, plan, cursor, p);
+            hipLaunchKernelGGL((lsb_plan_scatter2_cursor_kernel<false>), dim3(p.ds_grid), dim3(LSB_THREADS), 0, s, kin, kout, plan->irr, cursor, q);
     }
     {
         KernelTimer kt(GS_K_OTHER, s);
@@ -636,13 +711,16 @@
     pk.armed = false;
     return &pk;
 }
-static void plan_peek_arm(PlanPeek *pk, const PlanBlock *plan, hipStream_t s)
+static uint32_t *plan_peek_clear(PlanPeek *pk)
+{
+    if (!pk) return nullptr;
+    for (int i = 0; i < PLAN_PEEK_WORDS; ++i) ((volatile uint32_t *)pk->host)[i] = 0;
+    return pk->dev;
+}
+static void plan_peek_arm(PlanPeek *pk, hipStream_t s)
 {
     if (!pk) return;
-    for (int i = 0; i < PLAN_PEEK_WORDS; ++i) ((volatile uint32_t *)pk->host)[i] = 0;
-    KernelTimer kt(GS_K_OTHER, s);
-    hipLaunchKernelGGL(lsb_plan_peek_kernel, dim3(1), dim3(1), 0, s, plan, pk->dev);
-    pk->armed = hipGetLastError() == hipSuccess && hipEventRecord(pk->ev, s) == hipSuccess;
+    pk->armed = hipEventRecord(pk->ev, s) == hipSuccess;
     if (!pk->armed) (void)hipGetLastError();
 }
 struct PlanSeen { bool ok = false; uint32_t route = 0, tasks[MSB_NCLASS] = {0, 0, 0, 0}, cursor_mode = 0; };
@@ -670,6 +748,20 @@
     for (int c = 0; c < MSB_NCLASS; ++c) seen.tasks[c] = w[3 + c];
     return seen;
 }
+#ifndef GS_PLAN_FINISH_CAP
+#define GS_PLAN_FINISH_CAP 2048
+#endif
+constexpr uint32_t PLAN_FINISH_CAP = GS_PLAN_FINISH_CAP;
+static_assert(PLAN_FINISH_CAP == 512 || PLAN_FINISH_CAP == 1024 || PLAN_FINISH_CAP == 2048, "the finish's cap");
+static uint32_t plan_finish_cap()
+{
+    static const uint32_t v = [] {
+        const char *e = getenv("GS_LSB_PLAN_FINISH_CAP");
+        const unsigned long x = e ? strtoul(e, nullptr, 10) : 0ul;
+        return x == 512ul || x == 1024ul || x == 2048ul ? (uint32_t)x : PLAN_FINISH_CAP;
+    }();
+    return v;
+}
 static thread_local uint32_t plan_peek_last[4] = {0, 0, 0, 0};
 
 int lsb_plan_sort(char *base, uint32_t *d_keys[2], int *selector, uint64_t n, int descending, int key_type, hipStream_t s)
@@ -686,9 +778,10 @@
     int sel = *selector, e;
     PassParams tw{};
     lsb_twiddle_masks(key_type, descending, true, true, tw);
-    if ((e = lsb_plan_look(d_keys[sel], d_keys[sel ^ 1], ws, plan, n, tw, s))) return e;
     PlanPeek *peek = plan_peek_get(s);
-    plan_peek_arm(peek, plan, s);
+    e = lsb_plan_look(d_keys[sel], d_keys[sel ^ 1], ws, plan, n, tw, s, plan_peek_clear(peek));
+    plan_peek_arm(peek, s);
+    if (e) return e;
     PlanSeen seen;
     plan_peek_last[0] = plan_peek_last[1] = 0; plan_peek_last[2] = 4; plan_peek_last[3] = (1u << MSB_NCLASS) - 1u;
     for (int slot = 0; slot < 4; ++slot) {
@@ -728,7 +821,7 @@
     }
     if ((e = (int)hipGetLastError())) return e;
     if ((e = msb_local_sorts_in_place(plan->level, lists.tasks, PLAN_GROUPS, PLAN_GROUPS, d_keys[sel], PLAN_SORT_BITS, n, tw.f32_out,
-                                      tw.xor_out, s, seen.ok ? seen.tasks : nullptr)))
+                                      tw.xor_out, s, seen.ok ? seen.tasks : nullptr, plan_finish_cap())))
         return e;
     *selector = sel;
     return hipSuccess;
@@ -784,6 +877,8 @@
     return hipSuccess;
 }
 
+uint32_t gs_lsb_plan_finish_cap(void) { return plan_finish_cap(); }
+
 int gs_lsb_plan_look_only(void *d_temp, const void *d_keys, void *d_alt, uint64_t num_items, int key_type, int descending, void *stream)
 {
     GS_CLEAR_STALE_ERROR();
diff --git a/gpu-sort_amd/csrc/gs_msb.hip b/gpu-sort_amd/csrc/gs_msb.hip
--- a/gpu-sort_amd/csrc/gs_msb.hip
+++ b/gpu-sort_amd/csrc/gs_msb.hip
@@ -1011,6 +1011,25 @@
     static_assert(!(STABLE && MODE != LS_ALL), "the stable sort has one plan");
     auto advance = [&](uint32_t from, MsbTask &out) {
         uint32_t t = from;
+        if constexpr (MODE == LS_FLAGGED || MODE == LS_DEDUPE) {
+            for (; t < ntasks; t += (uint32_t)WAVE * gridDim.x) {
+                const unsigned long long cand = (unsigned long long)t + (unsigned long long)lane * gridDim.x;
+                const bool in = cand < (unsigned long long)ntasks;
+                const MsbTask c = ws.tasks[cls][in ? (uint32_t)cand : t];
+                const bool mine = in && (MODE == LS_FLAGGED ? (c.pad & (LS_FLAG | LS_DONE)) == LS_FLAG
+                                                            : ((c.pad & LS_DD) != 0u && (c.pad & LS_FLAG) != 0u && c.sort_bits > (uint32_t)LOCAL_B1 && c.sort_bits <= 16u));
+                const unsigned long long m = __builtin_amdgcn_ballot_w64(mine);
+                if (m != 0ull) {
+                    const int first = __builtin_amdgcn_readfirstlane(__builtin_ctzll(m));
+                    out.offset = (uint32_t)__builtin_amdgcn_readlane((int)c.offset, first);
+                    out.size = (uint32_t)__builtin_amdgcn_readlane((int)c.size, first);
+                    out.sort_bits = (uint32_t)__builtin_amdgcn_readlane((int)c.sort_bits, first);
+                    out.pad = (uint32_t)__builtin_amdgcn_readlane((int)c.pad, first);
+                    return t + (uint32_t)first * gridDim.x;
+                }
+            }
+            return ntasks;
+        }
         for (; t < ntasks; t += gridDim.x) {
             const MsbTask c = ws.tasks[cls][t];
             const bool mine = MODE == LS_ALL ? (STABLE || (c.pad & LS_DONE) == 0u)
@@ -1609,7 +1628,8 @@
 template <bool HAS_VALUES, bool STABLE = false>
 static void launch_local_sorts(const MsbWs &ws, int L, uint32_t bound, const uint32_t *sk, uint32_t *dk, const uint32_t *sv,
                                uint32_t *dv, int f32_in, uint32_t xor_in, int f32_out, uint32_t xor_out, hipStream_t s,
-                               int min_bits = 0, uint64_t num_items = 0, const uint32_t *known_tasks = nullptr, bool maybe_skew = true)
+                               int min_bits = 0, uint64_t num_items = 0, const uint32_t *known_tasks = nullptr, bool maybe_skew = true,
+                               uint32_t leftover_cap = 0u)
 {
     KernelTimer kt(GS_K_MSB_LOCAL_SORT, s);
     auto grid_of = [&](int c) {
@@ -1624,12 +1644,15 @@
 #endif
         return (uint32_t)(b < MSB_LS_MAX_GRID ? (b ? b : 1) : MSB_LS_MAX_GRID);
     };
-#define GS_LS1P(C, HV, M, P) hipLaunchKernelGGL((msb_local_sort_kernel<msb_class_threads(C), msb_class_kpt(C), HV, STABLE, M, P>), dim3(grid_of(C)), \
-                                               dim3(msb_class_threads(C)), 0, s, ws, L, C, sk, dk, sv, dv, f32_in, xor_in, f32_out, xor_out)
+    auto left_of = [&](int c) {
+        const uint32_t g = grid_of(c);
+        return leftover_cap && leftover_cap < g ? leftover_cap : g;
+    };
+#define GS_LS1G(C, HV, M, P, G) hipLaunchKernelGGL((msb_local_sort_kernel<msb_class_threads(C), msb_class_kpt(C), HV, STABLE, M, P>), dim3(G), \
+                                                  dim3(msb_class_threads(C)), 0, s, ws, L, C, sk, dk, sv, dv, f32_in, xor_in, f32_out, xor_out)
+#define GS_LS1P(C, HV, M, P) GS_LS1G(C, HV, M, P, grid_of(C))
 #define GS_LS1(C, HV, M) GS_LS1P(C, HV, M, false)
-#define GS_LSDD(C, HV, M) hipLaunchKernelGGL((msb_local_sort_kernel<msb_class_threads(C), msb_class_kpt(C), HV, STABLE, M, false>),                \
-                                             dim3(grid_of(C)), dim3(msb_class_threads(C)), 0, s, ws, L, C, sk, dk, sv, dv,                             \
-                                             f32_in, xor_in, f32_out, xor_out)
+#define GS_LSDD(C, HV, M) GS_LS1G(C, HV, M, false, (M) == LS_DEDUPE ? left_of(C) : grid_of(C))
     const bool plain = !f32_in && !xor_in && !f32_out && !xor_out;
     static const bool dedupe_on = [] { const char *e = getenv("GS_MSB_DEDUPE"); return !(e && e[0] == '0'); }();
 #define GS_LS(C, HV)                                                                                                  \
@@ -1640,7 +1663,7 @@
         else if (!onepass_possible(min_bits, local_b1((int)msb_class_cap(C)), local_b1((int)msb_class_cap(C) * (HV ? 2 : 1)) + 2)) \
             { if constexpr (DD) { if (dd) GS_LSDD(C, HV, LS_DEDUPE_ALL); } GS_LS1(C, HV, LS_ALL); }                    \
         else { if (plain) GS_LS1P(C, HV, LS_ONEPASS, true); else GS_LS1(C, HV, LS_ONEPASS);                           \
-               if constexpr (DD) { if (dd) GS_LSDD(C, HV, LS_DEDUPE); } GS_LS1(C, HV, LS_FLAGGED); }                   \
+               if constexpr (DD) { if (dd) GS_LSDD(C, HV, LS_DEDUPE); } GS_LS1G(C, HV, LS_FLAGGED, false, left_of(C)); } \
     } while (0)
     auto wanted = [&](int c) { return !known_tasks || known_tasks[c] != 0u; };
     if constexpr (!STABLE) {
@@ -1658,11 +1681,13 @@
 #undef GS_LS
 #undef GS_LS1
 #undef GS_LS1P
+#undef GS_LS1G
 #undef GS_LSDD
 }
 
 int msb_local_sorts_in_place(MsbLevel *level, MsbTask *const tasks[MSB_NCLASS], uint32_t max_tasks, uint32_t bound, uint32_t *keys,
-                             int sort_bits, uint64_t num_items, int f32_out, uint32_t xor_out, hipStream_t s, const uint32_t *known_tasks)
+                             int sort_bits, uint64_t num_items, int f32_out, uint32_t xor_out, hipStream_t s, const uint32_t *known_tasks,
+                             uint32_t leftover_cap)
 {
     MsbWs ws{};
     ws.level = level;
@@ -1670,7 +1695,8 @@
     ws.max_tasks = max_tasks;
     ws.tile_shift = 13u;
     ws.key_bits = 32u;
-    launch_local_sorts<false>(ws, 0, bound, keys, keys, nullptr, nullptr, 0, 0u, f32_out, xor_out, s, sort_bits, num_items, known_tasks);
+    launch_local_sorts<false>(ws, 0, bound, keys, keys, nullptr, nullptr, 0, 0u, f32_out, xor_out, s, sort_bits, num_items, known_tasks, true,
+                              leftover_cap);
     return (int)hipGetLastError();
 }
 
diff --git a/gpu-sort_amd/csrc/gs_msb_tasks.hpp b/gpu-sort_amd/csrc/gs_msb_tasks.hpp
--- a/gpu-sort_amd/csrc/gs_msb_tasks.hpp
+++ b/gpu-sort_amd/csrc/gs_msb_tasks.hpp
@@ -38,6 +38,6 @@
 
 int msb_local_sorts_in_place(MsbLevel *level, MsbTask *const tasks[MSB_NCLASS], uint32_t max_tasks, uint32_t bound, uint32_t *keys,
                              int sort_bits, uint64_t num_items, int f32_out, uint32_t xor_out, hipStream_t s,
-                             const uint32_t *known_tasks = nullptr);
+                             const uint32_t *known_tasks = nullptr, uint32_t leftover_cap = 0u);
 
 }
diff --git a/include/gpusort.h b/include/gpusort.h
--- a/include/gpusort.h
+++ b/include/gpusort.h
@@ -57,6 +57,7 @@
 int  gs_lsb_plan_status(void *d_temp, uint64_t num_items, uint32_t out[8], void *stream);
 int  gs_lsb_plan_cursor_status(void *d_temp, uint64_t num_items, uint32_t out[4], void *stream);
 int  gs_lsb_plan_peek_status(uint32_t out[4]);
+uint32_t gs_lsb_plan_finish_cap(void);
 int  gs_lsb_plan_look_only(void *d_temp, const void *d_keys, void *d_alt, uint64_t num_items,
                            int key_type, int descending, void *stream);
 int  gs_lsb_plan_layout(uint64_t num_items, uint64_t out[4]);
```

New measurement: 171.4 Gkeys/s (median of 6 runs). +6.0%, better.
